# Accustomer/CUDA-AKAZE

Measured on AMD Instinct MI355X. Metric: pairs_per_sec_detect_describe_match_1080p, higher is better.
Workload: dtype f32; 1 GPU; configs[1]: 1920x1080 grayscale pairs, 4 octaves x 4 sublevels, PM_G2, MLDB-486, max_pts 10000, float path; detect+describe both images + match, D2H included; pairs_per_launch_sequence=256, distinct_pairs_per_gpu=16, float_sequences_enqueued=77, octave_streams=one stream per context, step_pipeline=2, rank0_gpu_numa_node=1

## Files before the change

### cuda-akaze_amd/akaze_hip/__init__.py

```python
import ctypes as C
import os

import numpy as np

try:
    import torch as _torch
except ImportError:
    _torch = None

_HERE = os.path.dirname(os.path.abspath(__file__))
LIB_PATH = os.environ.get("HAK_LIB") or os.path.join(os.path.dirname(_HERE), "libhipakaze.so")

FLEN = 61
MAX_DIST = 96
PM_G1, PM_G2, WEICKERT, CHARBONNIER = 0, 1, 2, 3

POINT_DTYPE = np.dtype([
    ("x", "<f4"), ("y", "<f4"), ("octave", "<i4"), ("response", "<f4"), ("size", "<f4"), ("angle", "<f4"),
    ("features", "u1", (FLEN,)), ("_pad", "u1", (3,)),
    ("match", "<i4"), ("distance", "<i4"), ("match_x", "<f4"), ("match_y", "<f4"),
])
assert POINT_DTYPE.itemsize == 104
MATCH_PAIR_DTYPE = np.dtype([("query", "<i4"), ("train", "<i4"), ("distance", "<i4"), ("second", "<i4"),
                             ("x1", "<f4"), ("y1", "<f4"), ("x2", "<f4"), ("y2", "<f4")])
assert MATCH_PAIR_DTYPE.itemsize == 32
HOMOGRAPHY_DTYPE = np.dtype([("H", "<f4", (9,)), ("inliers", "<i4"), ("hypothesis", "<i4"), ("refined", "<i4"),
                             ("n", "<i4")])
assert HOMOGRAPHY_DTYPE.itemsize == 52


class HakError(RuntimeError):
    pass


class hak_config(C.Structure):
    _fields_ = [
        ("noctaves", C.c_int), ("max_scale", C.c_int), ("per", C.c_float), ("kcontrast", C.c_float),
        ("soffset", C.c_float), ("reordering", C.c_int), ("derivative_factor", C.c_float),
        ("dthreshold", C.c_float), ("diffusivity", C.c_int), ("descriptor_pattern_size", C.c_int),
        ("max_pts", C.c_int), ("upright", C.c_int), ("batch", C.c_int),
    ]


class hak_traffic(C.Structure):
    _fields_ = [("fed_px_steps", C.c_double), ("fed_bytes", C.c_double), ("all_stage_bytes", C.c_double),
                ("fed_launches", C.c_int), ("fed_fused_bytes", C.c_double), ("hessian_bytes", C.c_double),
                ("prologue_bytes", C.c_double), ("describe_bytes", C.c_double), ("nms_bytes", C.c_double)]


PROF = dict(fed=0, lowpass=1, flow=2, hessian=3, contrast=4, down=5, extrema=6, nms=7, describe=8, match=9)

_vp, _fp, _ip = C.c_void_p, C.POINTER(C.c_float), C.POINTER(C.c_int)
SYMBOLS = {
    "hak_device_count": (C.c_int, []),
    "hak_set_device": (C.c_int, [C.c_int]),
    "hak_last_error": (C.c_char_p, []),
    "hak_default_config": (None, [C.POINTER(hak_config)]),
    "hak_create": (C.c_int, [C.POINTER(hak_config), C.c_int, C.c_int, C.POINTER(_vp)]),
    "hak_destroy": (None, [_vp]),
    "hak_set_stream": (C.c_int, [_vp, _vp]),
    "hak_sync": (C.c_int, [_vp]),
    "hak_wait_event": (C.c_int, [_vp, _vp]),
    "hak_phase_event": (C.c_int, [_vp, C.POINTER(C.c_void_p)]),
    "hak_set_concurrency": (C.c_int, [_vp, C.c_int]),
    "hak_set_null_order": (C.c_int, [_vp, C.c_int]),
    "hak_set_retain_best": (C.c_int, [_vp, C.c_int]),
    "hak_set_retain_grid": (C.c_int, [_vp, C.c_int]),
    "hak_detect_and_compute": (C.c_int, [_vp, _vp, C.c_int, _vp, C.c_int, _ip, _vp, C.c_int]),
    "hak_detect_and_compute_pair": (C.c_int, [_vp, _vp, _vp, C.c_int, _vp, _vp, C.c_int, C.c_int, _ip, _ip, _vp, _vp, C.c_int, C.c_int]),
    "hak_detect_and_compute_batch": (C.c_int, [_vp, _vp, C.c_long, C.c_int, C.c_int, _vp, _vp, C.c_int]),
    "hak_fast_detect_and_compute": (C.c_int, [_vp, _vp, C.c_int, _vp, C.c_int, _ip, _vp, C.c_int]),
    "hak_fast_detect_and_compute_batch": (C.c_int, [_vp, _vp, C.c_long, C.c_int, C.c_int, _vp, _vp, C.c_int]),
    "hak_match": (C.c_int, [_vp, _vp, C.c_int, _vp, C.c_int, _vp]),
    "hak_match_batch": (C.c_int, [_vp, _vp, _vp, C.c_int]),
    "hak_match_knn2": (C.c_int, [_vp, _vp, C.c_int, _vp, C.c_int, C.c_int, C.c_int, C.c_int, C.c_int, _vp, _vp, _ip, _vp]),
    "hak_match_knn2_batch": (C.c_int, [_vp, _vp, _vp, C.c_int, C.c_int, C.c_int, C.c_int, C.c_int, _vp, _vp]),
    "hak_find_homography": (C.c_int, [_vp, _vp, C.c_int, C.c_int, C.c_float, C.c_uint, C.c_int, _vp, _vp]),
    "hak_find_homography_batch": (C.c_int, [_vp, _vp, C.c_long, _vp, C.c_int, C.c_int, C.c_float, C.c_uint, C.c_int, _vp, _vp]),
    "hak_match_guided": (C.c_int, [_vp, _vp, C.c_int, _vp, C.c_int, _fp, C.c_float, C.c_int, C.c_int, C.c_int, C.c_int, _vp, _vp, _ip, _vp]),
    "hak_match_guided_batch": (C.c_int, [_vp, _vp, _vp, C.c_int, _vp, C.c_float, C.c_int, C.c_int, C.c_int, C.c_int, _vp, _vp]),
    "hak_points_alloc": (C.c_int, [C.POINTER(_vp), C.c_int]),
    "hak_points_free": (C.c_int, [_vp]),
    "hak_image_alloc": (C.c_int, [C.POINTER(_vp), C.c_int, C.c_int, _ip]),
    "hak_image_upload": (C.c_int, [_vp, C.c_int, _vp, C.c_int, C.c_int]),
    "hak_image_free": (C.c_int, [_vp]),
    "hak_ingest_u8": (C.c_int, [_vp, _vp, C.c_long, C.c_int, _vp, C.c_long, C.c_int, C.c_int, C.c_int, C.c_int]),
    "hak_host_alloc": (C.c_int, [C.POINTER(_vp), C.c_long]),
    "hak_host_free": (C.c_int, [_vp]),
    "hak_download_batch": (C.c_int, [_vp, _vp, _vp, C.c_int, _vp, _vp]),
    "hak_memcpy_d2h": (C.c_int, [_vp, _vp, C.c_long]),
    "hak_memcpy_h2d": (C.c_int, [_vp, _vp, C.c_long]),
    "hak_fed_tau": (C.c_int, [C.c_float, C.c_int, C.c_float, C.c_int, _fp, C.c_int]),
    "hak_gauss_taps": (None, [C.c_float, C.c_int, _fp]),
    "hak_compare_indices": (None, [_ip, _ip]),
    "hak_describe_plan_query": (C.c_int, [C.c_int, C.POINTER(C.c_uint), C.POINTER(C.c_uint)]),
    "hak_query_schedule": (C.c_int, [_vp, _ip, _ip, _fp, _fp]),
    "hak_query_geometry": (C.c_int, [_vp, _ip]),
    "hak_query_traffic": (C.c_int, [_vp, C.c_int, C.POINTER(hak_traffic)]),
    "hak_prof_enable": (C.c_int, [_vp, C.c_int]),
    "hak_prof_read": (C.c_int, [_vp, C.c_int, C.POINTER(C.c_double), _ip]),
    "hak_prof_reset": (C.c_int, [_vp]),
}
TEST_SYMBOLS = {
    "hak_debug_plane": (C.c_int, [_vp, C.c_int, C.c_int, C.c_int, C.c_int, _vp]),
    "hak_debug_kcontrast": (C.c_int, [_vp, C.c_int, _fp]),
    "hak_op_lowpass": (C.c_int, [_vp, _vp, C.c_int, C.c_int, C.c_int, C.c_float, C.c_int]),
    "hak_op_down_smooth": (C.c_int, [_vp, _vp, _vp, C.c_int, C.c_int, C.c_int, C.c_int, C.c_int, C.c_int]),
    "hak_op_kcontrast": (C.c_int, [_vp, C.c_int, C.c_int, C.c_int, C.c_float, _fp, _fp, _ip]),
    "hak_op_flow": (C.c_int, [_vp, _vp, C.c_int, C.c_int, C.c_int, C.c_int, C.c_float]),
    "hak_op_nld_steps": (C.c_int, [_vp, _vp, _vp, _vp, C.c_int, C.c_int, C.c_int, _fp, C.c_int]),
    "hak_op_rcp_check": (C.c_int, [C.c_uint, C.c_uint, C.POINTER(C.c_ulonglong)]),
    "hak_op_smooth_flow": (C.c_int, [_vp, _vp, _vp, C.c_int, C.c_int, C.c_int, C.c_int, C.c_float]),
    "hak_op_hessian": (C.c_int, [_vp, _vp, _vp, _vp, C.c_int, C.c_int, C.c_int, C.c_int]),
    "hak_debug_set_plane": (C.c_int, [_vp, C.c_int, C.c_int, C.c_int, C.c_int, _vp]),
    "hak_op_tail_begin": (C.c_int, [_vp]),
    "hak_op_tail_level": (C.c_int, [_vp, C.c_int, C.c_int, _vp]),
    "hak_op_tail_det_level": (C.c_int, [_vp, C.c_int, C.c_int, _vp]),
    "hak_op_tail_seed": (C.c_int, [_vp, _vp, _vp]),
    "hak_op_tail_finish": (C.c_int, [_vp, _vp, C.c_int, C.c_int, C.c_int, _ip]),
    "hak_op_orient_describe": (C.c_int, [_vp, _vp, C.c_int, C.c_int]),
    "hak_op_copy_probe": (C.c_int, [C.c_long, C.c_int, C.POINTER(C.c_double)]),
    "hak_op_copy_probe_shapes": (C.c_int, [C.c_long, C.c_int, C.POINTER(C.c_double), C.c_int]),
    "hak_op_stream_probe": (C.c_int, [C.c_int, C.c_int, C.c_int, C.c_int, C.c_int, C.c_int, C.POINTER(C.c_double), C.POINTER(C.c_double)]),
    "hak_op_hess_probe": (C.c_int, [C.c_int, C.c_int, C.c_int, C.c_int, C.c_int, C.POINTER(C.c_double), C.POINTER(C.c_double)]),
    "hak_debug_fill_match_scratch": (C.c_int, [_vp, C.c_int]),
    "hak_op_gather_probe": (C.c_int, [C.c_long, C.c_int, C.c_int, C.c_int, C.POINTER(C.c_double)]),
}

if not os.path.exists(LIB_PATH):
    raise ImportError(
        f"{LIB_PATH} is missing: build it with `python -c 'import __graft_entry__ as g; g.build()'` "
        "(there is no CPU fallback for the HIP path)")
TEST_LIB_PATH = os.path.join(os.path.dirname(LIB_PATH), "libhipakaze_test.so")


class _Libs:

    def __init__(self):
        self.product = C.CDLL(LIB_PATH, mode=C.RTLD_GLOBAL)
        self.test = None
        for name, (res, args) in SYMBOLS.items():
            try:
                f = getattr(self.product, name)
            except AttributeError:
                if os.environ.get("HAK_LIB"):
                    continue
                raise
            f.restype, f.argtypes = res, args
            setattr(self, name, f)

    def load_test(self):
        if self.test is None:
            if not os.path.exists(TEST_LIB_PATH):
                raise ImportError(f"{TEST_LIB_PATH} is missing: build it with `make -C cuda-akaze_amd/csrc`")
            self.test = C.CDLL(TEST_LIB_PATH)
            for name, (res, args) in TEST_SYMBOLS.items():
                f = getattr(self.test, name)
                f.restype, f.argtypes = res, args
                setattr(self, name, f)
        return self.test

    def __getattr__(self, name):
        if name in TEST_SYMBOLS:
            self.load_test()
            return self.__dict__[name]
        raise AttributeError(name)


lib = _Libs()


def check(status):
    if status != 0:
        raise HakError(lib.hak_last_error().decode() or f"libhipakaze status {status}")


def iAlignUp(a, b):
    return a - a % b + b if a % b else a


def device_count():
    return lib.hak_device_count()


def default_config(**kw):
    cfg = hak_config()
    lib.hak_default_config(C.byref(cfg))
    for k, v in kw.items():
        setattr(cfg, k, v)
    return cfg


def fed_tau(T, M=1, tau_max=0.25, reordering=True):
    buf = np.zeros(4096, np.float32)
    n = lib.hak_fed_tau(T, M, tau_max, int(reordering), buf.ctypes.data_as(_fp), 4096)
    if n < 0:
        raise HakError("FED cycle too long")
    return buf[:n].copy()


def gauss_taps(var, radius):
    buf = np.zeros(8, np.float32)
    lib.hak_gauss_taps(var, radius, buf.ctypes.data_as(_fp))
    return buf[:radius + 1].copy()


def compare_indices():
    a = np.zeros(488, np.int32)
    b = np.zeros(488, np.int32)
    lib.hak_compare_indices(a.ctypes.data_as(_ip), b.ctypes.data_as(_ip))
    return a, b


def describe_plan(pattern_size):
    pos = np.zeros((7, 64), np.uint32)
    cell = np.zeros((7, 64), np.uint32)
    ok = lib.hak_describe_plan_query(pattern_size, pos.ctypes.data_as(C.POINTER(C.c_uint)), cell.ctypes.data_as(C.POINTER(C.c_uint)))
    return bool(ok), pos, cell


class AkazeData:

    def __init__(self):
        self.num_pts = 0
        self.max_pts = 0
        self.h_data = None
        self.d_data = None
        self.h_pinned = None


def initAkazeData(data, max_pts, host, dev, pinned=False):
    data.num_pts = 0
    data.max_pts = max_pts
    data.h_pinned = None
    if host and pinned:
        hp = _vp()
        check(lib.hak_host_alloc(C.byref(hp), max_pts * POINT_DTYPE.itemsize))
        data.h_pinned = hp.value
        buf = (C.c_uint8 * (max_pts * POINT_DTYPE.itemsize)).from_address(hp.value)
        data.h_data = np.frombuffer(buf, dtype=POINT_DTYPE)
        data.h_data[:] = np.zeros(1, POINT_DTYPE)[0]
    else:
        data.h_data = np.zeros(max_pts, POINT_DTYPE) if host else None
    data.d_data = None
    if dev:
        p = _vp()
        check(lib.hak_points_alloc(C.byref(p), max_pts))
        data.d_data = p.value


def freeAkazeData(data):
    if data.d_data is not None:
        check(lib.hak_points_free(data.d_data))
    data.d_data = None
    data.h_data = None
    if getattr(data, "h_pinned", None):
        check(lib.hak_host_free(data.h_pinned))
        data.h_pinned = None
    data.num_pts = 0
    data.max_pts = 0


class Akazer:
# ... 225 lines not shown
```

### cuda-akaze_amd/csrc/fed_common.h

```cpp
#pragma once
#include "hak_internal.h"
#include <type_traits>

template <typename V> struct FedV;
template <> struct FedV<float> { using V4 = float4; };
template <> struct FedV<int> { using V4 = int4; };
__device__ __forceinline__ float4 mk4(float a, float b, float c, float d) { return make_float4(a, b, c, d); }
__device__ __forceinline__ int4 mk4(int a, int b, int c, int d) { return make_int4(a, b, c, d); }
__device__ __forceinline__ float vadd(float a, float b) { return a + b; }
__device__ __forceinline__ float vsub(float a, float b) { return a - b; }
__device__ __forceinline__ float vmul(float a, float b) { return a * b; }
__device__ __forceinline__ int vadd(int a, int b) { return (int)((unsigned)a + (unsigned)b); }
__device__ __forceinline__ int vsub(int a, int b) { return (int)((unsigned)a - (unsigned)b); }
__device__ __forceinline__ int vmul(int a, int b) { return (int)((unsigned)a * (unsigned)b); }
__device__ __forceinline__ float vstep(float f, float sum, float L) { return fmaf(f, sum, L); }
__device__ __forceinline__ int vstep(int f, int sum, int L) { return vadd(vmul(f, sum >> 16) >> 16, L); }

template <typename V, int NS>
struct FedFacs { V f[NS]; };

__device__ __forceinline__ int hak_dpp_shr1(int v) { return __builtin_amdgcn_update_dpp(0, v, 0x138, 0xf, 0xf, true); }
__device__ __forceinline__ int hak_dpp_shl1(int v) { return __builtin_amdgcn_update_dpp(0, v, 0x130, 0xf, 0xf, true); }
__device__ __forceinline__ float wave_shr1(float v) { return __int_as_float(hak_dpp_shr1(__float_as_int(v))); }
__device__ __forceinline__ float wave_shl1(float v) { return __int_as_float(hak_dpp_shl1(__float_as_int(v))); }
__device__ __forceinline__ int wave_shr1(int v)
{
    int r = hak_dpp_shr1(v);
    asm volatile("" : "+v"(r));
    return r;
}
__device__ __forceinline__ int wave_shl1(int v)
{
    int r = hak_dpp_shl1(v);
    asm volatile("" : "+v"(r));
    return r;
}

typedef float hak_v4f __attribute__((ext_vector_type(4)));
typedef int hak_v4i __attribute__((ext_vector_type(4)));
__device__ __forceinline__ void hak_store_nt(float4* p, const float4 v)
{
    const hak_v4f t = {v.x, v.y, v.z, v.w};
    __builtin_nontemporal_store(t, reinterpret_cast<hak_v4f*>(p));
}
__device__ __forceinline__ void hak_store_nt(int4* p, const int4 v)
{
    const hak_v4i t = {v.x, v.y, v.z, v.w};
    __builtin_nontemporal_store(t, reinterpret_cast<hak_v4i*>(p));
}

typedef unsigned hak_v4u __attribute__((ext_vector_type(4)));
constexpr unsigned HAK_BUF_OOB = 0x40000000u;
__device__ __forceinline__ __amdgpu_buffer_rsrc_t hak_buf_rsrc(void* base)
{
    return __builtin_amdgcn_make_buffer_rsrc(base, 0, HAK_BUF_OOB, 0x00020000);
}
__device__ __forceinline__ void hak_buf_store_nt(__amdgpu_buffer_rsrc_t r, unsigned voff, const float4 v)
{
    const hak_v4u d = {__float_as_uint(v.x), __float_as_uint(v.y), __float_as_uint(v.z), __float_as_uint(v.w)};
    __builtin_amdgcn_raw_buffer_store_b128(d, r, voff, 0, 2);
}
__device__ __forceinline__ void hak_buf_store_nt(__amdgpu_buffer_rsrc_t r, unsigned voff, const int4 v)
{
    const hak_v4u d = {(unsigned)v.x, (unsigned)v.y, (unsigned)v.z, (unsigned)v.w};
    __builtin_amdgcn_raw_buffer_store_b128(d, r, voff, 0, 2);
}

__device__ __forceinline__ float4 hak_load_stream(const float4* p)
{
#ifdef HAK_NT_LOADS
    const hak_v4f t = __builtin_nontemporal_load(reinterpret_cast<const hak_v4f*>(p));
    return make_float4(t.x, t.y, t.z, t.w);
#else
    return *p;
#endif
}
__device__ __forceinline__ int4 hak_load_stream(const int4* p)
{
#ifdef HAK_NT_LOADS
    const hak_v4i t = __builtin_nontemporal_load(reinterpret_cast<const hak_v4i*>(p));
    return make_int4(t.x, t.y, t.z, t.w);
#else
    return *p;
#endif
}

constexpr int pmod(int a, int m) { return ((a % m) + m) % m; }

template <typename V> struct GHrow { V h1, h2, h3, h4; };
__device__ __forceinline__ float vneg(float a) { return -a; }
__device__ __forceinline__ int vneg(int a) { return (int)(0u - (unsigned)a); }

template <bool XEDGE, typename V, typename V4>
__device__ __forceinline__ V4 fed_row(const V4 Lc, const GHrow<V>& gh, const V4 Qn, const V4 Qp, int x0, int w, V stepfac)
{
    const V Lr = wave_shl1(Lc.x);
    const V d1 = vsub(Lc.y, Lc.x), d2 = vsub(Lc.z, Lc.y), d3 = vsub(Lc.w, Lc.z), d4 = vsub(Lr, Lc.w);
    const V P1 = vmul(gh.h1, d1), P2 = vmul(gh.h2, d2), P3 = vmul(gh.h3, d3);
    V P4 = vmul(gh.h4, d4);
    if (XEDGE) P4 = x0 + 3 == w - 1 ? vneg(P3) : P4;
    V P0 = wave_shr1(P4);
    if (XEDGE) P0 = x0 == 0 ? vneg(P1) : P0;
    V4 o;
    o.x = vstep(stepfac, vsub(vadd(vsub(P1, P0), Qn.x), Qp.x), Lc.x);
    o.y = vstep(stepfac, vsub(vadd(vsub(P2, P1), Qn.y), Qp.y), Lc.y);
    o.z = vstep(stepfac, vsub(vadd(vsub(P3, P2), Qn.z), Qp.z), Lc.z);
    o.w = vstep(stepfac, vsub(vadd(vsub(P4, P3), Qn.w), Qp.w), Lc.w);
    return o;
}
template <typename V, typename V4>
__device__ __forceinline__ V4 fed_q(const V4 gv, const V4 Ln, const V4 Lc)
{
    return mk4(vmul(gv.x, vsub(Ln.x, Lc.x)), vmul(gv.y, vsub(Ln.y, Lc.y)), vmul(gv.z, vsub(Ln.z, Lc.z)), vmul(gv.w, vsub(Ln.w, Lc.w)));
}
template <typename V4> __device__ __forceinline__ V4 vneg4(const V4 a) { return mk4(vneg(a.x), vneg(a.y), vneg(a.z), vneg(a.w)); }
template <typename V4> __device__ __forceinline__ V4 vsel4(const bool c, const V4 a, const V4 b)
{
    return mk4(c ? a.x : b.x, c ? a.y : b.y, c ? a.z : b.z, c ? a.w : b.w);
}


template <typename V> struct SfTaps { V k0, k1, k2; };
__device__ __forceinline__ float sf_conv(float c, float a1, float b1, float a2, float b2, const SfTaps<float>& t)
{
    float ws = c * t.k0;
    ws += t.k1 * (a1 + b1);
    ws += t.k2 * (a2 + b2);
    return ws;
}
__device__ __forceinline__ int sf_conv(int c, int a1, int b1, int a2, int b2, const SfTaps<int>& t)
{
    const unsigned ws = (unsigned)c * (unsigned)t.k0 + (unsigned)t.k1 * (unsigned)(a1 + b1) + (unsigned)t.k2 * (unsigned)(a2 + b2);
    return (int)ws >> 16;
}
__device__ __forceinline__ float sf_dif2(float dx, float dy, float ikc) { return ikc * (dx * dx + dy * dy); }
__device__ __forceinline__ float sf_dif2(int dx, int dy, float ikc)
{
    return (float)(int)((unsigned)dx * (unsigned)dx + (unsigned)dy * (unsigned)dy) * ikc;
}
__device__ __forceinline__ void sf_store_g(float* o, float g) { *o = g; }
__device__ __forceinline__ void sf_store_g(int* o, float g) { *o = (int)(g * 65536 + 0.5f); }

__device__ __forceinline__ float sf_g_value(float g) { return g; }
__device__ __forceinline__ int sf_g_value_int(float g) { return (int)(g * 65536 + 0.5f); }
template <typename V> __device__ __forceinline__ V sf_g_as(float g);
template <> __device__ __forceinline__ float sf_g_as<float>(float g) { return g; }
template <> __device__ __forceinline__ int sf_g_as<int>(float g) { return (int)(g * 65536 + 0.5f); }

__device__ __forceinline__ float hak_rcp_newton(float d)
{
    const float y0 = __builtin_amdgcn_rcpf(d);
    const float e = fmaf(-d, y0, 1.0f);
    return fmaf(e, y0, y0);
}
```

### cuda-akaze_amd/csrc/hak_api.hip

```cpp
#include "hak_internal.h"
#include <chrono>
#include <cmath>
#include <cstdio>
#include <cstring>
#include <mutex>
#include <string>
#include <vector>

#include "hak_ctx.h"

static thread_local std::string g_err;
int hak_fail(const std::string& m) { g_err = m; return 1; }

extern "C" const char* hak_last_error(void) { return g_err.c_str(); }

extern "C" int hak_device_count(void)
{
    int n = 0;
    if (hipGetDeviceCount(&n) != hipSuccess) return 0;
    return n;
}

extern "C" int hak_set_device(int dev)
{
// ... 719 lines not shown
        if (!c) { pool_release(sc, false); (void)hipFree(buf); }
        return fail("hak_match_guided: out of device memory for the search scratch");
    }
    int4* fwd = sc->knn;
    int4* rev = sc->knn + n1;
    *sc->h_cnt = -1;
    {
        ProfScope ps(c, HAK_PROF_MATCH);
        hak_launch_guided(st, d_pts1, d_pts2, nullptr, nullptr, n1, n2, 0, 0, 1, nullptr, H, radius, cross_check ? 1 : 0,
                          hak_guided_scratch_carve(buf, 1, cap2, rev, 0), fwd, 0);
        hak_launch_knn2_finish(st, d_pts1, d_pts2, nullptr, n1, 0, 0, 1, fwd, cross_check ? rev : nullptr, 0, ratio_num, ratio_den,
                               cross_check ? 1 : 0, max_dist, d_out, 0, sc->d_cnt, sc);
    }
    int rc = 0;
    if (hipGetLastError() != hipSuccess) rc = fail("guided match launch failed");
    if (!rc && hipStreamSynchronize(st) != hipSuccess) rc = fail("hipStreamSynchronize(guided match)");
    rc = match_list_tail(c, sc, rc, h_pts1, d_pts1, n1, d_out, count, h_out);
    if (!c) (void)hipFree(buf);
    return rc;
}

extern "C" int hak_match_guided_batch(hak_ctx* c, hak_point* d_points, const int* d_num_pts, int npairs, const hak_homography* d_H,
                                      float radius, int ratio_num, int ratio_den, int cross_check, int max_dist, hak_match_pair* d_out,
                                      int* d_counts)
{
    if (!c) return fail("hak_match_guided_batch needs a context");
    if (!d_points || !d_num_pts || !d_H || !d_counts || npairs < 1) return fail("bad argument");
    if (2 * npairs > c->cfg.batch + 1) return fail("npairs exceeds the context's batch capacity");
    if (guided_args(radius, ratio_num, ratio_den)) return 1;
    if (max_dist <= 0) max_dist = HAK_MAX_DIST;
    const long mp = c->cfg.max_pts;
    if (!hak_mkey_fits(mp)) return fail("max_pts must stay below 2^20 for the matcher");
    if (knn_scratch(c)) return 1;
    const long npair_cap = (c->cfg.batch + 1) / 2;
    if (guided_scratch(c, hak_guided_scratch_bytes(npair_cap, mp))) return 1;
    order_after_null_stream(c, c->stream);
    int4* fwd = c->knn;
    int4* rev = c->knn + (size_t)npair_cap * mp;
    { ProfScope ps(c, HAK_PROF_MATCH);
      hak_launch_guided(c->stream, d_points, d_points + mp, d_num_pts, d_num_pts + 1, (int)mp, (int)mp, 2 * mp, 2 * mp, npairs, d_H, nullptr,
                        radius, cross_check ? 1 : 0, hak_guided_scratch_carve(c->guided, npair_cap, mp, rev, mp), fwd, mp);
      hak_launch_knn2_finish(c->stream, d_points, d_points + mp, d_num_pts, 0, 2 * mp, 2 * mp, npairs, fwd, cross_check ? rev : nullptr,
                             mp, ratio_num, ratio_den, cross_check ? 1 : 0, max_dist, d_out, mp, d_counts); }
    if (hipGetLastError() != hipSuccess) return fail("guided match launch failed");
    return 0;
}

extern "C" int hak_points_alloc(hak_point** d, int count)
{
    HIP_TRY(hipMalloc((void**)d, sizeof(hak_point) * (size_t)count));
    HIP_TRY(hipMemset(*d, 0, sizeof(hak_point) * (size_t)count));
    HIP_TRY(hipStreamSynchronize(nullptr));
    return 0;
}
extern "C" int hak_points_free(hak_point* d) { HIP_TRY(hipFree(d)); return 0; }

extern "C" int hak_image_alloc(float** d, int w, int h, int* pitch)
{
    int p = (w % 128 != 0) ? (w - w % 128 + 128) : w;
    HIP_TRY(hipMalloc((void**)d, sizeof(float) * (size_t)p * h));
    if (pitch) *pitch = p;
    return 0;
}
extern "C" int hak_image_upload(float* d, int pitch, const float* hsrc, int w, int h)
{
    HIP_TRY(hipMemcpy2D(d, sizeof(float) * pitch, hsrc, sizeof(float) * w, sizeof(float) * w, h, hipMemcpyHostToDevice));
    return 0;
}
extern "C" int hak_image_free(float* d) { HIP_TRY(hipFree(d)); return 0; }

extern "C" int hak_ingest_u8(hak_ctx* c, const unsigned char* d_src, long src_stride, int src_pitch,
                             float* d_dst, long dst_stride, int dst_pitch, int w, int h, int nimg)
{
    if (!d_src || !d_dst || w < 1 || h < 1 || nimg < 1 || src_pitch < w || dst_pitch < w) return fail("bad ingest argument");
    if (hak_device_count() == 0) return fail("no HIP device: libhipakaze has no CPU fallback");
    order_after_null_stream(c, c ? c->stream : nullptr);
    hak_launch_ingest_u8(c ? c->stream : nullptr, d_src, src_stride, src_pitch, d_dst, dst_stride, dst_pitch, w, h, nimg);
    if (hipGetLastError() != hipSuccess) return fail("ingest launch failed");
    return 0;
}
extern "C" int hak_host_alloc(void** p, long bytes) { HIP_TRY(hipHostMalloc(p, (size_t)bytes)); return 0; }
extern "C" int hak_host_free(void* p) { HIP_TRY(hipHostFree(p)); return 0; }

extern "C" int hak_download_batch(hak_ctx* c, const hak_point* d_points, const int* d_num_pts, int nimg,
                                  hak_point* h_points, int* h_num_pts)
{
    if (!c || !d_points || !d_num_pts || !h_points || !h_num_pts) return fail("null argument");
    {
        hipPointerAttribute_t ap{}, an{};
        const bool pinned = hipPointerGetAttributes(&ap, h_points) == hipSuccess && ap.type == hipMemoryTypeHost &&
                            hipPointerGetAttributes(&an, h_num_pts) == hipSuccess && an.type == hipMemoryTypeHost;
        (void)hipGetLastError();
        if (pinned) {
            hak_launch_download(c->stream, d_points, d_num_pts, c->cfg.max_pts, nimg, h_points, h_num_pts);
            if (hipGetLastError() != hipSuccess) return fail("download launch failed");
            HIP_TRY(hipStreamSynchronize(c->stream));
            return 0;
        }
    }
    HIP_TRY(hipMemcpyAsync(h_num_pts, d_num_pts, sizeof(int) * (size_t)nimg, hipMemcpyDeviceToHost, c->stream));
    HIP_TRY(hipStreamSynchronize(c->stream));
    const long mp = c->cfg.max_pts;
    for (int i = 0; i < nimg; i++)
        if (h_num_pts[i] > 0)
            HIP_TRY(hipMemcpyAsync(h_points + i * mp, d_points + i * mp, sizeof(hak_point) * (size_t)h_num_pts[i],
                                   hipMemcpyDeviceToHost, c->stream));
    HIP_TRY(hipStreamSynchronize(c->stream));
    return 0;
}

extern "C" int hak_memcpy_d2h(void* dst, const void* src, long bytes)
{
    HIP_TRY(hipMemcpy(dst, src, (size_t)bytes, hipMemcpyDeviceToHost));
    return 0;
}
extern "C" int hak_memcpy_h2d(void* dst, const void* src, long bytes)
{
    HIP_TRY(hipMemcpy(dst, src, (size_t)bytes, hipMemcpyHostToDevice));
    return 0;
}

extern "C" int hak_query_schedule(const hak_ctx* c, int* nsteps, int* sigma_size, float* sizes, float* borders)
{
    if (!c) return -1;
    for (size_t l = 0; l < c->plan.size(); l++) {
        if (nsteps) nsteps[l] = c->plan[l].nsteps;
        if (sigma_size) sigma_size[l] = c->plan[l].sigma_size;
        if (sizes) sizes[l] = c->plan[l].size;
        if (borders) borders[l] = c->plan[l].border;
    }
    return c->L.noct;
}

extern "C" int hak_query_geometry(const hak_ctx* c, int* whp)
{
    if (!c) return -1;
    for (int o = 0; o < c->L.noct; o++) {
        whp[3 * o] = c->L.oct[o].w; whp[3 * o + 1] = c->L.oct[o].h; whp[3 * o + 2] = c->L.oct[o].p;
    }
    return c->L.noct;
}

extern "C" int hak_query_traffic(const hak_ctx* c, int npts_hint, hak_traffic* out)
{
    if (!c || !out) return fail("null argument");
    const HakLayout& L = c->L;
    double pxsteps = 0, all = 0, folded = 0;
    int launches = 0;
    for (int o = 0; o < L.noct; o++) {
        const double N = (double)L.oct[o].w * L.oct[o].h;
        for (int s = 0; s < L.ms; s++) {
            const LevelPlan& lp = c->plan[(size_t)o * L.ms + s];
            pxsteps += N * lp.nsteps;
            launches += lp.nsteps ? hak_fed_groups(lp.nsteps, c->knobs.max_fuse, L.oct[o].w) : 0;
            if (s > 0 && hak_fed_sf_covers(c->knobs, c->cfg.diffusivity, L.oct[o], c->cfg.batch)) folded += 16.0 * N;
            if (s == 0 && o > 0 && hak_fed_sf_covers(c->knobs, c->cfg.diffusivity, L.oct[o], c->cfg.batch, &L.oct[o - 1]))
                folded += 4.0 * L.oct[o - 1].w * L.oct[o - 1].h + 16.0 * N;
            if (o == 0 && s == 0) all += 56.0 * N;
            else if (s == 0) all += 4.0 * L.oct[o - 1].w * L.oct[o - 1].h + 8.0 * N + 8.0 * N + 24.0 * N + 4.0 * N;
            else all += 44.0 * N;
        }
    }
    all += 16.0 * L.oct[0].w * L.oct[0].h;
    all += 12.0 * pxsteps;
    all += (872.0 + 5292.0 + 104.0) * npts_hint;
    out->fed_px_steps = pxsteps;
    out->fed_bytes = 12.0 * pxsteps + folded;
    out->all_stage_bytes = all;
    out->fed_launches = launches;
    out->fed_fused_bytes = c->fed_fused_bytes;
    double lvl_px = 0;
    for (int o = 0; o < L.noct; o++) lvl_px += (double)L.ms * L.oct[o].w * L.oct[o].h;
    out->hessian_bytes = 12.0 * lvl_px;
    out->prologue_bytes = 16.0 * L.oct[0].w * L.oct[0].h;
    out->describe_bytes = (872.0 + 5292.0) * npts_hint;
    out->nms_bytes = 104.0 * npts_hint;
    return 0;
}

extern "C" int hak_prof_enable(hak_ctx* c, int on) { if (!c) return 1; c->prof_on = on != 0; return 0; }
extern "C" int hak_prof_reset(hak_ctx* c)
{
    if (!c) return 1;
    for (auto& p : c->prof) { p.used = 0; p.acc_ms = 0; p.launches = 0; }
    return 0;
}
extern "C" int hak_prof_read(hak_ctx* c, int k, double* total_ms, int* launches)
{
    if (!c || k < 0 || k >= HAK_PROF_COUNT) return fail("bad profile class");
    HIP_TRY(hipStreamSynchronize(c->stream));
    ProfClass& p = c->prof[k];
    for (size_t i = 0; i + 1 < p.used; i += 2) {
        float ms = 0;
        HIP_TRY(hipEventElapsedTime(&ms, p.ev[i], p.ev[i + 1]));
        p.acc_ms += ms;
    }
    p.used = 0;
    if (total_ms) *total_ms = p.acc_ms;
    if (launches) *launches = p.launches;
    return 0;
}
```

### cuda-akaze_amd/csrc/hak_internal.h

```cpp
#pragma once
#include <cstdlib>
#include <hip/hip_runtime.h>
#include <stdint.h>
#include "../../include/hipakaze.h"
#include "hak_knobs.h"

#define HAK_NBINS 300
#define HAK_WAVE 64

struct HakOct {
    int w, h, p;
    long plane;
};

struct HakLayout {
    int noct, ms;
    HakOct oct[HAK_MAX_OCTAVES];
    long lvl_off[HAK_MAX_OCTAVES];
    long smooth_off[HAK_MAX_OCTAVES], flow_off[HAK_MAX_OCTAVES], tmp_off[HAK_MAX_OCTAVES];
    long arena;

    __host__ __device__ long lt(int o, int s) const { return lvl_off[o] + (long)s * oct[o].plane; }
    __host__ __device__ long dxy(int o, int s) const { return lvl_off[o] + (long)(ms + 2 * s) * oct[o].plane; }
};
// ... 235 lines not shown
    unsigned prefix;
    int pad;
};
#define HAK_SEL_BINS 2048
#define HAK_SEL_PASSES 3
struct HakSelScratch {
    HakSelState* st = nullptr;
    unsigned* bins = nullptr;
    int* tie = nullptr;
};

__device__ __forceinline__ unsigned sel_key(unsigned u, int fast)
{
    return fast ? (u ^ 0x80000000u) : ((u >> 31) ? ~u : (u | 0x80000000u));
}
__device__ __forceinline__ int sel_cap(int img, int max_pts, int cap0, int cap1)
{
    return cap0 > 0 ? (img == 0 ? cap0 : cap1) : max_pts;
}

#define HAK_GRID_MIN 8
#define HAK_GRID_MAX 128
struct HakGridState {
    int active;
    int cap;
    int q;
    int rem;
};
struct HakGridScratch {
    HakGridState* st = nullptr;
    int* count = nullptr;
    unsigned long long* comp = nullptr;
    long cell_cap = 0;
    int G = 0;
};

struct HakBatch {
    float* base;
    long stride;
    int nimg;
    HakImgState* state;
    unsigned long long* maps;
    long map_stride;
    unsigned long long* bitmap;
    int* rowcount;
    unsigned long long* cand;
    long cand_cap;
    const HakKnobs* knobs = nullptr;
    int* perm = nullptr;
    int perm_cap = 0;
    int cap0 = 0, cap1 = 0;
    HakSelScratch sel{};
    HakGridScratch grid{};
};
static inline HakKnobs hak_knobs_of(const HakBatch* b) { return (b && b->knobs) ? *b->knobs : hak_knobs_from_env(); }
template <typename V>
static inline HakExtremaArgs<V> hak_extrema_args(const HakBatch* b, const HakLayout* L, const HakTables* htab, int octave, int sub, V threshold)
{
    HakExtremaArgs<V> ex{};
    if (b) {
        const int layer = octave * L->ms + sub;
        ex.maps = b->maps; ex.map_stride = b->map_stride; ex.cand = b->cand; ex.cand_cap = b->cand_cap;
        ex.state = b->state; ex.p0 = L->oct[0].p; ex.octave = octave; ex.layer = layer;
        ex.psz = (int)htab->borders[octave * L->ms]; ex.border = htab->borders[layer]; ex.threshold = threshold;
    }
    return ex;
}

void hak_launch_lowpass(hipStream_t st, const float* src, long src_stride, int src_pitch, float* dst, long dst_stride,
                        int w, int h, int p, int nimg, const float* taps, int R);
void hak_launch_down_smooth(hipStream_t st, const float* src, float* dst, float* smooth, long stride,
                            HakOct so, HakOct dd, int nimg, const float* taps);
void hak_launch_contrast(hipStream_t st, const float* smooth, long stride, int w, int h, int p, int nimg,
                         HakImgState* state, float per, int noct);
void hak_launch_reset_state(hipStream_t st, HakImgState* state, int nimg);
void hak_launch_flow(hipStream_t st, const float* src, float* dst, long stride, int w, int h, int p, int nimg,
                     int diffusivity, const HakImgState* state, int octave, float fixed_ikc = 0.f);
static inline bool hak_stream_pays(int mode, int w, int h, int nimg)
{
    if (mode != 1) return mode != 0;
    const long strips = (w + 239) / 240;
    return strips * ((h + 31) / 32) * nimg >= 2048;
}
static inline int hak_stream_rows(int h, long strips_times_images, int min_rows)
{
    const long want = hak_process_knobs().stream_min_waves;
    int nseg = 4 * ((h + 512) / 1024 > 1 ? (h + 512) / 1024 : 1);
    while (strips_times_images * nseg < want && (h + 2 * nseg - 1) / (2 * nseg) >= min_rows) nseg *= 2;
    const int ry = (h + nseg - 1) / nseg;
    return ry > min_rows ? ry : min_rows;
}
static inline bool hak_hessian_stream_covers(int w, int h, int step, bool lp)
{
    return step >= 1 && step <= 4 && (w & 3) == 0 && w >= 16 && h >= 2 * step + 2 && (!lp || h >= 8);
}
bool hak_launch_hessian_stream(hipStream_t st, const float* src, float* dxy, float* det, bool store_det, long stride,
                               int w, int h, int p, int nimg, int step, float fac1, float fac2,
                               const HakBatch* b, const HakLayout* L, const HakTables* htab, int octave, int sub, float dthreshold,
                               const float* lp_taps = nullptr);
bool hak_launch_hessian_stream(hipStream_t st, const int* src, int* dxy, int* det, bool store_det, long stride,
                               int w, int h, int p, int nimg, int step, int fac1, int fac2,
                               const HakBatch* b, const HakLayout* L, const HakTables* htab, int octave, int sub, int idthreshold);
bool hak_launch_hessian_level(hipStream_t st, const float* src, float* dxy, float* det, bool store_det, long stride,
                              int w, int h, int p, int nimg, int step,
                              const HakBatch* b, const HakLayout* L, const HakTables* htab, int octave, int sub, float dthreshold,
                              const float* lp_taps = nullptr);
bool hak_launch_hessian_level(hipStream_t st, const int* src, int* dxy, int* det, bool store_det, long stride,
                              int w, int h, int p, int nimg, int step,
                              const HakBatch* b, const HakLayout* L, const HakTables* htab, int octave, int sub, int idthreshold);
bool hak_launch_base_stream(hipStream_t st, const float* img, long img_stride, int sp, float* lt, float* grad, long stride, int w, int h,
                            int p, int nimg, const float* taps1, const float* taps_base, int R, HakImgState* state, int mode);
bool hak_launch_base_stream(hipStream_t st, const unsigned char* img, long img_stride, int sp, int* lt, int* grad, long stride, int w,
                            int h, int p, int nimg, const int* taps1, const int* taps_base, int R, HakImgState* state, int mode);
bool hak_launch_base_level(hipStream_t st, const float* img, long img_stride, int sp, float* lt, float* grad_scratch, long stride,
                           int w, int h, int p, int nimg, const float* taps1, const float* taps_base, int R,
                           HakImgState* state, float per, int noct, const HakKnobs& knobs);
bool hak_launch_base_level(hipStream_t st, const unsigned char* img, long img_stride, int sp, int* lt, int* grad_scratch, long stride,
                           int w, int h, int p, int nimg, const int* taps1, const int* taps_base, int R, HakImgState* state,
                           float per, int noct, const HakKnobs& knobs);
void hak_launch_smooth_flow(hipStream_t st, const float* src, float* smooth, float* flow, long stride,
                            int w, int h, int p, int nimg, const float* taps, int diffusivity,
                            const HakImgState* state, int octave, float fixed_ikc = 0.f);
void hak_launch_smooth_flow(hipStream_t st, const int* src, int* smooth, int* flow, long stride,
                            int w, int h, int p, int nimg, const int* taps, int diffusivity,
                            const HakImgState* state, int octave);
#define HAK_LEVEL_TILE_MAX_PX (1920L * 1088L)
int hak_launch_level_tile(hipStream_t st, const float* src, HakOct so, bool head, float* smooth, float* dst, float* tmp, long stride,
                          HakOct dd, int nimg, const float* taps, int diffusivity, const float* tau, int n,
                          const HakImgState* state, int octave, float* dxy = nullptr, int step = 0, const HakBatch* b = nullptr,
                          const HakLayout* L = nullptr, const HakTables* htab = nullptr, int sub = 0, float dthreshold = 0.f,
                          bool* hess_done = nullptr, float fixed_ikc = 0.f);
int hak_launch_level_tile(hipStream_t st, const int* src, HakOct so, bool head, int* smooth, int* dst, int* tmp, long stride,
                          HakOct dd, int nimg, const int* taps, int diffusivity, const float* tau, int n,
                          const HakImgState* state, int octave, int* dxy = nullptr, int step = 0, const HakBatch* b = nullptr,
                          const HakLayout* L = nullptr, const HakTables* htab = nullptr, int sub = 0, int idthreshold = 0, bool* hess_done = nullptr);
int hak_launch_rcp_check(unsigned lo, unsigned hi, unsigned long long* d_bad);
static inline bool hak_fed_sf_covers(const HakKnobs& kn, int diffusivity, const HakOct& dd, int nimg, const HakOct* so = nullptr)
{
    if (!hak_stream_pays(kn.fuse_sf, dd.w, dd.h, nimg) || diffusivity != HAK_PM_G2 || (dd.w & 3) != 0 || dd.w < 16 || dd.h < 8) return false;
    return !so || (kn.fuse_head && !(so->w & 1) && !(so->h & 1));
}
bool hak_launch_fed_sf_head(hipStream_t st, const float* src, HakOct so, float* smooth, float* flow, float* dst, long stride,
                            HakOct dd, int nimg, const float* taps, int diffusivity, const float* tau, int ns,
                            const HakImgState* state, int octave, bool write_g);
bool hak_launch_fed_sf_head(hipStream_t st, const int* src, HakOct so, int* smooth, int* flow, int* dst, long stride,
                            HakOct dd, int nimg, const int* taps, int diffusivity, const float* tau, int ns,
                            const HakImgState* state, int octave, bool write_g);
bool hak_launch_fed_sf(hipStream_t st, const float* src, float* smooth, float* flow, float* dst, long stride,
                       int w, int h, int p, int nimg, const float* taps, int diffusivity, const float* tau, int ns,
                       const HakImgState* state, int octave, bool write_g, bool store_smooth = true, float fixed_ikc = 0.f);
bool hak_launch_fed_sf(hipStream_t st, const int* src, int* smooth, int* flow, int* dst, long stride,
                       int w, int h, int p, int nimg, const int* taps, int diffusivity, const float* tau, int ns,
                       const HakImgState* state, int octave, bool write_g);
int hak_fed_groups(int n, int max_fuse, int w);
int hak_fed_group_size(int n, int G, int g);
void hak_launch_fed_group(hipStream_t st, const float* src, const float* flow, float* dst, long stride,
                          int w, int h, int p, int nimg, const float* tau, int ns);
void hak_launch_fed_group(hipStream_t st, const int* src, const int* flow, int* dst, long stride,
                          int w, int h, int p, int nimg, const float* tau, int ns);
void hak_launch_derivate(hipStream_t st, const float* src, float* dxy, long stride,
                         int w, int h, int p, int nimg, int step);
void hak_launch_hessian(hipStream_t st, const float* dxy, float* det, long stride,
                        int w, int h, int p, int nimg, int step);
void hak_deriv_factors(float* fac1, float* fac2);
void hak_launch_deinterleave(hipStream_t st, const float* ab, float* a, float* b, int w, int h, int p);

void hak_launch_ingest_u8(hipStream_t st, const unsigned char* src, long src_stride, int sp, float* dst, long dst_stride,
                          int dp, int w, int h, int nimg);

void hak_launch_extrema_level(hipStream_t st, const HakBatch& b, const HakLayout& L, const HakTables* htab, int octave,
                              int s, float dthreshold, long det_off);
void hak_launch_extrema_level(hipStream_t st, const HakBatch& b, const HakLayout& L, const HakTables* htab, int octave, int s, int threshold,
                              long det_off);
void hak_launch_download(hipStream_t st, const hak_point* d_points, const int* d_num, long max_pts, int nimg, hak_point* h_points,
                         int* h_num);
struct HakPairDst { hak_point* d[2]; hak_point* h[2]; int cap[2]; };
void hak_launch_download_pair(hipStream_t st, const hak_point* src, const int* d_num, long max_pts, const HakPairDst& dst, int* h_num);
void hak_launch_nms_emit(hipStream_t st, const HakBatch& b, const HakLayout& L, const HakTables* tab, int psz,
                         hak_point* points, int max_pts, int* num_out, int fast = 0, int refine = 1);
void hak_launch_clear_maps(hipStream_t st, const HakBatch& b, const HakLayout& L);
void hak_launch_select(hipStream_t st, const HakBatch& b, const HakLayout& L, int max_pts, int cap0, int cap1, int fast);
void hak_launch_grid_select(hipStream_t st, const HakBatch& b, const HakLayout& L, int max_pts, int cap0, int cap1, int fast);
void hak_launch_seed_maps(hipStream_t st, const HakBatch& b, const HakLayout& L, const unsigned* d_resp_bits, const int* d_layer);

void hak_launch_down_smooth(hipStream_t st, const int* src, int* dst, int* smooth, long stride, HakOct so, HakOct dd, int nimg,
                            const int* taps);
void hak_launch_contrast(hipStream_t st, const int* smooth, long stride, int w, int h, int p, int nimg, HakImgState* state,
                         float per, int noct);
void hak_launch_flow(hipStream_t st, const int* src, int* dst, long stride, int w, int h, int p, int nimg, int type,
                     const HakImgState* state, int octave);
void hakf_launch_reset(hipStream_t st, HakImgState* state, int nimg);
void hakf_launch_conv_u8(hipStream_t st, const unsigned char* src, long src_stride, int sp, int* dst, long dst_stride,
                         int w, int h, int p, int nimg, const int* taps, int R);
void hakf_launch_conv_int(hipStream_t st, const int* src, int* dst, long stride, int w, int h, int p, int nimg, const int* taps, int R);
void hakf_launch_nld_step(hipStream_t st, const int* src, const int* flow, int* dst, long stride, int w, int h, int p, int nimg, float tau);
void hakf_launch_hessian(hipStream_t st, const int* src, int* dxy, int* det, long stride, int w, int h, int p, int nimg, int step);
void hakf_launch_det(hipStream_t st, const int* dxy, int* det, long stride, int w, int h, int p, int nimg, int step);
void hakf_launch_describe(hipStream_t st, const HakBatch& b, const HakLayout& L, const HakTables* tab, hak_point* points, int max_pts,
                          int patsize, int upright, int desc, int planned);

void hak_launch_describe(hipStream_t st, const HakBatch& b, const HakLayout& L, const HakTables* tab,
                         hak_point* points, int max_pts, int patsize, int upright, int desc, int planned, int orient = 1);

#define HAK_COPY_SHAPES 26
int hak_launch_copy_probe(long bytes, int iters, double* ms_per_copy, double* shapes_ms = nullptr);
int hak_launch_gather_probe(long bytes, int blocks, int per_lane, int iters, double* ms_per_launch);
int hak_launch_stream_probe(int w, int h, int nimg, int nwrite, int warm, int iters, double* ms, double* bytes);
int hak_launch_hess_probe(int w, int h, int nimg, int step, int iters, double* ms, double* bytes);

static inline int hak_grid_x(int blocks) { return blocks < 1 ? 1 : blocks > 4096 ? 4096 : blocks; }

#define HAK_MKEY_BITS 20
#define HAK_MKEY_EMPTY 0xFFFFFFFFu
static inline bool hak_mkey_fits(long n) { return n < (1L << HAK_MKEY_BITS); }
__device__ __forceinline__ unsigned hak_mkey(unsigned dist, unsigned index) { return (dist << HAK_MKEY_BITS) | index; }
__device__ __forceinline__ unsigned hak_mkey_dist(unsigned k) { return k >> HAK_MKEY_BITS; }
__device__ __forceinline__ int hak_mkey_index(unsigned k) { return (int)(k & ((1u << HAK_MKEY_BITS) - 1u)); }
__device__ __forceinline__ void hak_mkey_two_smallest(unsigned& best, unsigned& sec, unsigned key)
{
    sec = min(sec, max(best, key));
    best = min(best, key);
}
__device__ __forceinline__ void hak_desc_load(const hak_point* p, unsigned int d[16])
{
    const unsigned int* f = reinterpret_cast<const unsigned int*>(p->features);
#pragma unroll
    for (int i = 0; i < 15; i++) d[i] = f[i];
    d[15] = f[15] & 0xFFu;
}
__device__ __forceinline__ unsigned hak_bcnt_acc(unsigned x, unsigned acc)
{
    unsigned r;
    asm("v_bcnt_u32_b32 %0, %1, %2" : "=v"(r) : "v"(x), "v"(acc));
    return r;
}
#define HAK_KNN_NO_DIST 512
__device__ __forceinline__ int4 hak_knn_none() { return make_int4(-1, HAK_KNN_NO_DIST, HAK_KNN_NO_DIST, 0); }
__device__ __forceinline__ int4 hak_knn_record(unsigned k1, unsigned k2)
{
    if (k1 == HAK_MKEY_EMPTY) return hak_knn_none();
    return make_int4(hak_mkey_index(k1), (int)hak_mkey_dist(k1), k2 == HAK_MKEY_EMPTY ? HAK_KNN_NO_DIST : (int)hak_mkey_dist(k2), 0);
}
__device__ __forceinline__ void hak_match_store(hak_point* p1, const hak_point* __restrict__ pts2, bool ok, int bi, int dist)
{
    if (ok) {
        p1->match = bi;
        p1->distance = dist;
        p1->match_x = pts2[bi].x;
        p1->match_y = pts2[bi].y;
    } else {
        p1->match = -1;
        p1->distance = -1;
        p1->match_x = -1.f;
        p1->match_y = -1.f;
    }
}
__device__ __forceinline__ void hak_match_decide(hak_point* p1, const hak_point* __restrict__ pts2, int n2, unsigned kmin, int attain)
{
    const int dmin = (int)hak_mkey_dist(kmin);
    const bool ok = kmin != HAK_MKEY_EMPTY && attain == 1 && dmin < HAK_MAX_DIST;
    hak_match_store(p1, pts2, ok, min(hak_mkey_index(kmin), max(n2 - 1, 0)), dmin);
}
template <typename F>
__device__ __forceinline__ void hak_match_decide_classes(hak_point* p1, const hak_point* __restrict__ pts2, int n2, F cls)
{
    unsigned kmin = cls(0);
#pragma unroll
    for (int t = 1; t < 16; t++)
        if (hak_mkey_dist(cls(t)) < hak_mkey_dist(kmin)) kmin = cls(t);
    int attain = 0;
#pragma unroll
    for (int t = 0; t < 16; t++) attain += hak_mkey_dist(cls(t)) == hak_mkey_dist(kmin) ? 1 : 0;
    hak_match_decide(p1, pts2, n2, kmin, attain);
}
__device__ __forceinline__ void hak_match_merge_slice(unsigned& K, unsigned& M, unsigned k2, unsigned m2)
{
    if (hak_mkey_dist(k2) < hak_mkey_dist(K)) M = m2;
    else if (hak_mkey_dist(k2) == hak_mkey_dist(K)) M |= m2;
    K = min(K, k2);
}
__device__ __forceinline__ bool hak_knn2_rule(const int i, const int n1, const int4* __restrict__ fwd, const int4* __restrict__ rev,
                                              const int ratio_num, const int ratio_den, const int cross, const int max_dist, int4& f)
{
    f = hak_knn_none();
    if (i >= n1) return false;
    f = fwd[i];
    bool ok = f.x >= 0 && f.y < max_dist && (long)f.y * ratio_den < (long)f.z * ratio_num;
    if (ok && cross) ok = rev[f.x].x == i;
    return ok;
}
__device__ __forceinline__ hak_match_pair hak_knn2_pair(int i, const int4 f, const hak_point* pts1, const hak_point* __restrict__ pts2)
{
    hak_match_pair r;
    r.query = i; r.train = f.x; r.distance = f.y; r.second = f.z;
    r.x1 = pts1[i].x; r.y1 = pts1[i].y; r.x2 = pts2[f.x].x; r.y2 = pts2[f.x].y;
    return r;
}

struct HakMatchScratch {
    unsigned* keys = nullptr; long keys_cap = 0;
    int* ticket = nullptr; long ticket_cap = 0;
    uint2* part = nullptr; long part_cap = 0;
    int4* knn = nullptr; long knn_cap = 0;
    int* blk = nullptr; long blk_cap = 0;
    int* d_cnt = nullptr; int* h_cnt = nullptr;
    int device = -1;
};
// ... 35 lines not shown
```

### cuda-akaze_amd/csrc/hak_knobs.h

```cpp
#pragma once
#include "../../include/hipakaze.h"

#define HAK_FED_MAX_FUSE 4

struct HakKnobs {
    int hess_stream = 1;
    int base_stream = 1;
    int base_hist = 0;
    int hess_cbuf = 256;
    int desc_order = 4;
    int desc_plan = 1;
    int desc_sort = 1;
    int hess_lp = 0;
    int level_tile = 1;
    int level_hess = 1;
    int level_min_steps = 8;
    int level_min_blocks = 96;
    int fuse_sf = 1;
    int fuse_head = 1;
    int max_fuse = 4;
    int hist_min_blocks = 256;
    int hist_rpb_max = 8;
    int hess_side = 0;
    int spine_max_px = 0;
    int side_streams = HAK_MAX_OCTAVES;
    int graph_pads = 1;
    int tail_fork = 1;
    int graph = 1;
    int serial = 0;
    int null_order = 1;
    int timing = 0;
    int prof_fence = 0;
    int stream_min_waves = 2048;
    int download_blocks = 128;
};
HakKnobs hak_knobs_from_env();
const HakKnobs& hak_process_knobs();

struct HakMatchKnobs {
    int valu = 0;
    int qt = 1;
    int slices = 0;
};
HakMatchKnobs hak_match_knobs_from_env();
```

### cuda-akaze_amd/csrc/hak_sequence.hip

```cpp
#include "hak_internal.h"
#include <cstdio>
#include <cstring>
#include <string>
#include <type_traits>

#include "hak_ctx.h"

static thread_local const char* g_launch_err = nullptr;
void hak_note_launch_error(const char* msg) { if (!g_launch_err) g_launch_err = msg; }

void order_after_null_stream(hak_ctx* c, hipStream_t st)
{
    if (!c || !c->null_order || !c->ev_null || st == nullptr) return;
    const hipError_t q = hipStreamQuery(nullptr);
    if (q == hipSuccess) return;
    (void)hipGetLastError();
    if (hipEventRecord(c->ev_null, nullptr) != hipSuccess || hipStreamWaitEvent(st, c->ev_null, 0) != hipSuccess) (void)hipGetLastError();
}

void maps_guard_begin(hak_ctx* c)
{
    if (c->maps_dirty) {
        const size_t h = c->L.oct[0].h, words = (c->L.oct[0].w + 63) / 64, B = c->cfg.batch;
        (void)hipMemsetAsync(c->maps, 0, sizeof(unsigned long long) * (size_t)c->L.oct[0].plane * B, c->stream);
        (void)hipMemsetAsync(c->bitmap, 0, sizeof(unsigned long long) * h * words * B, c->stream);
        (void)hipMemsetAsync(c->rowcount, 0, sizeof(int) * h * B, c->stream);
    }
    c->maps_dirty = true;
}
int maps_guard_end(hak_ctx* c, int rc)
{
    if (!rc) c->maps_dirty = false;
    if (c->ev_last) (void)hipEventRecord(c->ev_last, c->sync_stream ? c->sync_stream : c->stream);
    return rc;
}

static bool level_tile_pays(const hak_ctx* c, const HakOct& oc, int nimg)
{
    const int mode = c->knobs.level_tile;
    if (mode != 1) return mode != 0;
    return c->knobs.fuse_sf != 2 && (long)oc.w * oc.h * nimg <= HAK_LEVEL_TILE_MAX_PX;
}

static bool spine_pays(const hak_ctx* c, int nimg)
{
    const long max_px = c->knobs.spine_max_px;
    if (max_px > 0 && c->knobs.level_tile == 1) return c->knobs.fuse_sf != 2 && (long)c->L.oct[0].w * c->L.oct[0].h * nimg <= max_px;
    return level_tile_pays(c, c->L.oct[0], nimg);
}

struct LevelArgs {
    hak_ctx* c;
    HakBatch b;
    const void* images;
    long image_stride;
    int pitch, nimg;
    bool hess_fused[HAK_MAX_OCTAVES * HAK_MAX_SCALES];
    bool hess_lp[HAK_MAX_OCTAVES * HAK_MAX_SCALES];
};

static LevelArgs level_args(hak_ctx* c, const void* images, long image_stride, int pitch, int nimg)
{
    const HakLayout& L = c->L;
    LevelArgs a{c, HakBatch{c->arena, L.arena, nimg, c->state, c->maps, L.oct[0].plane, c->bitmap, c->rowcount, c->cand, c->cand_cap, &c->knobs,
                            c->perm, c->cfg.max_pts},
                images, image_stride, pitch, nimg, {}, {}};
    hak_batch_selection(c, a.b);
    return a;
}

template <typename V> constexpr bool is_fast = std::is_same_v<V, int>;
template <typename V> static const V* taps_of(const float* f, const int* i) { if constexpr (is_fast<V>) return i; else return f; }
template <typename V> static V dthreshold_of(const hak_ctx* c) { if constexpr (is_fast<V>) return 65; else return c->cfg.dthreshold; }

template <typename V>
static void build_level(LevelArgs& a, int o, int s, hipStream_t st, V* smooth_alt = nullptr)
{
    hak_ctx* const c = a.c;
    hak_ctx* const pc = is_fast<V> ? nullptr : c;
    const hak_config& cfg = c->cfg;
    const HakLayout& L = c->L;
    const HakKnobs& kn = c->knobs;
    const int nimg = a.nimg;
    V* const A = reinterpret_cast<V*>(c->arena);
    const long S = L.arena;
    const HakOct oc = L.oct[o];
    V* smooth = smooth_alt ? smooth_alt : A + L.smooth_off[o];
    V* flow = A + L.flow_off[o];
    V* tmp = A + L.tmp_off[o];
    const LevelPlan& lp = c->plan[(size_t)o * L.ms + s];
    V* Lt = A + L.lt(o, s);
    const V* taps1 = taps_of<V>(c->taps1, c->itaps1);
    auto count_fed = [&](int nl, double bytes) { if constexpr (!is_fast<V>) { c->fed_launches += nl; c->fed_fused_bytes += bytes; } };
    if (o == 0 && s == 0) {
        ProfScope ps(pc, HAK_PROF_CONTRAST, st);
        const auto* img = static_cast<const std::conditional_t<is_fast<V>, unsigned char, float>*>(a.images);
        const V* taps_base = taps_of<V>(c->taps_base, c->itaps_base);
        const bool based = hak_launch_base_level(st, img, a.image_stride, a.pitch, Lt, tmp, S, oc.w, oc.h, oc.p, nimg, taps1, taps_base, c->base_R,
                                                 c->state, cfg.per, L.noct, kn);
        if constexpr (is_fast<V>) {
            if (!based) {
                hakf_launch_conv_u8(st, img, a.image_stride, a.pitch, smooth, S, oc.w, oc.h, oc.p, nimg, taps1, 2);
                hak_launch_contrast(st, smooth, S, oc.w, oc.h, oc.p, nimg, c->state, cfg.per, L.noct);
                hakf_launch_conv_u8(st, img, a.image_stride, a.pitch, Lt, S, oc.w, oc.h, oc.p, nimg, taps_base, c->base_R);
            }
        } else (void)based;
        return;
    }
    const int n = lp.nsteps;
    if (level_tile_pays(c, oc, nimg) && (is_fast<V> || s == 0 || n >= kn.level_min_steps || kn.level_tile == 2)) {
        ProfScope ps(pc, HAK_PROF_FED, st);
        const int nl = hak_launch_level_tile(st, s == 0 ? A + L.lt(o - 1, 0) : A + L.lt(o, s - 1), s == 0 ? L.oct[o - 1] : oc, s == 0, smooth, Lt, tmp, S,
                                             oc, nimg, taps1, cfg.diffusivity, lp.tau.data(), n, c->state, o,
                                             kn.level_hess ? A + L.dxy(o, s) : nullptr, lp.sigma_size, &a.b, &L, &c->htab, s, dthreshold_of<V>(c),
                                             &a.hess_fused[o * HAK_MAX_SCALES + s]);
        count_fed(nl, (s == 0 ? 1.0 * L.oct[o - 1].w * L.oct[o - 1].h : 4.0 * oc.w * oc.h) + 8.0 * oc.w * oc.h + (nl - 1) * 12.0 * oc.w * oc.h);
        return;
    }
    const int G = hak_fed_groups(n, kn.max_fuse, oc.w);
    const int ns0 = hak_fed_group_size(n, G, 0);
    V* dst0 = (G % 2 == 1) ? Lt : tmp;
    const V* fsrc;
    bool fused_first = false;
    if (s == 0) {
        if (hak_fed_sf_covers(kn, cfg.diffusivity, oc, nimg, &L.oct[o - 1])) {
            ProfScope ps(pc, HAK_PROF_FED, st);
            fused_first = hak_launch_fed_sf_head(st, A + L.lt(o - 1, 0), L.oct[o - 1], smooth, flow, dst0, S, oc, nimg, taps1, cfg.diffusivity,
                                                 lp.tau.data(), ns0, c->state, o, G > 1);
            if (fused_first) count_fed(1, 2.0 * L.oct[o - 1].w * L.oct[o - 1].h + (G > 1 ? 12.0 : 8.0) * oc.w * oc.h);
        }
        V* first = (G % 2 == 0) ? Lt : tmp;
        if (!fused_first) {
            { ProfScope ps(pc, HAK_PROF_DOWN, st);
              hak_launch_down_smooth(st, A + L.lt(o - 1, 0), first, smooth, S, L.oct[o - 1], oc, nimg, taps1); }
            ProfScope ps(pc, HAK_PROF_FLOW, st);
            hak_launch_flow(st, smooth, flow, S, oc.w, oc.h, oc.p, nimg, cfg.diffusivity, c->state, o);
        }
        fsrc = first;
    } else {
        fsrc = A + L.lt(o, s - 1);
        if (hak_fed_sf_covers(kn, cfg.diffusivity, oc, nimg)) {
            ProfScope ps(pc, HAK_PROF_FED, st);
            if constexpr (is_fast<V>) {
                fused_first = hak_launch_fed_sf(st, fsrc, smooth, flow, dst0, S, oc.w, oc.h, oc.p, nimg, taps1, cfg.diffusivity, lp.tau.data(),
                                                ns0, c->state, o, G > 1);
            } else {
                const bool lp_hess = kn.hess_lp != 0 && hak_stream_pays(kn.hess_stream, oc.w, oc.h, nimg) &&
                                     hak_hessian_stream_covers(oc.w, oc.h, lp.sigma_size, true);
                fused_first = hak_launch_fed_sf(st, fsrc, smooth, flow, dst0, S, oc.w, oc.h, oc.p, nimg, taps1, cfg.diffusivity, lp.tau.data(),
                                                ns0, c->state, o, G > 1, !lp_hess);
                if (fused_first) {
                    a.hess_lp[o * HAK_MAX_SCALES + s] = lp_hess;
                    count_fed(1, ((G > 1 ? 16.0 : 12.0) - (lp_hess ? 4.0 : 0.0)) * oc.w * oc.h);
                }
            }
        }
        if (!fused_first) {
            ProfScope ps(pc, HAK_PROF_LOWPASS, st);
            hak_launch_smooth_flow(st, fsrc, smooth, flow, S, oc.w, oc.h, oc.p, nimg, taps1, cfg.diffusivity, c->state, o);
        }
    }
    const V* src = fsrc;
    int done = 0;
    for (int g = 0; g < G; g++) {
        const int ns = hak_fed_group_size(n, G, g);
        V* dst = ((G - g) % 2 == 1) ? Lt : tmp;
        if (!(g == 0 && fused_first)) {
            ProfScope ps(pc, HAK_PROF_FED, st);
            hak_launch_fed_group(st, src, flow, dst, S, oc.w, oc.h, oc.p, nimg, lp.tau.data() + done, ns);
            count_fed(1, 12.0 * oc.w * oc.h);
        }
        done += ns;
        src = dst;
    }
}

template <typename V>
static void hessian_level(LevelArgs& a, int o, int s, hipStream_t st, const V* smooth_alt = nullptr)
{
    if (a.hess_fused[o * HAK_MAX_SCALES + s]) return;
    hak_ctx* const c = a.c;
    const HakLayout& L = c->L;
    V* const A = reinterpret_cast<V*>(c->arena);
    const HakOct oc = L.oct[o];
    const LevelPlan& lp = c->plan[(size_t)o * L.ms + s];
    const bool lph = a.hess_lp[o * HAK_MAX_SCALES + s];
    const V* hsrc = (o == 0 && s == 0) ? A + L.lt(0, 0) : lph ? A + L.lt(o, s - 1) : smooth_alt ? smooth_alt : A + L.smooth_off[o];
    const V thr = dthreshold_of<V>(c);
    ProfScope ps(is_fast<V> ? nullptr : c, HAK_PROF_HESSIAN, st);
    bool done;
    if constexpr (is_fast<V>)
        done = hak_launch_hessian_level(st, hsrc, A + L.dxy(o, s), A + L.flow_off[o], false, L.arena, oc.w, oc.h, oc.p, a.nimg, lp.sigma_size,
                                        &a.b, &L, &c->htab, o, s, thr);
    else
        done = hak_launch_hessian_level(st, hsrc, A + L.dxy(o, s), A + L.flow_off[o], false, L.arena, oc.w, oc.h, oc.p, a.nimg, lp.sigma_size,
                                        &a.b, &L, &c->htab, o, s, thr, lph ? c->taps1 : nullptr);
    if (!done) hak_launch_extrema_level(st, a.b, L, &c->htab, o, s, thr, L.flow_off[o]);
}

static int enqueue_detect(hak_ctx* c, const float* d_images, long image_stride, int pitch, int nimg,
                          hak_point* d_points, int* d_num_pts, int desc, int max_pts, hak_point* h_points = nullptr, int cap0 = 0, int cap1 = 0)
{
    const hak_config& cfg = c->cfg;
    const HakLayout& L = c->L;
    const bool spine = c->concurrent && L.noct > 1 && spine_pays(c, nimg);
    const hipStream_t main_st = c->stream;
    c->sync_stream = c->stream;
    float* A = c->arena;
    LevelArgs a = level_args(c, d_images, image_stride, pitch, nimg);
    HakBatch& b = a.b;
    b.cap0 = cap0; b.cap1 = cap1;
    c->last_fast = false;
    c->fed_launches = 0;
    c->fed_fused_bytes = 0;

    hak_launch_reset_state(main_st, c->state, nimg);

    if (spine) {
        const int last = L.noct - 1;
        hipGraphNode_t head_node[HAK_MAX_OCTAVES] = {};
        hipGraph_t cap_graph = nullptr;
        for (int o = 0; o <= last; o++) {
            build_level<float>(a, o, 0, main_st);
            if (o < last) {
                (void)hipEventRecord(c->ev_ready[o], main_st);
                hipStreamCaptureStatus cs = hipStreamCaptureStatusNone;
                const hipGraphNode_t* deps = nullptr;
                size_t ndeps = 0;
                if (hipStreamGetCaptureInfo_v2(main_st, &cs, nullptr, &cap_graph, &deps, &ndeps) == hipSuccess &&
                    cs == hipStreamCaptureStatusActive && ndeps == 1) head_node[o] = deps[0];
                else (void)hipGetLastError();
            }
        }
        for (int o = 0; o < last && c->knobs.graph_pads; o++)
            for (int k = 0; k < last - 1 - o && head_node[o] && cap_graph; k++) {
                hipGraphNode_t pad = nullptr;
                if (hipGraphAddEmptyNode(&pad, cap_graph, &head_node[o], 1) != hipSuccess) (void)hipGetLastError();
            }
        const int nside = c->knobs.side_streams < last ? c->knobs.side_streams : (last > 0 ? last : 1);
        auto side_of = [&](int o) { return c->oct_stream[1 + (o < nside ? o : nside - 1)]; };
        for (int s = 0; s < L.ms; s++)
            for (int k = 0; k <= last; k++) {
                const int o = k == 0 ? last : k - 1;
                const hipStream_t st = o == last ? main_st : side_of(o);
                if (s == 0 && o != last && hipStreamWaitEvent(st, c->ev_ready[o], 0) != hipSuccess) return fail("stream wait");
                if (s > 0) build_level<float>(a, o, s, st);
                hessian_level<float>(a, o, s, st);
            }
        for (int i = 0; i < nside && last > 0; i++) {
            (void)hipEventRecord(c->ev_done[i + 1], c->oct_stream[i + 1]);
            if (hipStreamWaitEvent(main_st, c->ev_done[i + 1], 0) != hipSuccess) return fail("stream join");
        }
    } else {
        bool side0 = c->knobs.hess_side != 0 && c->concurrent && L.noct > 1 && c->hess_stream && L.ms <= HAK_MAX_SCALES &&
                     !hak_stream_pays(c->knobs.hess_stream, L.oct[0].w, L.oct[0].h, nimg) && !level_tile_pays(c, L.oct[0], nimg) &&
                     !hak_stream_pays(c->knobs.fuse_sf, L.oct[0].w, L.oct[0].h, nimg);
        for (int s = 1; s < L.ms && side0; s++)
            side0 = hak_fed_groups(c->plan[s].nsteps, c->knobs.max_fuse, L.oct[0].w) == 1 && c->plan[s].sigma_size <= 4;
        hipStream_t st = main_st;
        for (int o = 0; o < L.noct; o++) {
            if (c->concurrent && o > 0) {
                st = c->oct_stream[o];
                if (hipStreamWaitEvent(st, c->ev_ready[o - 1], 0) != hipSuccess) return fail("stream wait");
            }
            for (int s = 0; s < L.ms; s++) {
                if (o == 0 && side0) {
                    float* sm = (s & 1) ? A + L.tmp_off[0] : A + L.smooth_off[0];
                    if (s >= 2 && hipStreamWaitEvent(st, c->ev_hd[s - 2], 0) != hipSuccess) return fail("stream wait");
                    build_level<float>(a, 0, s, st, sm);
                    if (s == 0) (void)hipEventRecord(c->ev_ready[0], st);
                    (void)hipEventRecord(c->ev_hs[s], st);
                    if (hipStreamWaitEvent(c->hess_stream, c->ev_hs[s], 0) != hipSuccess) return fail("stream wait");
                    hessian_level<float>(a, 0, s, c->hess_stream, sm);
                    (void)hipEventRecord(c->ev_hd[s], c->hess_stream);
                    continue;
                }
                build_level<float>(a, o, s, st);
                if (c->concurrent && s == 0) (void)hipEventRecord(c->ev_ready[o], st);
                hessian_level<float>(a, o, s, st);
            }
            if (c->concurrent && o > 0) (void)hipEventRecord(c->ev_done[o], st);
        }
        if (c->concurrent)
            for (int o = 1; o < L.noct; o++)
                if (hipStreamWaitEvent(main_st, c->ev_done[o], 0) != hipSuccess) return fail("stream join");
        if (side0)
            if (hipStreamWaitEvent(main_st, c->ev_hd[L.ms - 1], 0) != hipSuccess) return fail("stream join");
    }
    {
        hipStreamCaptureStatus cs = hipStreamCaptureStatusNone;
        hipGraph_t g = nullptr;
        const hipGraphNode_t* deps = nullptr;
        size_t ndeps = 0;
        if (hipStreamGetCaptureInfo_v2(main_st, &cs, nullptr, &g, &deps, &ndeps) != hipSuccess) { (void)hipGetLastError(); cs = hipStreamCaptureStatusNone; }
        hipError_t pe;
        if (cs == hipStreamCaptureStatusActive) {
            hipGraphNode_t node = nullptr;
            pe = hipGraphAddEventRecordNode(&node, g, deps, ndeps, c->ev_phase);
            if (pe == hipSuccess) pe = hipStreamUpdateCaptureDependencies(main_st, &node, 1, hipStreamSetCaptureDependencies);
        } else pe = hipEventRecord(c->ev_phase, main_st);
        if (pe != hipSuccess) { fprintf(stderr, "hipakaze: phase event record: %s\n", hipGetErrorString(pe)); (void)hipGetLastError(); }
    }
    bool tail_fork = false;
    { ProfScope ps(c, HAK_PROF_NMS);
      hak_launch_nms_emit(main_st, b, L, c->dtab, c->psz, d_points, max_pts, d_num_pts);
      tail_fork = spine && c->knobs.tail_fork;
      if (tail_fork) {
          (void)hipEventRecord(c->ev_tail_fork, main_st);
          if (hipStreamWaitEvent(c->oct_stream[1], c->ev_tail_fork, 0) != hipSuccess) return fail("stream wait");
          hak_launch_clear_maps(c->oct_stream[1], b, L);
          (void)hipEventRecord(c->ev_tail_join, c->oct_stream[1]);
      } else hak_launch_clear_maps(main_st, b, L); }
    { ProfScope ps(c, HAK_PROF_DESCRIBE);
      hak_launch_describe(main_st, b, L, c->dtab, d_points, max_pts, cfg.descriptor_pattern_size, cfg.upright, desc, c->htab.dsc_plan_ok); }
    if (h_points)
        hak_launch_download(main_st, d_points, d_num_pts, max_pts, nimg, h_points, c->h_num);
    if (tail_fork && hipStreamWaitEvent(main_st, c->ev_tail_join, 0) != hipSuccess) return fail("stream join");
    if (hipGetLastError() != hipSuccess) return fail("kernel launch failed");
    if (g_launch_err) { const char* m = g_launch_err; g_launch_err = nullptr; return fail(m); }
    return 0;
}

int enqueue_fast_detect(hak_ctx* c, const unsigned char* d_images, long image_stride, int pitch, int nimg,
                        hak_point* d_points, int* d_num_pts, int desc, int max_pts)
{
    const hak_config& cfg = c->cfg;
    const HakLayout& L = c->L;
    const hipStream_t st = c->stream;
    LevelArgs a = level_args(c, d_images, image_stride, pitch, nimg);
    c->last_fast = true;
    c->sync_stream = c->stream;
    hakf_launch_reset(st, c->state, nimg);
    for (int o = 0; o < L.noct; o++)
        for (int s = 0; s < L.ms; s++) {
            build_level<int>(a, o, s, st);
            hessian_level<int>(a, o, s, st);
        }
    hak_launch_nms_emit(st, a.b, L, c->dtab, c->psz, d_points, max_pts, d_num_pts, 1);
    hak_launch_clear_maps(st, a.b, L);
    hakf_launch_describe(st, a.b, L, c->dtab, d_points, max_pts, cfg.descriptor_pattern_size, cfg.upright, desc, c->htab.dsc_plan_ok);
    if (hipGetLastError() != hipSuccess) return fail("kernel launch failed");
    return 0;
}

static int run_detect_inner(hak_ctx* c, const float* d_images, long image_stride, int pitch, int nimg,
                            hak_point* d_points, int* d_num_pts, int desc, int max_pts, hak_point* h_pinned, int cap0, int cap1)
{
    const bool launch_bound = c->concurrent && c->L.noct > 1 && spine_pays(c, nimg);
    if (!c->use_graph || c->prof_on || (launch_bound && c->knobs.graph != 2))
        return enqueue_detect(c, d_images, image_stride, pitch, nimg, d_points, d_num_pts, desc, max_pts, h_pinned, cap0, cap1);
    hak_ctx::GraphKey key;
    memset(&key, 0, sizeof(key));
    key.img = d_images; key.stride = image_stride; key.pitch = pitch; key.nimg = nimg; key.pts = d_points;
    key.num = d_num_pts; key.desc = desc; key.max_pts = max_pts; key.conc = c->concurrent ? 1 : 0; key.st = c->stream; key.hpts = h_pinned; key.cap0 = cap0; key.cap1 = cap1;
    key.retain = (c->retain_best ? 1 : 0) | (c->retain_grid << 1);
    int slot = -1, victim = 0;
    for (int i = 0; i < hak_ctx::NGRAPH; i++) {
        if (c->graph_exec[i] && memcmp(&key, &c->gkey[i], sizeof(key)) == 0) slot = i;
        if (c->graph_age[i] < c->graph_age[victim]) victim = i;
    }
    if (slot >= 0) {
        c->graph_age[slot] = ++c->graph_clock;
        if (hipGraphLaunch(c->graph_exec[slot], c->stream) != hipSuccess) return fail("hipGraphLaunch");
        return 0;
    }
    slot = victim;
    if (c->graph_exec[slot]) { (void)hipGraphExecDestroy(c->graph_exec[slot]); c->graph_exec[slot] = nullptr; }
    hipGraph_t graph = nullptr;
    if (hipStreamBeginCapture(c->stream, hipStreamCaptureModeThreadLocal) != hipSuccess) {
        (void)hipGetLastError();
        c->use_graph = false;
        return enqueue_detect(c, d_images, image_stride, pitch, nimg, d_points, d_num_pts, desc, max_pts, h_pinned, cap0, cap1);
    }
    const int rc = enqueue_detect(c, d_images, image_stride, pitch, nimg, d_points, d_num_pts, desc, max_pts, h_pinned, cap0, cap1);
    const hipError_t e = hipStreamEndCapture(c->stream, &graph);
    if (rc) { if (graph) (void)hipGraphDestroy(graph); return rc; }
    if (e != hipSuccess || !graph) return fail(std::string("hipStreamEndCapture: ") + hipGetErrorString(e));
    const hipError_t ei = hipGraphInstantiate(&c->graph_exec[slot], graph, nullptr, nullptr, 0);
    (void)hipGraphDestroy(graph);
    if (ei != hipSuccess) { c->graph_exec[slot] = nullptr; return fail(std::string("hipGraphInstantiate: ") + hipGetErrorString(ei)); }
    c->gkey[slot] = key;
    c->graph_age[slot] = ++c->graph_clock;
    if (hipGraphLaunch(c->graph_exec[slot], c->stream) != hipSuccess) return fail("hipGraphLaunch");
    return 0;
}

int run_detect(hak_ctx* c, const float* d_images, long image_stride, int pitch, int nimg,
               hak_point* d_points, int* d_num_pts, int desc, int max_pts, hak_point* h_pinned, int cap0, int cap1)
{
    order_after_null_stream(c, c->stream);
    maps_guard_begin(c);
    return maps_guard_end(c, run_detect_inner(c, d_images, image_stride, pitch, nimg, d_points, d_num_pts, desc, max_pts, h_pinned, cap0, cap1));
}
```

### cuda-akaze_amd/csrc/hak_test_api.hip

```cpp
#include "hak_ctx.h"
#include "../../include/hipakaze_test.h"
#include <cmath>
#include <cstdio>
#include <cstring>

extern "C" int hak_debug_plane(hak_ctx* c, int img, int kind, int o, int s, float* h_dst)
{
    if (!c || img < 0 || img >= c->cfg.batch || o < 0 || o >= c->L.noct || s < 0 || s >= c->L.ms) return fail("bad plane");
    const HakLayout& L = c->L;
    const HakOct oc = L.oct[o];
    HIP_TRY(hipStreamSynchronize(c->stream));
    const float* arena = c->arena + (long)img * L.arena;
    if (kind == HAK_PLANE_LT) {
        HIP_TRY(hipMemcpy2D(h_dst, sizeof(float) * oc.w, arena + L.lt(o, s), sizeof(float) * oc.p, sizeof(float) * oc.w, oc.h, hipMemcpyDeviceToHost));
        return 0;
    }
    float* tmp = nullptr;
    HIP_TRY(hipMalloc((void**)&tmp, sizeof(float) * 2 * (size_t)oc.plane));
    int rc = 0;
    const float* src = tmp;
    if (kind == HAK_PLANE_DET) {
        const int step = c->plan[(size_t)o * L.ms + s].sigma_size;
        if (c->last_fast) hakf_launch_det(nullptr, reinterpret_cast<const int*>(arena + L.dxy(o, s)), reinterpret_cast<int*>(tmp), 0, oc.w, oc.h, oc.p, 1, step);
        else hak_launch_hessian(nullptr, arena + L.dxy(o, s), tmp, 0, oc.w, oc.h, oc.p, 1, step);
    } else {
        hak_launch_deinterleave(nullptr, arena + L.dxy(o, s), tmp, tmp + oc.plane, oc.w, oc.h, oc.p);
        if (kind == HAK_PLANE_LY) src = tmp + oc.plane;
    }
    if (hipDeviceSynchronize() != hipSuccess) rc = fail("debug plane kernel");
    if (!rc && hipMemcpy2D(h_dst, sizeof(float) * oc.w, src, sizeof(float) * oc.p, sizeof(float) * oc.w, oc.h, hipMemcpyDeviceToHost) != hipSuccess)
        rc = fail("debug plane copy");
    (void)hipFree(tmp);
    return rc;
}

extern "C" int hak_debug_kcontrast(hak_ctx* c, int img, float* kc)
{
    if (!c || img < 0 || img >= c->cfg.batch) return fail("bad image index");
    HakImgState s;
    HIP_TRY(hipStreamSynchronize(c->stream));
    HIP_TRY(hipMemcpy(&s, c->state + img, sizeof(s), hipMemcpyDeviceToHost));
    *kc = s.kcontrast[0];
    return 0;
}

extern "C" int hak_op_lowpass(const float* s, float* d, int w, int h, int p, float var, int radius)
{
    if (radius < 1 || radius > 5) return fail("radius must be 1..5");
    float taps[8];
    hak_gauss_taps(var, radius, taps);
    hak_launch_lowpass(nullptr, s, 0, p, d, 0, w, h, p, 1, taps, radius);
    HIP_TRY(hipDeviceSynchronize());
    return 0;
}

extern "C" int hak_op_down_smooth(const float* s, float* d, float* sm, int sw, int sh, int sp, int dw, int dh, int dp)
{
    float taps[8];
    hak_gauss_taps(1.f, 2, taps);
    HakOct so{sw, sh, sp, (long)sh * sp}, dd{dw, dh, dp, (long)dh * dp};
    hak_launch_down_smooth(nullptr, s, d, sm, 0, so, dd, 1, taps);
    HIP_TRY(hipDeviceSynchronize());
    return 0;
}

extern "C" int hak_op_kcontrast(const float* smooth, int w, int h, int p, float per, float* kc, float* hmax, int* hist)
{
    HakImgState* st = nullptr;
    HIP_TRY(hipMalloc((void**)&st, sizeof(HakImgState)));
    hak_launch_reset_state(nullptr, st, 1);
    hak_launch_contrast(nullptr, smooth, 0, w, h, p, 1, st, per, 1);
    HakImgState hs;
    HIP_TRY(hipMemcpy(&hs, st, sizeof(hs), hipMemcpyDeviceToHost));
    HIP_TRY(hipFree(st));
    if (kc) *kc = hs.kcontrast[0];
    if (hmax) memcpy(hmax, &hs.hmax_bits, 4);
    if (hist) { memcpy(hist, hs.hist, sizeof(hs.hist)); hist[0] += hak_hist_extra0(w, h); }
    return 0;
}

extern "C" int hak_op_flow(const float* s, float* d, int w, int h, int p, int diffusivity, float kcontrast)
{
    float ikc = 1.f / (kcontrast * kcontrast);
    hak_launch_flow(nullptr, s, d, 0, w, h, p, 1, diffusivity, nullptr, 0, ikc);
    HIP_TRY(hipDeviceSynchronize());
    return 0;
}

extern "C" int hak_op_rcp_check(unsigned lo_bits, unsigned hi_bits, unsigned long long* mismatches)
{
    if (!mismatches) return fail("null argument");
    unsigned long long* d = nullptr;
    HIP_TRY(hipMalloc((void**)&d, sizeof(unsigned long long)));
    HIP_TRY(hipMemset(d, 0, sizeof(unsigned long long)));
    int rc = hak_launch_rcp_check(lo_bits, hi_bits, d);
    if (!rc && hipDeviceSynchronize() != hipSuccess) rc = fail("rcp check kernel");
    if (!rc && hipMemcpy(mismatches, d, sizeof(unsigned long long), hipMemcpyDeviceToHost) != hipSuccess) rc = fail("rcp check download");
    (void)hipFree(d);
    return rc;
}

extern "C" int hak_op_smooth_flow(const float* s, float* sm, float* fl, int w, int h, int p, int diffusivity, float kcontrast)
{
    float taps[8];
    hak_gauss_taps(1.f, 2, taps);
    const float ikc = 1.f / (kcontrast * kcontrast);
    hak_launch_smooth_flow(nullptr, s, sm, fl, 0, w, h, p, 1, taps, diffusivity, nullptr, 0, ikc);
    HIP_TRY(hipDeviceSynchronize());
    return 0;
}

extern "C" int hak_op_nld_steps(const float* src, const float* flow, float* dst, float* tmp, int w, int h, int p,
                                const float* tau, int nsteps)
{
    if (nsteps < 1) return fail("nsteps < 1");
    if (p % 4) return fail("pitch must be a multiple of 4");
    const int G = hak_fed_groups(nsteps, hak_knobs_from_env().max_fuse, w);
    const float* s = src;
    int done = 0;
    for (int g = 0; g < G; g++) {
        const int ns = hak_fed_group_size(nsteps, G, g);
        float* d = ((G - g) % 2 == 1) ? dst : tmp;
        hak_launch_fed_group(nullptr, s, flow, d, 0, w, h, p, 1, tau + done, ns);
        done += ns;
        s = d;
    }
    HIP_TRY(hipDeviceSynchronize());
    return 0;
}

extern "C" int hak_op_hessian(const float* s, float* lx, float* ly, float* det, int w, int h, int p, int step)
{
    float* dxy = nullptr;
    HIP_TRY(hipMalloc((void**)&dxy, sizeof(float) * 2 * (size_t)h * p));
    hak_launch_hessian_level(nullptr, s, dxy, det, true, 0, w, h, p, 1, step, nullptr, nullptr, nullptr, 0, 0, 0.f);
    hak_launch_deinterleave(nullptr, dxy, lx, ly, w, h, p);
    const hipError_t e = hipDeviceSynchronize();
    (void)hipFree(dxy);
    if (e != hipSuccess) return fail(std::string("hak_op_hessian: ") + hipGetErrorString(e));
    return 0;
}

static HakBatch tail_batch(hak_ctx* c)
{
    HakBatch b{c->arena, c->L.arena, 1, c->state, c->maps, c->L.oct[0].plane, c->bitmap, c->rowcount, c->cand, c->cand_cap, &c->knobs};
    hak_batch_selection(c, b);
    return b;
}
static int tail_level_ok(hak_ctx* c, int o, int s, const void* h)
{
    if (!c || !h) return fail("null argument");
    if (o < 0 || o >= c->L.noct || s < 0 || s >= c->L.ms) return fail("bad level");
    return 0;
}

extern "C" int hak_debug_set_plane(hak_ctx* c, int img, int kind, int o, int s, const float* h_src)
{
    if (tail_level_ok(c, o, s, h_src)) return 1;
    if (img < 0 || img >= c->cfg.batch) return fail("bad image index");
    const HakLayout& L = c->L;
    const HakOct oc = L.oct[o];
    HIP_TRY(hipStreamSynchronize(c->stream));
    float* arena = c->arena + (long)img * L.arena;
    if (kind == HAK_PLANE_LT) {
        HIP_TRY(hipMemcpy2D(arena + L.lt(o, s), sizeof(float) * oc.p, h_src, sizeof(float) * oc.w, sizeof(float) * oc.w, oc.h, hipMemcpyHostToDevice));
        return 0;
    }
    if (kind != HAK_PLANE_LX && kind != HAK_PLANE_LY) return fail("only the Lt, Lx and Ly planes can be set");
    float* dst = arena + L.dxy(o, s) + (kind == HAK_PLANE_LY ? 1 : 0);
    for (int y = 0; y < oc.h; y++)
        HIP_TRY(hipMemcpy2D(dst + 2L * y * oc.p, 2 * sizeof(float), h_src + (long)y * oc.w, sizeof(float), sizeof(float), oc.w, hipMemcpyHostToDevice));
    return 0;
}

extern "C" int hak_op_tail_begin(hak_ctx* c)
{
    if (!c) return fail("null context");
    c->last_fast = false;
    c->sync_stream = c->stream;
    maps_guard_begin(c);
    hak_launch_reset_state(c->stream, c->state, 1);
    HIP_TRY(hipStreamSynchronize(c->stream));
    return 0;
}

extern "C" int hak_op_tail_level(hak_ctx* c, int o, int s, const float* h_src)
{
    if (tail_level_ok(c, o, s, h_src)) return 1;
    const HakLayout& L = c->L;
    const HakOct oc = L.oct[o];
    float* A = c->arena;
    float* smooth = A + L.smooth_off[o];
    HIP_TRY(hipMemcpy2D(smooth, sizeof(float) * oc.p, h_src, sizeof(float) * oc.w, sizeof(float) * oc.w, oc.h, hipMemcpyHostToDevice));
    HakBatch b = tail_batch(c);
    const int step = c->plan[(size_t)o * L.ms + s].sigma_size;
    if (!hak_launch_hessian_level(c->stream, smooth, A + L.dxy(o, s), A + L.flow_off[o], false, L.arena, oc.w, oc.h, oc.p, 1, step, &b, &L,
                                  &c->htab, o, s, c->cfg.dthreshold))
        hak_launch_extrema_level(c->stream, b, L, &c->htab, o, s, c->cfg.dthreshold, L.flow_off[o]);
    if (hipGetLastError() != hipSuccess) return fail("tail level launch failed");
    HIP_TRY(hipStreamSynchronize(c->stream));
    return 0;
}

extern "C" int hak_op_tail_det_level(hak_ctx* c, int o, int s, const float* h_det)
{
    if (tail_level_ok(c, o, s, h_det)) return 1;
    const HakLayout& L = c->L;
    const HakOct oc = L.oct[o];
    HIP_TRY(hipMemcpy2D(c->arena + L.flow_off[o], sizeof(float) * oc.p, h_det, sizeof(float) * oc.w, sizeof(float) * oc.w, oc.h,
                        hipMemcpyHostToDevice));
    hak_launch_extrema_level(c->stream, tail_batch(c), L, &c->htab, o, s, c->cfg.dthreshold, L.flow_off[o]);
    if (hipGetLastError() != hipSuccess) return fail("extrema launch failed");
    HIP_TRY(hipStreamSynchronize(c->stream));
    return 0;
}

extern "C" int hak_op_tail_seed(hak_ctx* c, const unsigned int* h_resp_bits, const int* h_layer)
{
    if (!c || !h_resp_bits || !h_layer) return fail("null argument");
    const size_t n = (size_t)c->L.oct[0].w * c->L.oct[0].h;
    unsigned* d_r = nullptr;
    int* d_l = nullptr;
    HIP_TRY(hipMalloc((void**)&d_r, sizeof(unsigned) * n));
    int rc = 0;
    if (hipMalloc((void**)&d_l, sizeof(int) * n) != hipSuccess) rc = fail("seed scratch");
    if (!rc && (hipMemcpy(d_r, h_resp_bits, sizeof(unsigned) * n, hipMemcpyHostToDevice) != hipSuccess ||
                hipMemcpy(d_l, h_layer, sizeof(int) * n, hipMemcpyHostToDevice) != hipSuccess)) rc = fail("seed upload");
    if (!rc) {
        hak_launch_seed_maps(c->stream, tail_batch(c), c->L, d_r, d_l);
        if (hipGetLastError() != hipSuccess || hipStreamSynchronize(c->stream) != hipSuccess) rc = fail("seed kernel");
    }
    (void)hipFree(d_r); (void)hipFree(d_l);
    return rc;
}

extern "C" int hak_op_tail_finish(hak_ctx* c, hak_point* d_points, int max_pts, int refine, int fast, int* num_pts)
{
    if (!c || !d_points || !num_pts || max_pts < 1) return fail("bad argument");
    hak_launch_nms_emit(c->stream, tail_batch(c), c->L, c->dtab, c->psz, d_points, max_pts, c->d_num, fast ? 1 : 0, refine ? 1 : 0);
    hak_launch_clear_maps(c->stream, tail_batch(c), c->L);
    int rc = hipGetLastError() != hipSuccess ? fail("tail finish launch failed") : 0;
    if (!rc && hipMemcpyAsync(c->h_num, c->d_num, sizeof(int), hipMemcpyDeviceToHost, c->stream) != hipSuccess) rc = fail("count download");
    if (!rc && hipStreamSynchronize(c->stream) != hipSuccess) rc = fail("sync");
    if (!rc) *num_pts = c->h_num[0];
    return maps_guard_end(c, rc);
}

extern "C" int hak_op_orient_describe(hak_ctx* c, hak_point* d_points, int n, int desc)
{
    if (!c || !d_points || n < 1) return fail("bad argument");
    HIP_TRY(hipMemcpy(&c->state[0].num_pts, &n, sizeof(int), hipMemcpyHostToDevice));
    hak_launch_describe(c->stream, tail_batch(c), c->L, c->dtab, d_points, n, c->cfg.descriptor_pattern_size, c->cfg.upright, desc ? 1 : 0,
                        c->htab.dsc_plan_ok, desc == 2 ? 0 : 1);
    if (hipGetLastError() != hipSuccess) return fail("describe launch failed");
    HIP_TRY(hipStreamSynchronize(c->stream));
    return 0;
}

extern "C" int hak_op_copy_probe(long bytes, int iters, double* gbytes_per_s)
{
    if (bytes < 16 || iters < 1 || !gbytes_per_s) return fail("bad probe argument");
    if (hak_device_count() == 0) return fail("no HIP device: libhipakaze has no CPU fallback");
    bytes &= ~15L;
    double ms = 0;
    if (hak_launch_copy_probe(bytes, iters, &ms) || ms <= 0) return fail("copy probe failed");
    *gbytes_per_s = 2.0 * (double)bytes / (ms * 1e-3) / 1e9;
    return 0;
}

extern "C" int hak_op_copy_probe_shapes(long bytes, int iters, double* gbytes_per_s, int n)
{
    if (bytes < 16 || iters < 1 || !gbytes_per_s || n < HAK_COPY_SHAPES) return fail("bad probe argument");
    if (hak_device_count() == 0) return fail("no HIP device: libhipakaze has no CPU fallback");
    bytes &= ~15L;
    double best = 0, ms[HAK_COPY_SHAPES] = {};
    if (hak_launch_copy_probe(bytes, iters, &best, ms)) return fail("copy probe failed");
    for (int i = 0; i < HAK_COPY_SHAPES; i++) {
        const double moved = i < HAK_COPY_SHAPES - 2 ? 2.0 * (double)bytes : (double)bytes;
        gbytes_per_s[i] = ms[i] > 0 ? moved / (ms[i] * 1e-3) / 1e9 : 0.0;
    }
    return HAK_COPY_SHAPES;
// ... 39 lines not shown
```

### cuda-akaze_amd/csrc/kernels_fed.hip

```cpp
#include "fed_common.h"

#ifndef HAK_FM_PD
#define HAK_FM_PD 3
#endif
#ifndef HAK_FM_PD_MAXNS
#define HAK_FM_PD_MAXNS 4
#endif

template <typename V, int NS>
struct FedState {
    using V4 = typename FedV<V>::V4;
    static constexpr int GS = 6;
    V4 Lw[NS][2];
    V4 Qw[NS][2];
    GHrow<V> GH[GS];
    V4 GV[GS];
    V4 gprev;
    static constexpr int PD = NS <= HAK_FM_PD_MAXNS ? HAK_FM_PD : 3;
    V4 Lq[PD], Gq[PD];
};

template <typename V, int NS, int U, bool YEDGE, bool XE>
__device__ __forceinline__ void fed_iter(FedState<V, NS>& S, const int t, const V* __restrict__ L,
                                         const V* __restrict__ G, V* __restrict__ D, const int p, const int xl,
                                         const int x0, const int w, const int h,
                                         const int ybeg, const int yend, const bool owns, const FedFacs<V, NS>& fac)
{
    using V4 = typename FedV<V>::V4;
    constexpr int GS = FedState<V, NS>::GS;
    {
        constexpr int PD = FedState<V, NS>::PD;
        const V4 g = S.Gq[pmod(U, PD)];
        S.Lw[0][pmod(U, 2)] = S.Lq[pmod(U, PD)];
        const long nrow = (long)min(t + PD, h - 1) * p + xl;
        S.Lq[pmod(U, PD)] = hak_load_stream(reinterpret_cast<const V4*>(L + nrow));
        S.Gq[pmod(U, PD)] = hak_load_stream(reinterpret_cast<const V4*>(G + nrow));
        const V gr = wave_shl1(g.x);
        S.GH[pmod(U, GS)] = GHrow<V>{vadd(g.x, g.y), vadd(g.y, g.z), vadd(g.z, g.w), vadd(g.w, gr)};
        S.GV[pmod(U - 1, GS)] = mk4(vadd(S.gprev.x, g.x), vadd(S.gprev.y, g.y), vadd(S.gprev.z, g.z), vadd(S.gprev.w, g.w));
        S.gprev = g;
    }
#pragma unroll
    for (int k = 1; k <= NS; k++) {
        const int rho = t - k;
        const V4 Lc = S.Lw[k - 1][pmod(U - k, 2)];
        V4 Qn = fed_q<V, V4>(S.GV[pmod(U - k, GS)], S.Lw[k - 1][pmod(U - k + 1, 2)], Lc);
        V4 Qp = S.Qw[k - 1][pmod(U - k - 1, 2)];
        if (YEDGE) {
            Qp = vsel4(rho == 0, vneg4(Qn), Qp);
            Qn = vsel4(rho == h - 1, vneg4(Qp), Qn);
        }
        S.Qw[k - 1][pmod(U - k, 2)] = Qn;
        const V4 out = fed_row<XE, V, V4>(Lc, S.GH[pmod(U - k, GS)], Qn, Qp, x0, w, fac.f[k - 1]);
        if (k < NS) {
            S.Lw[k < NS ? k : 0][pmod(U - k, 2)] = out;
        } else if (rho >= ybeg && rho < yend && owns) {
            hak_store_nt(reinterpret_cast<V4*>(D + (long)rho * p + x0), out);
        }
    }
}

template <typename V, int NS, bool XE>
__device__ __forceinline__ void fed_strip(const V* __restrict__ L, const V* __restrict__ G,
                                          V* __restrict__ D, int w, int h, int p, const FedFacs<V, NS>& fac,
                                          int x0, int ybeg, int yend, bool owns)
{
    using V4 = typename FedV<V>::V4;
    const int xl = min(max(x0, 0), p - 4);
    const int t0 = max(0, ybeg - NS);
    const int tend = min(yend - 1, h - 1) + NS;
    FedState<V, NS> S;
    const V z = 0;
#pragma unroll
    for (int k = 0; k < NS; k++) S.Lw[k][0] = S.Lw[k][1] = S.Qw[k][0] = S.Qw[k][1] = mk4(z, z, z, z);
#pragma unroll
    for (int i = 0; i < FedState<V, NS>::GS; i++) {
        S.GH[i] = GHrow<V>{z, z, z, z};
        S.GV[i] = mk4(z, z, z, z);
    }
    S.gprev = mk4(z, z, z, z);
#pragma unroll
    for (int i = 0; i < FedState<V, NS>::PD; i++) {
        const long row = (long)min(t0 + i, h - 1) * p + xl;
        S.Lq[i] = hak_load_stream(reinterpret_cast<const V4*>(L + row));
        S.Gq[i] = hak_load_stream(reinterpret_cast<const V4*>(G + row));
    }
    for (int tb = t0; tb <= tend; tb += 6) {
        if (tb <= NS || tb + 5 >= h) {
            fed_iter<V, NS, 0, true, XE>(S, tb + 0, L, G, D, p, xl, x0, w, h, ybeg, yend, owns, fac);
            fed_iter<V, NS, 1, true, XE>(S, tb + 1, L, G, D, p, xl, x0, w, h, ybeg, yend, owns, fac);
            fed_iter<V, NS, 2, true, XE>(S, tb + 2, L, G, D, p, xl, x0, w, h, ybeg, yend, owns, fac);
            fed_iter<V, NS, 3, true, XE>(S, tb + 3, L, G, D, p, xl, x0, w, h, ybeg, yend, owns, fac);
            fed_iter<V, NS, 4, true, XE>(S, tb + 4, L, G, D, p, xl, x0, w, h, ybeg, yend, owns, fac);
            fed_iter<V, NS, 5, true, XE>(S, tb + 5, L, G, D, p, xl, x0, w, h, ybeg, yend, owns, fac);
        } else {
            fed_iter<V, NS, 0, false, XE>(S, tb + 0, L, G, D, p, xl, x0, w, h, ybeg, yend, owns, fac);
            fed_iter<V, NS, 1, false, XE>(S, tb + 1, L, G, D, p, xl, x0, w, h, ybeg, yend, owns, fac);
            fed_iter<V, NS, 2, false, XE>(S, tb + 2, L, G, D, p, xl, x0, w, h, ybeg, yend, owns, fac);
            fed_iter<V, NS, 3, false, XE>(S, tb + 3, L, G, D, p, xl, x0, w, h, ybeg, yend, owns, fac);
            fed_iter<V, NS, 4, false, XE>(S, tb + 4, L, G, D, p, xl, x0, w, h, ybeg, yend, owns, fac);
            fed_iter<V, NS, 5, false, XE>(S, tb + 5, L, G, D, p, xl, x0, w, h, ybeg, yend, owns, fac);
        }
    }
}

template <typename V, int NS>
__global__ __launch_bounds__(256) void k_fed_multi(const V* __restrict__ src, const V* __restrict__ flow,
                                                   V* __restrict__ dst, long stride, int w, int h, int p,
                                                   FedFacs<V, NS> fac, int ry, int xv, int hx, int nbx, int nby, int nimg)
{
    int bx, by, img;
    if (!hak_xcd_decode(nbx, nby, nimg, bx, by, img)) return;
    const V* L = src + (long)img * stride;
    const V* G = flow + (long)img * stride;
    V* D = dst + (long)img * stride;
    const int lane = threadIdx.x & 63;
    const int wv = __builtin_amdgcn_readfirstlane(threadIdx.x >> 6);
    const int x0 = bx * xv - hx + 4 * lane;
    const int ybeg = (by * 4 + wv) * ry;
    if (ybeg >= h) return;
    const int yend = min(ybeg + ry, h);
    const bool owns = 4 * lane >= hx && 4 * lane < hx + xv && x0 < w && x0 >= 0;
    if (bx == 0 || (bx + 1) * xv + hx >= w) fed_strip<V, NS, true>(L, G, D, w, h, p, fac, x0, ybeg, yend, owns);
    else fed_strip<V, NS, false>(L, G, D, w, h, p, fac, x0, ybeg, yend, owns);
}

__global__ __launch_bounds__(256) void k_fed_generic(const float* __restrict__ src, const float* __restrict__ flow,
                                                     float* __restrict__ dst, long stride, int w, int h, int p,
                                                     float stepfac, int ry)
{
    const float* L = src + (long)blockIdx.z * stride;
    const float* G = flow + (long)blockIdx.z * stride;
    float* D = dst + (long)blockIdx.z * stride;
    const int lane = threadIdx.x & 63;
    const int wv = __builtin_amdgcn_readfirstlane(threadIdx.x >> 6);
    const int x0 = blockIdx.x * 248 - 4 + 4 * lane;
    const int ybeg = (blockIdx.y * 4 + wv) * ry;
    if (ybeg >= h) return;
    const int yend = min(ybeg + ry, h);
    const int xl = min(max(x0, 0), p - 4);
    const bool owns = lane >= 1 && lane < 63 && x0 < w && x0 >= 0;
    for (int y = ybeg; y < yend; y++) {
        const int yn = y == 0 ? 1 : y - 1, ys = y == h - 1 ? h - 2 : y + 1;
        const float4 Lc = *reinterpret_cast<const float4*>(L + (long)y * p + xl);
        const float4 Gc = *reinterpret_cast<const float4*>(G + (long)y * p + xl);
        const float4 Ln = *reinterpret_cast<const float4*>(L + (long)yn * p + xl);
        const float4 Gn = *reinterpret_cast<const float4*>(G + (long)yn * p + xl);
        const float4 Ls = *reinterpret_cast<const float4*>(L + (long)ys * p + xl);
        const float4 Gs = *reinterpret_cast<const float4*>(G + (long)ys * p + xl);
        const float Ll = wave_shr1(Lc.w), Lr = wave_shl1(Lc.x), Gl = wave_shr1(Gc.w), Gr = wave_shl1(Gc.x);
        const float l[6] = {Ll, Lc.x, Lc.y, Lc.z, Lc.w, Lr}, g[6] = {Gl, Gc.x, Gc.y, Gc.z, Gc.w, Gr};
        const float ln[4] = {Ln.x, Ln.y, Ln.z, Ln.w}, gn[4] = {Gn.x, Gn.y, Gn.z, Gn.w};
        const float ls[4] = {Ls.x, Ls.y, Ls.z, Ls.w}, gs[4] = {Gs.x, Gs.y, Gs.z, Gs.w};
        float o[4];
#pragma unroll
        for (int e = 0; e < 4; e++) {
            const int x = x0 + e;
            float LW = l[e], GW = g[e], LE = l[e + 2], GE = g[e + 2];
            if (x == 0) { LW = LE; GW = GE; }
            if (x == w - 1) { LE = l[e]; GE = g[e]; }
            const float Lx = l[e + 1], Gx = g[e + 1];
            const float step = (Gx + GE) * (LE - Lx) + (Gx + GW) * (LW - Lx) + (Gx + gs[e]) * (ls[e] - Lx) +
                               (Gx + gn[e]) * (ln[e] - Lx);
            o[e] = fmaf(stepfac, step, Lx);
        }
        if (owns) {
            float* drow = D + (long)y * p + x0;
            if (x0 + 3 < w) *reinterpret_cast<float4*>(drow) = make_float4(o[0], o[1], o[2], o[3]);
            else {
                if (x0 < w) drow[0] = o[0];
                if (x0 + 1 < w) drow[1] = o[1];
                if (x0 + 2 < w) drow[2] = o[2];
            }
        }
    }
}

template <typename V, int NS>
static void launch_multi(hipStream_t st, const V* src, const V* flow, V* dst, long stride,
                         int w, int h, int p, int nimg, const float* tau)
{
    FedFacs<V, NS> fac;
    for (int k = 0; k < NS; k++) {
        if constexpr (std::is_same<V, float>::value) fac.f[k] = 0.5f * tau[k];
        else fac.f[k] = (int)(0.5f * tau[k] * 65536 + 0.5f);
    }
    const int hx = 4;
    const int xv = 256 - 2 * hx;
    const int gx = (w + xv - 1) / xv;
    const int ry = hak_stream_rows(h, (long)gx * nimg, 8);
    const int gy = (h + 4 * ry - 1) / (4 * ry);
    k_fed_multi<V, NS><<<hak_xcd_grid(gx, gy, nimg), 256, 0, st>>>(src, flow, dst, stride, w, h, p, fac, ry, xv, hx, gx, gy, nimg);
}

int hak_fed_groups(int n, int max_fuse, int w)
{
    if (max_fuse < 1 || w % 4 != 0) max_fuse = 1;
    if (max_fuse > HAK_FED_MAX_FUSE) max_fuse = HAK_FED_MAX_FUSE;
    return (n + max_fuse - 1) / max_fuse;
}

int hak_fed_group_size(int n, int G, int g)
{
    int done = 0, ns = 0;
    for (int i = 0; i <= g; i++) { ns = (n - done + (G - i) - 1) / (G - i); done += ns; }
    return ns;
}

template <typename V>
static void launch_fed_group_t(hipStream_t st, const V* src, const V* flow, V* dst, long stride,
                               int w, int h, int p, int nimg, const float* tau, int ns)
{
    if (w % 4 != 0) {
        if constexpr (std::is_same<V, int>::value) hakf_launch_nld_step(st, src, flow, dst, stride, w, h, p, nimg, tau[0]);
        else {
            const int gx = (w + 247) / 248;
            int ry = 16;
            while (ry > 2 && (long)gx * ((h + ry - 1) / ry) * nimg < 2048) ry >>= 1;
            dim3 grid(gx, (h + 4 * ry - 1) / (4 * ry), nimg);
            k_fed_generic<<<grid, 256, 0, st>>>(src, flow, dst, stride, w, h, p, 0.5f * tau[0], ry);
        }
        return;
    }
    switch (ns) {
    case 1: launch_multi<V, 1>(st, src, flow, dst, stride, w, h, p, nimg, tau); break;
    case 2: launch_multi<V, 2>(st, src, flow, dst, stride, w, h, p, nimg, tau); break;
    case 3: launch_multi<V, 3>(st, src, flow, dst, stride, w, h, p, nimg, tau); break;
    default: launch_multi<V, 4>(st, src, flow, dst, stride, w, h, p, nimg, tau); break;
    }
}

void hak_launch_fed_group(hipStream_t st, const float* src, const float* flow, float* dst, long stride,
                          int w, int h, int p, int nimg, const float* tau, int ns)
{ launch_fed_group_t<float>(st, src, flow, dst, stride, w, h, p, nimg, tau, ns); }
void hak_launch_fed_group(hipStream_t st, const int* src, const int* flow, int* dst, long stride,
                          int w, int h, int p, int nimg, const float* tau, int ns)
{ launch_fed_group_t<int>(st, src, flow, dst, stride, w, h, p, nimg, tau, ns); }
```

### cuda-akaze_amd/csrc/kernels_fedsf.hip

```cpp
#include "fed_common.h"

#ifndef HAK_FS_PD
#define HAK_FS_PD 3
#endif
#ifndef HAK_FS_PD_MAXNS
#define HAK_FS_PD_MAXNS 4
#endif

namespace {

template <typename V, int NS>
struct FsState {
    using V4 = typename FedV<V>::V4;
    static constexpr int GS = 6;
    static constexpr int PD = NS <= HAK_FS_PD_MAXNS ? HAK_FS_PD : 3;
    V4 Lr[6];
    V4 Rp[6];
    V4 Sm[3];
    V SmL[3], SmR[3];
    V4 Lw[NS][2];
    V4 Qw[NS][2];
    GHrow<V> GH[GS];
    V4 GV[GS];
    V4 gprev;
    V4 Lq[PD];
};

template <bool DEC, typename V, typename V4>
__device__ __forceinline__ V4 fs_fetch(const V* __restrict__ L, const int row, const int lp, const int xl, const int sh)
{
    if constexpr (!DEC) return hak_load_stream(reinterpret_cast<const V4*>(L + (long)row * lp + xl));
    else {
        const V* r = L + (long)min(2 * row, sh - 1) * lp + min(2 * xl, lp - 8);
        const V4 a = hak_load_stream(reinterpret_cast<const V4*>(r)), b = hak_load_stream(reinterpret_cast<const V4*>(r + 4));
        return mk4(a.x, a.z, b.x, b.z);
    }
}

struct FsOut { __amdgpu_buffer_rsrc_t r; unsigned smo, go; };

template <typename V, int NS, int U, bool YEDGE, bool XE, bool WRITE_G, bool DEC, bool WRITE_SM>
__device__ __forceinline__ void fs_iter(FsState<V, NS>& S, const int t, const V* __restrict__ L, V* __restrict__ SMO,
                                        V* __restrict__ GO, V* __restrict__ D, const int p, const int xl,
                                        const int x0, const int w, const int h, const int ybeg, const int yend,
                                        const bool owns, const FedFacs<V, NS>& fac, const SfTaps<V> kk, const float ikc,
                                        const int lp, const int sh, const FsOut& O)
{
    using V4 = typename FedV<V>::V4;
    constexpr int GS = FsState<V, NS>::GS, PD = FsState<V, NS>::PD;
    const bool le = x0 == 0, re = x0 + 3 == w - 1;
    {
        const V4 Lc = S.Lq[pmod(U, PD)];
        S.Lr[pmod(U, 6)] = Lc;
        S.Lq[pmod(U, PD)] = fs_fetch<DEC, V, V4>(L, min(t + PD, h - 1), lp, xl, sh);
    }
    {
        const V4 c = S.Lr[pmod(U, 6)];
        const V sl1 = wave_shr1(c.w), sl2 = wave_shr1(c.z), sr1 = wave_shl1(c.x), sr2 = wave_shl1(c.y);
        V4 l1 = mk4(sl1, c.x, c.y, c.z), l2 = mk4(sl2, sl1, c.x, c.y);
        V4 r1 = mk4(c.y, c.z, c.w, sr1), r2 = mk4(c.z, c.w, sr1, sr2);
        if (XE) {
            l1.x = le ? c.y : l1.x;
            l2.x = le ? c.z : l2.x;
            l2.y = le ? c.y : l2.y;
            if constexpr (!DEC) {
                r1.w = re ? c.z : r1.w;
                r2.z = re ? c.z : r2.z;
                r2.w = re ? c.y : r2.w;
            } else {
                r1.w = re ? c.w : r1.w;
                r2.z = re ? c.w : r2.z;
                r2.w = re ? c.z : r2.w;
            }
        }
        V4 rp;
        rp.x = sf_conv(c.x, l1.x, r1.x, l2.x, r2.x, kk);
        rp.y = sf_conv(c.y, l1.y, r1.y, l2.y, r2.y, kk);
        rp.z = sf_conv(c.z, l1.z, r1.z, l2.z, r2.z, kk);
        rp.w = sf_conv(c.w, l1.w, r1.w, l2.w, r2.w, kk);
        S.Rp[pmod(U, 6)] = rp;
        if (YEDGE) {
            S.Rp[pmod(U - 2, 6)] = vsel4(t == 1, rp, S.Rp[pmod(U - 2, 6)]);
            S.Rp[pmod(U - 4, 6)] = vsel4(t == 2, rp, S.Rp[pmod(U - 4, 6)]);
            if constexpr (!DEC) {
                S.Rp[pmod(U, 6)] = vsel4(t == h, S.Rp[pmod(U - 2, 6)], S.Rp[pmod(U, 6)]);
                S.Rp[pmod(U, 6)] = vsel4(t == h + 1, S.Rp[pmod(U - 4, 6)], S.Rp[pmod(U, 6)]);
            } else {
                S.Rp[pmod(U, 6)] = vsel4(t == h, S.Rp[pmod(U - 1, 6)], S.Rp[pmod(U, 6)]);
                S.Rp[pmod(U, 6)] = vsel4(t == h + 1, S.Rp[pmod(U - 3, 6)], S.Rp[pmod(U, 6)]);
            }
        }
    }
    {
        const int a = t - 2;
        const V4 c = S.Rp[pmod(U - 2, 6)], u1 = S.Rp[pmod(U - 3, 6)], d1 = S.Rp[pmod(U - 1, 6)];
        const V4 u2 = S.Rp[pmod(U - 4, 6)], d2 = S.Rp[pmod(U, 6)];
        V4 sm;
        sm.x = sf_conv(c.x, u1.x, d1.x, u2.x, d2.x, kk);
        sm.y = sf_conv(c.y, u1.y, d1.y, u2.y, d2.y, kk);
        sm.z = sf_conv(c.z, u1.z, d1.z, u2.z, d2.z, kk);
        sm.w = sf_conv(c.w, u1.w, d1.w, u2.w, d2.w, kk);
        if constexpr (WRITE_SM)
            hak_buf_store_nt(O.r, O.smo + (a >= ybeg && a < yend ? (unsigned)(a * p) * (unsigned)sizeof(V) : HAK_BUF_OOB), sm);
        V sl = wave_shr1(sm.w), sr = wave_shl1(sm.x);
        if (XE) {
            sl = le ? sm.y : sl;
            sr = re ? sm.z : sr;
        }
        S.Sm[pmod(U, 3)] = sm; S.SmL[pmod(U, 3)] = sl; S.SmR[pmod(U, 3)] = sr;
        if (YEDGE && a == 1) { S.Sm[pmod(U - 2, 3)] = sm; S.SmL[pmod(U - 2, 3)] = sl; S.SmR[pmod(U - 2, 3)] = sr; }
        if (YEDGE && a == h) {
            S.Sm[pmod(U, 3)] = S.Sm[pmod(U - 2, 3)]; S.SmL[pmod(U, 3)] = S.SmL[pmod(U - 2, 3)]; S.SmR[pmod(U, 3)] = S.SmR[pmod(U - 2, 3)];
        }
    }
    const int tf = t - 3;
    {
        const V4 su = S.Sm[pmod(U - 2, 3)], sc = S.Sm[pmod(U - 1, 3)], sd = S.Sm[pmod(U, 3)];
        const V uL = S.SmL[pmod(U - 2, 3)], uR = S.SmR[pmod(U - 2, 3)];
        const V cL = S.SmL[pmod(U - 1, 3)], cR = S.SmR[pmod(U - 1, 3)];
        const V dL = S.SmL[pmod(U, 3)], dR = S.SmR[pmod(U, 3)];
        V4 g;
        float4 den;
#define FS_G(k, ul, uc, ur, cl, cr, ll, lc, lr)                                             \
        {                                                                                   \
            const V dx = 10 * ((cr) - (cl)) + 3 * ((ur) + (lr) - (ul) - (ll));              \
            const V dy = 10 * ((lc) - (uc)) + 3 * ((ll) + (lr) - (ul) - (ur));              \
            den.k = 1.f + sf_dif2(dx, dy, ikc);                                             \
        }
        FS_G(x, uL, su.x, su.y, cL, sc.y, dL, sd.x, sd.y)
        FS_G(y, su.x, su.y, su.z, sc.x, sc.z, sd.x, sd.y, sd.z)
        FS_G(z, su.y, su.z, su.w, sc.y, sc.w, sd.y, sd.z, sd.w)
        FS_G(w, su.z, su.w, uR, sc.z, cR, sd.z, sd.w, dR)
#undef FS_G
        const bool fast = den.x < 0x1p64f && den.y < 0x1p64f && den.z < 0x1p64f && den.w < 0x1p64f;
        if (__ballot(!fast) == 0ull) {
            g = mk4(sf_g_as<V>(hak_rcp_newton(den.x)), sf_g_as<V>(hak_rcp_newton(den.y)), sf_g_as<V>(hak_rcp_newton(den.z)),
                    sf_g_as<V>(hak_rcp_newton(den.w)));
        } else {
            g = mk4(sf_g_as<V>(1.f / den.x), sf_g_as<V>(1.f / den.y), sf_g_as<V>(1.f / den.z), sf_g_as<V>(1.f / den.w));
        }
        if (WRITE_G) hak_buf_store_nt(O.r, O.go + (tf >= ybeg && tf < yend ? (unsigned)(tf * p) * (unsigned)sizeof(V) : HAK_BUF_OOB), g);
        const V gr = wave_shl1(g.x);
        S.GH[pmod(U, GS)] = GHrow<V>{vadd(g.x, g.y), vadd(g.y, g.z), vadd(g.z, g.w), vadd(g.w, gr)};
        S.GV[pmod(U - 1, GS)] = mk4(vadd(S.gprev.x, g.x), vadd(S.gprev.y, g.y), vadd(S.gprev.z, g.z), vadd(S.gprev.w, g.w));
        S.gprev = g;
    }
#pragma unroll
    for (int k = 1; k <= NS; k++) {
        const int rho = tf - k;
        const V4 Lc = k == 1 ? S.Lr[pmod(U - 3 - 1, 6)] : S.Lw[k - 1][pmod(U - k, 2)];
        const V4 Ls = k == 1 ? S.Lr[pmod(U - 3, 6)] : S.Lw[k - 1][pmod(U - k + 1, 2)];
        V4 Qn = fed_q<V, V4>(S.GV[pmod(U - k, GS)], Ls, Lc);
        V4 Qp = S.Qw[k - 1][pmod(U - k - 1, 2)];
        if (YEDGE) {
            Qp = vsel4(rho == 0, vneg4(Qn), Qp);
            Qn = vsel4(rho == h - 1, vneg4(Qp), Qn);
        }
        S.Qw[k - 1][pmod(U - k, 2)] = Qn;
        const V4 out = fed_row<XE, V, V4>(Lc, S.GH[pmod(U - k, GS)], Qn, Qp, x0, w, fac.f[k - 1]);
        if (k < NS) {
            S.Lw[k < NS ? k : 0][pmod(U - k, 2)] = out;
        } else if (rho >= ybeg && rho < yend && owns) {
            hak_store_nt(reinterpret_cast<V4*>(D + (long)rho * p + x0), out);
        }
    }
}

template <typename V, int NS, bool XE, bool WRITE_G, bool DEC, bool WRITE_SM>
__device__ __forceinline__ void fs_strip(const V* __restrict__ L, V* __restrict__ SMO, V* __restrict__ GO,
                                         V* __restrict__ D, int w, int h, int p, const FedFacs<V, NS>& fac,
                                         const SfTaps<V> kk, const float ikc, int x0, int ybeg, int yend, bool owns,
                                         const int lp, const int sh)
{
    using V4 = typename FedV<V>::V4;
    const int xl = min(max(x0, 0), p - 4);
    FsOut O;
    {
        V* lo = SMO ? SMO : GO;
        if (WRITE_G && SMO) lo = GO < lo ? GO : lo;
        O.r = hak_buf_rsrc(lo);
        const unsigned xb = (unsigned)x0 * (unsigned)sizeof(V);
        O.smo = owns && SMO ? xb + (unsigned)((SMO - lo) * (long)sizeof(V)) : HAK_BUF_OOB;
        O.go = WRITE_G && owns ? xb + (unsigned)((GO - lo) * (long)sizeof(V)) : HAK_BUF_OOB;
    }
    const int t0 = max(0, ybeg - NS - 4);
    const int tend = min(yend - 1, h - 1) + NS + 3;
    FsState<V, NS> S;
    const V z = 0;
    const V4 z4 = mk4(z, z, z, z);
#pragma unroll
    for (int i = 0; i < 6; i++) { S.Lr[i] = z4; S.Rp[i] = z4; }
#pragma unroll
    for (int i = 0; i < 3; i++) { S.Sm[i] = z4; S.SmL[i] = z; S.SmR[i] = z; }
#pragma unroll
    for (int k = 0; k < NS; k++) S.Lw[k][0] = S.Lw[k][1] = S.Qw[k][0] = S.Qw[k][1] = z4;
#pragma unroll
    for (int i = 0; i < FsState<V, NS>::GS; i++) {
        S.GH[i] = GHrow<V>{z, z, z, z};
        S.GV[i] = z4;
    }
    S.gprev = z4;
#pragma unroll
    for (int i = 0; i < FsState<V, NS>::PD; i++)
        S.Lq[i] = fs_fetch<DEC, V, V4>(L, min(t0 + i, h - 1), lp, xl, sh);
    for (int tb = t0; tb <= tend; tb += 6) {
        if (tb <= NS + 4 || tb + 5 >= h) {
            fs_iter<V, NS, 0, true, XE, WRITE_G, DEC, WRITE_SM>(S, tb + 0, L, SMO, GO, D, p, xl, x0, w, h, ybeg, yend, owns, fac, kk, ikc, lp, sh, O);
            fs_iter<V, NS, 1, true, XE, WRITE_G, DEC, WRITE_SM>(S, tb + 1, L, SMO, GO, D, p, xl, x0, w, h, ybeg, yend, owns, fac, kk, ikc, lp, sh, O);
            fs_iter<V, NS, 2, true, XE, WRITE_G, DEC, WRITE_SM>(S, tb + 2, L, SMO, GO, D, p, xl, x0, w, h, ybeg, yend, owns, fac, kk, ikc, lp, sh, O);
            fs_iter<V, NS, 3, true, XE, WRITE_G, DEC, WRITE_SM>(S, tb + 3, L, SMO, GO, D, p, xl, x0, w, h, ybeg, yend, owns, fac, kk, ikc, lp, sh, O);
            fs_iter<V, NS, 4, true, XE, WRITE_G, DEC, WRITE_SM>(S, tb + 4, L, SMO, GO, D, p, xl, x0, w, h, ybeg, yend, owns, fac, kk, ikc, lp, sh, O);
            fs_iter<V, NS, 5, true, XE, WRITE_G, DEC, WRITE_SM>(S, tb + 5, L, SMO, GO, D, p, xl, x0, w, h, ybeg, yend, owns, fac, kk, ikc, lp, sh, O);
        } else {
            fs_iter<V, NS, 0, false, XE, WRITE_G, DEC, WRITE_SM>(S, tb + 0, L, SMO, GO, D, p, xl, x0, w, h, ybeg, yend, owns, fac, kk, ikc, lp, sh, O);
            fs_iter<V, NS, 1, false, XE, WRITE_G, DEC, WRITE_SM>(S, tb + 1, L, SMO, GO, D, p, xl, x0, w, h, ybeg, yend, owns, fac, kk, ikc, lp, sh, O);
            fs_iter<V, NS, 2, false, XE, WRITE_G, DEC, WRITE_SM>(S, tb + 2, L, SMO, GO, D, p, xl, x0, w, h, ybeg, yend, owns, fac, kk, ikc, lp, sh, O);
            fs_iter<V, NS, 3, false, XE, WRITE_G, DEC, WRITE_SM>(S, tb + 3, L, SMO, GO, D, p, xl, x0, w, h, ybeg, yend, owns, fac, kk, ikc, lp, sh, O);
            fs_iter<V, NS, 4, false, XE, WRITE_G, DEC, WRITE_SM>(S, tb + 4, L, SMO, GO, D, p, xl, x0, w, h, ybeg, yend, owns, fac, kk, ikc, lp, sh, O);
            fs_iter<V, NS, 5, false, XE, WRITE_G, DEC, WRITE_SM>(S, tb + 5, L, SMO, GO, D, p, xl, x0, w, h, ybeg, yend, owns, fac, kk, ikc, lp, sh, O);
        }
    }
}

constexpr int FS_HX = 8;
constexpr int FS_XV = 256 - 2 * FS_HX;

template <typename V, int NS, bool WRITE_G, bool DEC, bool WRITE_SM>
__global__ __launch_bounds__(256) void k_fed_sf(const V* __restrict__ src, V* __restrict__ smooth, V* __restrict__ flow,
                                                V* __restrict__ dst, long stride, int w, int h, int p,
                                                FedFacs<V, NS> fac, SfTaps<V> kk, const HakImgState* __restrict__ state, int octave,
                                                float fixed_ikc, int ry, int nbx, int nby, int nimg, int lp, int sh)
{
    int bx, by, img;
    if (!hak_xcd_decode(nbx, nby, nimg, bx, by, img)) return;
    const V* L = src + (long)img * stride;
    V* SMO = smooth ? smooth + (long)img * stride : nullptr;
    V* GO = flow + (long)img * stride;
    V* D = dst + (long)img * stride;
    const float ikc = state ? state[img].ikc[octave] : fixed_ikc;
    const int lane = threadIdx.x & 63;
    const int wv = __builtin_amdgcn_readfirstlane(threadIdx.x >> 6);
    const int x0 = bx * FS_XV - FS_HX + 4 * lane;
    const int ybeg = (by * 4 + wv) * ry;
    if (ybeg >= h) return;
    const int yend = min(ybeg + ry, h);
    const bool owns = 4 * lane >= FS_HX && 4 * lane < FS_HX + FS_XV && x0 < w && x0 >= 0;
    if (bx == 0 || (bx + 1) * FS_XV + FS_HX >= w) fs_strip<V, NS, true, WRITE_G, DEC, WRITE_SM>(L, SMO, GO, D, w, h, p, fac, kk, ikc, x0, ybeg, yend, owns, lp, sh);
    else fs_strip<V, NS, false, WRITE_G, DEC, WRITE_SM>(L, SMO, GO, D, w, h, p, fac, kk, ikc, x0, ybeg, yend, owns, lp, sh);
}

template <typename V, int NS>
void launch_fs(hipStream_t st, const V* src, V* smooth, V* flow, V* dst, long stride, int w, int h, int p,
               int nimg, SfTaps<V> kk, const float* tau, const HakImgState* state, int octave, float fixed_ikc, bool write_g,
               int sp = 0, int sh = 0)
{
    FedFacs<V, NS> fac;
    for (int k = 0; k < NS; k++) {
        if constexpr (std::is_same<V, float>::value) fac.f[k] = 0.5f * tau[k];
        else fac.f[k] = (int)(0.5f * tau[k] * 65536 + 0.5f);
    }
    const int gx = (w + FS_XV - 1) / FS_XV;
    const int ry = hak_stream_rows(h, (long)gx * nimg, 8);
    const int gy = (h + 4 * ry - 1) / (4 * ry);
    const unsigned grid = hak_xcd_grid(gx, gy, nimg);
    if (!smooth) {
        if constexpr (std::is_same<V, float>::value) {
            if (write_g) k_fed_sf<V, NS, true, false, false><<<grid, 256, 0, st>>>(src, smooth, flow, dst, stride, w, h, p, fac, kk, state, octave, fixed_ikc, ry, gx, gy, nimg, p, h);
            else k_fed_sf<V, NS, false, false, false><<<grid, 256, 0, st>>>(src, smooth, flow, dst, stride, w, h, p, fac, kk, state, octave, fixed_ikc, ry, gx, gy, nimg, p, h);
        }
    } else if (sp > 0) {
        if (write_g) k_fed_sf<V, NS, true, true, true><<<grid, 256, 0, st>>>(src, smooth, flow, dst, stride, w, h, p, fac, kk, state, octave, fixed_ikc, ry, gx, gy, nimg, sp, sh);
        else k_fed_sf<V, NS, false, true, true><<<grid, 256, 0, st>>>(src, smooth, flow, dst, stride, w, h, p, fac, kk, state, octave, fixed_ikc, ry, gx, gy, nimg, sp, sh);
    } else {
        if (write_g) k_fed_sf<V, NS, true, false, true><<<grid, 256, 0, st>>>(src, smooth, flow, dst, stride, w, h, p, fac, kk, state, octave, fixed_ikc, ry, gx, gy, nimg, p, h);
        else k_fed_sf<V, NS, false, false, true><<<grid, 256, 0, st>>>(src, smooth, flow, dst, stride, w, h, p, fac, kk, state, octave, fixed_ikc, ry, gx, gy, nimg, p, h);
    }
}

template <typename V>
bool launch_fs_any(hipStream_t st, const V* src, V* smooth, V* flow, V* dst, long stride, int w, int h, int p, int nimg,
                   SfTaps<V> kk, int diffusivity, const float* tau, int ns, const HakImgState* state, int octave, float fixed_ikc,
                   bool write_g, int sp = 0, int sh = 0)
{
    if (diffusivity != HAK_PM_G2 || (w & 3) || w < 16 || h < 8 || ns < 1 || ns > 4) return false;
    if (!smooth && (sp > 0 || !std::is_same<V, float>::value)) return false;
    if ((write_g && smooth ? (flow < smooth ? smooth - flow : flow - smooth) : 0L) + (long)h * p >= (long)HAK_BUF_OOB / (long)sizeof(V)) return false;
    switch (ns) {
    case 1: launch_fs<V, 1>(st, src, smooth, flow, dst, stride, w, h, p, nimg, kk, tau, state, octave, fixed_ikc, write_g, sp, sh); break;
    case 2: launch_fs<V, 2>(st, src, smooth, flow, dst, stride, w, h, p, nimg, kk, tau, state, octave, fixed_ikc, write_g, sp, sh); break;
    case 3: launch_fs<V, 3>(st, src, smooth, flow, dst, stride, w, h, p, nimg, kk, tau, state, octave, fixed_ikc, write_g, sp, sh); break;
    default: launch_fs<V, 4>(st, src, smooth, flow, dst, stride, w, h, p, nimg, kk, tau, state, octave, fixed_ikc, write_g, sp, sh); break;
    }
    return true;
}

__global__ __launch_bounds__(256) void k_rcp_check(unsigned lo, unsigned hi, unsigned long long* bad)
{
    unsigned long long n = 0;
    for (unsigned long long b = lo + blockIdx.x * (unsigned long long)blockDim.x + threadIdx.x; b < hi;
         b += (unsigned long long)gridDim.x * blockDim.x) {
        const float d = __uint_as_float((unsigned)b);
        n += __float_as_uint(hak_rcp_newton(d)) != __float_as_uint(1.0f / d);
    }
    if (n) atomicAdd(bad, n);
}

template <typename V>
bool launch_fed_sf_head_t(hipStream_t st, const V* src, HakOct so, V* smooth, V* flow, V* dst, long stride, HakOct dd, int nimg,
                          const V* taps, int diffusivity, const float* tau, int ns, const HakImgState* state, int octave, bool write_g)
{
    if ((so.w & 1) || (so.h & 1) || so.p < 2 * 8 || dd.w != so.w / 2 || dd.h != so.h / 2) return false;
    return launch_fs_any<V>(st, src, smooth, flow, dst, stride, dd.w, dd.h, dd.p, nimg, SfTaps<V>{taps[0], taps[1], taps[2]},
                            diffusivity, tau, ns, state, octave, 0.f, write_g, so.p, so.h);
}

}

int hak_launch_rcp_check(unsigned lo, unsigned hi, unsigned long long* d_bad)
{
    k_rcp_check<<<4096, 256>>>(lo, hi, d_bad);
    return hipGetLastError() == hipSuccess ? 0 : 1;
}

bool hak_launch_fed_sf(hipStream_t st, const float* src, float* smooth, float* flow, float* dst, long stride,
                       int w, int h, int p, int nimg, const float* taps, int diffusivity, const float* tau, int ns,
                       const HakImgState* state, int octave, bool write_g, bool store_smooth, float fixed_ikc)
{ return launch_fs_any<float>(st, src, store_smooth ? smooth : nullptr, flow, dst, stride, w, h, p, nimg, SfTaps<float>{taps[0], taps[1], taps[2]},
                                diffusivity, tau, ns, state, octave, fixed_ikc, write_g); }
bool hak_launch_fed_sf(hipStream_t st, const int* src, int* smooth, int* flow, int* dst, long stride,
                       int w, int h, int p, int nimg, const int* taps, int diffusivity, const float* tau, int ns,
                       const HakImgState* state, int octave, bool write_g)
{ return launch_fs_any<int>(st, src, smooth, flow, dst, stride, w, h, p, nimg, SfTaps<int>{taps[0], taps[1], taps[2]},
                              diffusivity, tau, ns, state, octave, 0.f, write_g); }

bool hak_launch_fed_sf_head(hipStream_t st, const float* src, HakOct so, float* smooth, float* flow, float* dst, long stride,
                            HakOct dd, int nimg, const float* taps, int diffusivity, const float* tau, int ns,
                            const HakImgState* state, int octave, bool write_g)
{ return launch_fed_sf_head_t<float>(st, src, so, smooth, flow, dst, stride, dd, nimg, taps, diffusivity, tau, ns, state, octave, write_g); }
bool hak_launch_fed_sf_head(hipStream_t st, const int* src, HakOct so, int* smooth, int* flow, int* dst, long stride,
                            HakOct dd, int nimg, const int* taps, int diffusivity, const float* tau, int ns,
                            const HakImgState* state, int octave, bool write_g)
{ return launch_fed_sf_head_t<int>(st, src, so, smooth, flow, dst, stride, dd, nimg, taps, diffusivity, tau, ns, state, octave, write_g); }
```

Measured before the change: 6167 pairs/s.

## Fuse up to eight FED steps per pass using two-pixel lanes for deep fusion

Raises the FED step-fusion limit from 4 to 8 for the float path. Fused kernels with more than 4 steps have each lane own 2 pixels instead of 4, with wider halos and longer unrolls, so register pressure stays bounded. The aim is fewer passes over the image pyramid, which cuts global-memory round trips and kernel launches. In exchange, halos grow and redundant compute rises at the strip edges, and the larger per-thread state may lower occupancy.

```diff
diff --git a/cuda-akaze_amd/akaze_hip/__init__.py b/cuda-akaze_amd/akaze_hip/__init__.py
--- a/cuda-akaze_amd/akaze_hip/__init__.py
+++ b/cuda-akaze_amd/akaze_hip/__init__.py
@@ -109,6 +109,9 @@
     "hak_op_kcontrast": (C.c_int, [_vp, C.c_int, C.c_int, C.c_int, C.c_float, _fp, _fp, _ip]),
     "hak_op_flow": (C.c_int, [_vp, _vp, C.c_int, C.c_int, C.c_int, C.c_int, C.c_float]),
     "hak_op_nld_steps": (C.c_int, [_vp, _vp, _vp, _vp, C.c_int, C.c_int, C.c_int, _fp, C.c_int]),
+    "hak_op_nld_steps_batch": (C.c_int, [_vp, _vp, _vp, _vp, C.c_long, C.c_int, C.c_int, C.c_int, C.c_int, _fp, C.c_int]),
+    "hak_op_fed_cycle": (C.c_int, [_vp, C.c_int, C.c_int, C.c_int, C.c_int, _vp, _vp, _vp, _vp, C.c_long, C.c_int, C.c_int, C.c_int, C.c_int,
+                                   _fp, _fp, C.c_int]),
     "hak_op_rcp_check": (C.c_int, [C.c_uint, C.c_uint, C.POINTER(C.c_ulonglong)]),
     "hak_op_smooth_flow": (C.c_int, [_vp, _vp, _vp, C.c_int, C.c_int, C.c_int, C.c_int, C.c_float]),
     "hak_op_hessian": (C.c_int, [_vp, _vp, _vp, _vp, C.c_int, C.c_int, C.c_int, C.c_int]),
diff --git a/cuda-akaze_amd/csrc/fed_common.h b/cuda-akaze_amd/csrc/fed_common.h
--- a/cuda-akaze_amd/csrc/fed_common.h
+++ b/cuda-akaze_amd/csrc/fed_common.h
@@ -1,6 +1,7 @@
 #pragma once
 #include "hak_internal.h"
 #include <type_traits>
+#include <utility>
 
 template <typename V> struct FedV;
 template <> struct FedV<float> { using V4 = float4; };
@@ -87,37 +88,117 @@
 
 constexpr int pmod(int a, int m) { return ((a % m) + m) % m; }
 
-template <typename V> struct GHrow { V h1, h2, h3, h4; };
 __device__ __forceinline__ float vneg(float a) { return -a; }
 __device__ __forceinline__ int vneg(int a) { return (int)(0u - (unsigned)a); }
 
-template <bool XEDGE, typename V, typename V4>
-__device__ __forceinline__ V4 fed_row(const V4 Lc, const GHrow<V>& gh, const V4 Qn, const V4 Qp, int x0, int w, V stepfac)
-{
-    const V Lr = wave_shl1(Lc.x);
-    const V d1 = vsub(Lc.y, Lc.x), d2 = vsub(Lc.z, Lc.y), d3 = vsub(Lc.w, Lc.z), d4 = vsub(Lr, Lc.w);
-    const V P1 = vmul(gh.h1, d1), P2 = vmul(gh.h2, d2), P3 = vmul(gh.h3, d3);
-    V P4 = vmul(gh.h4, d4);
-    if (XEDGE) P4 = x0 + 3 == w - 1 ? vneg(P3) : P4;
-    V P0 = wave_shr1(P4);
-    if (XEDGE) P0 = x0 == 0 ? vneg(P1) : P0;
-    V4 o;
-    o.x = vstep(stepfac, vsub(vadd(vsub(P1, P0), Qn.x), Qp.x), Lc.x);
-    o.y = vstep(stepfac, vsub(vadd(vsub(P2, P1), Qn.y), Qp.y), Lc.y);
-    o.z = vstep(stepfac, vsub(vadd(vsub(P3, P2), Qn.z), Qp.z), Lc.z);
-    o.w = vstep(stepfac, vsub(vadd(vsub(P4, P3), Qn.w), Qp.w), Lc.w);
+template <typename V, int W> struct alignas(sizeof(V) * W) FedPx { V e[W]; };
+template <typename V, int W> __device__ __forceinline__ FedPx<V, W> px_fill(const V a)
+{
+    FedPx<V, W> r;
+#pragma unroll
+    for (int j = 0; j < W; j++) r.e[j] = a;
+    return r;
+}
+template <typename V, int W> __device__ __forceinline__ FedPx<V, W> px_add(const FedPx<V, W>& a, const FedPx<V, W>& b)
+{
+    FedPx<V, W> r;
+#pragma unroll
+    for (int j = 0; j < W; j++) r.e[j] = vadd(a.e[j], b.e[j]);
+    return r;
+}
+template <typename V, int W> __device__ __forceinline__ FedPx<V, W> px_neg(const FedPx<V, W>& a)
+{
+    FedPx<V, W> r;
+#pragma unroll
+    for (int j = 0; j < W; j++) r.e[j] = vneg(a.e[j]);
+    return r;
+}
+template <typename V, int W> __device__ __forceinline__ FedPx<V, W> px_sel(const bool c, const FedPx<V, W>& a, const FedPx<V, W>& b)
+{
+    FedPx<V, W> r;
+#pragma unroll
+    for (int j = 0; j < W; j++) r.e[j] = c ? a.e[j] : b.e[j];
+    return r;
+}
+template <typename V, int W> __device__ __forceinline__ FedPx<V, W> px_load(const V* p)
+{
+    typedef V vec __attribute__((ext_vector_type(W)));
+#ifdef HAK_NT_LOADS
+    const vec t = __builtin_nontemporal_load(reinterpret_cast<const vec*>(p));
+#else
+    const vec t = *reinterpret_cast<const vec*>(p);
+#endif
+    FedPx<V, W> r;
+#pragma unroll
+    for (int j = 0; j < W; j++) r.e[j] = t[j];
+    return r;
+}
+template <typename V, int W> __device__ __forceinline__ void px_store_nt(V* p, const FedPx<V, W>& v)
+{
+    typedef V vec __attribute__((ext_vector_type(W)));
+    vec t;
+#pragma unroll
+    for (int j = 0; j < W; j++) t[j] = v.e[j];
+    __builtin_nontemporal_store(t, reinterpret_cast<vec*>(p));
+}
+__device__ __forceinline__ unsigned px_bits(float a) { return __float_as_uint(a); }
+__device__ __forceinline__ unsigned px_bits(int a) { return (unsigned)a; }
+template <typename V, int W> __device__ __forceinline__ void px_buf_store_nt(__amdgpu_buffer_rsrc_t r, unsigned voff, const FedPx<V, W>& v)
+{
+    if constexpr (W == 4) {
+        const hak_v4u d = {px_bits(v.e[0]), px_bits(v.e[1]), px_bits(v.e[2]), px_bits(v.e[3])};
+        __builtin_amdgcn_raw_buffer_store_b128(d, r, voff, 0, 2);
+    } else {
+        static_assert(W == 2, "a lane owns 4 or 2 pixels");
+        typedef unsigned v2u __attribute__((ext_vector_type(2)));
+        const v2u d = {px_bits(v.e[0]), px_bits(v.e[1])};
+        __builtin_amdgcn_raw_buffer_store_b64(d, r, voff, 0, 2);
+    }
+}
+
+template <typename V, int W> struct GHrow { V h[W]; };
+template <typename V, int W> __device__ __forceinline__ GHrow<V, W> fed_gh(const FedPx<V, W>& g)
+{
+    const V gr = wave_shl1(g.e[0]);
+    GHrow<V, W> r;
+#pragma unroll
+    for (int j = 0; j < W; j++) r.h[j] = vadd(g.e[j], j + 1 < W ? g.e[(j + 1) % W] : gr);
+    return r;
+}
+
+template <bool XEDGE, typename V, int W>
+__device__ __forceinline__ FedPx<V, W> fed_row(const FedPx<V, W>& Lc, const GHrow<V, W>& gh, const FedPx<V, W>& Qn, const FedPx<V, W>& Qp,
+                                               int x0, int w, V stepfac)
+{
+    const V Lr = wave_shl1(Lc.e[0]);
+    V P[W + 1];
+#pragma unroll
+    for (int j = 1; j <= W; j++) P[j] = vmul(gh.h[j - 1], vsub(j < W ? Lc.e[j % W] : Lr, Lc.e[j - 1]));
+    if (XEDGE) P[W] = x0 + W - 1 == w - 1 ? vneg(P[W - 1]) : P[W];
+    P[0] = wave_shr1(P[W]);
+    if (XEDGE) P[0] = x0 == 0 ? vneg(P[1]) : P[0];
+    FedPx<V, W> o;
+#pragma unroll
+    for (int j = 0; j < W; j++) o.e[j] = vstep(stepfac, vsub(vadd(vsub(P[j + 1], P[j]), Qn.e[j]), Qp.e[j]), Lc.e[j]);
     return o;
 }
-template <typename V, typename V4>
-__device__ __forceinline__ V4 fed_q(const V4 gv, const V4 Ln, const V4 Lc)
-{
-    return mk4(vmul(gv.x, vsub(Ln.x, Lc.x)), vmul(gv.y, vsub(Ln.y, Lc.y)), vmul(gv.z, vsub(Ln.z, Lc.z)), vmul(gv.w, vsub(Ln.w, Lc.w)));
-}
-template <typename V4> __device__ __forceinline__ V4 vneg4(const V4 a) { return mk4(vneg(a.x), vneg(a.y), vneg(a.z), vneg(a.w)); }
+template <typename V, int W>
+__device__ __forceinline__ FedPx<V, W> fed_q(const FedPx<V, W>& gv, const FedPx<V, W>& Ln, const FedPx<V, W>& Lc)
+{
+    FedPx<V, W> r;
+#pragma unroll
+    for (int j = 0; j < W; j++) r.e[j] = vmul(gv.e[j], vsub(Ln.e[j], Lc.e[j]));
+    return r;
+}
 template <typename V4> __device__ __forceinline__ V4 vsel4(const bool c, const V4 a, const V4 b)
 {
     return mk4(c ? a.x : b.x, c ? a.y : b.y, c ? a.z : b.z, c ? a.w : b.w);
 }
+
+constexpr int HAK_FED_WIDE_STEPS = 4;
+constexpr int fed_lane_px(int ns) { return ns <= HAK_FED_WIDE_STEPS ? 4 : 2; }
+constexpr int fed_gsum_slots(int ns) { return ns + 1 <= 6 ? 6 : 9; }
+constexpr int fed_unroll(int ns) { return ns + 1 <= 6 ? 6 : 18; }
 
 
 template <typename V> struct SfTaps { V k0, k1, k2; };
diff --git a/cuda-akaze_amd/csrc/hak_api.hip b/cuda-akaze_amd/csrc/hak_api.hip
--- a/cuda-akaze_amd/csrc/hak_api.hip
+++ b/cuda-akaze_amd/csrc/hak_api.hip
@@ -895,7 +895,7 @@
         for (int s = 0; s < L.ms; s++) {
             const LevelPlan& lp = c->plan[(size_t)o * L.ms + s];
             pxsteps += N * lp.nsteps;
-            launches += lp.nsteps ? hak_fed_groups(lp.nsteps, c->knobs.max_fuse, L.oct[o].w) : 0;
+            launches += lp.nsteps ? hak_fed_groups(lp.nsteps, c->knobs.max_fuse, L.oct[o].w, hak_fed_wide_only(o, L.oct[o].w)) : 0;
             if (s > 0 && hak_fed_sf_covers(c->knobs, c->cfg.diffusivity, L.oct[o], c->cfg.batch)) folded += 16.0 * N;
             if (s == 0 && o > 0 && hak_fed_sf_covers(c->knobs, c->cfg.diffusivity, L.oct[o], c->cfg.batch, &L.oct[o - 1]))
                 folded += 4.0 * L.oct[o - 1].w * L.oct[o - 1].h + 16.0 * N;
diff --git a/cuda-akaze_amd/csrc/hak_internal.h b/cuda-akaze_amd/csrc/hak_internal.h
--- a/cuda-akaze_amd/csrc/hak_internal.h
+++ b/cuda-akaze_amd/csrc/hak_internal.h
@@ -411,7 +411,8 @@
 bool hak_launch_fed_sf(hipStream_t st, const int* src, int* smooth, int* flow, int* dst, long stride,
                        int w, int h, int p, int nimg, const int* taps, int diffusivity, const float* tau, int ns,
                        const HakImgState* state, int octave, bool write_g);
-int hak_fed_groups(int n, int max_fuse, int w);
+int hak_fed_groups(int n, int max_fuse, int w, bool wide_only);
+bool hak_fed_wide_only(int octave, int w);
 int hak_fed_group_size(int n, int G, int g);
 void hak_launch_fed_group(hipStream_t st, const float* src, const float* flow, float* dst, long stride,
                           int w, int h, int p, int nimg, const float* tau, int ns);
diff --git a/cuda-akaze_amd/csrc/hak_knobs.h b/cuda-akaze_amd/csrc/hak_knobs.h
--- a/cuda-akaze_amd/csrc/hak_knobs.h
+++ b/cuda-akaze_amd/csrc/hak_knobs.h
@@ -1,7 +1,7 @@
 #pragma once
 #include "../../include/hipakaze.h"
 
-#define HAK_FED_MAX_FUSE 4
+#define HAK_FED_MAX_FUSE 8
 
 struct HakKnobs {
     int hess_stream = 1;
@@ -18,7 +18,7 @@
     int level_min_blocks = 96;
     int fuse_sf = 1;
     int fuse_head = 1;
-    int max_fuse = 4;
+    int max_fuse = 8;
     int hist_min_blocks = 256;
     int hist_rpb_max = 8;
     int hess_side = 0;
diff --git a/cuda-akaze_amd/csrc/hak_sequence.hip b/cuda-akaze_amd/csrc/hak_sequence.hip
--- a/cuda-akaze_amd/csrc/hak_sequence.hip
+++ b/cuda-akaze_amd/csrc/hak_sequence.hip
@@ -117,7 +117,7 @@
         count_fed(nl, (s == 0 ? 1.0 * L.oct[o - 1].w * L.oct[o - 1].h : 4.0 * oc.w * oc.h) + 8.0 * oc.w * oc.h + (nl - 1) * 12.0 * oc.w * oc.h);
         return;
     }
-    const int G = hak_fed_groups(n, kn.max_fuse, oc.w);
+    const int G = hak_fed_groups(n, is_fast<V> && kn.max_fuse > 4 ? 4 : kn.max_fuse, oc.w, hak_fed_wide_only(o, oc.w));
     const int ns0 = hak_fed_group_size(n, G, 0);
     V* dst0 = (G % 2 == 1) ? Lt : tmp;
     const V* fsrc;
@@ -256,7 +256,7 @@
                      !hak_stream_pays(c->knobs.hess_stream, L.oct[0].w, L.oct[0].h, nimg) && !level_tile_pays(c, L.oct[0], nimg) &&
                      !hak_stream_pays(c->knobs.fuse_sf, L.oct[0].w, L.oct[0].h, nimg);
         for (int s = 1; s < L.ms && side0; s++)
-            side0 = hak_fed_groups(c->plan[s].nsteps, c->knobs.max_fuse, L.oct[0].w) == 1 && c->plan[s].sigma_size <= 4;
+            side0 = hak_fed_groups(c->plan[s].nsteps, c->knobs.max_fuse, L.oct[0].w, true) == 1 && c->plan[s].sigma_size <= 4;
         hipStream_t st = main_st;
         for (int o = 0; o < L.noct; o++) {
             if (c->concurrent && o > 0) {
diff --git a/cuda-akaze_amd/csrc/hak_test_api.hip b/cuda-akaze_amd/csrc/hak_test_api.hip
--- a/cuda-akaze_amd/csrc/hak_test_api.hip
+++ b/cuda-akaze_amd/csrc/hak_test_api.hip
@@ -115,7 +115,7 @@
 {
     if (nsteps < 1) return fail("nsteps < 1");
     if (p % 4) return fail("pitch must be a multiple of 4");
-    const int G = hak_fed_groups(nsteps, hak_knobs_from_env().max_fuse, w);
+    const int G = hak_fed_groups(nsteps, hak_knobs_from_env().max_fuse, w, false);
     const float* s = src;
     int done = 0;
     for (int g = 0; g < G; g++) {
@@ -127,6 +127,66 @@
     }
     HIP_TRY(hipDeviceSynchronize());
     return 0;
+}
+
+extern "C" int hak_op_nld_steps_batch(const float* src, const float* flow, float* dst, float* tmp, long stride, int w, int h, int p,
+                                      int nimg, const float* tau, int nsteps)
+{
+    if (nsteps < 1 || nimg < 1) return fail("nsteps < 1 or nimg < 1");
+    if (p % 4 || stride % 4) return fail("pitch and stride must be multiples of 4");
+    const int G = hak_fed_groups(nsteps, hak_knobs_from_env().max_fuse, w, false);
+    const float* s = src;
+    int done = 0;
+    for (int g = 0; g < G; g++) {
+        const int ns = hak_fed_group_size(nsteps, G, g);
+        float* d = ((G - g) % 2 == 1) ? dst : tmp;
+        hak_launch_fed_group(nullptr, s, flow, d, stride, w, h, p, nimg, tau + done, ns);
+        done += ns;
+        s = d;
+    }
+    HIP_TRY(hipDeviceSynchronize());
+    return 0;
+}
+
+extern "C" int hak_op_fed_cycle(const float* src, int head, int sw, int sh, int sp, float* smooth, float* flow, float* dst, float* tmp,
+                                long stride, int w, int h, int p, int nimg, const float* kcontrast, const float* tau, int nsteps)
+{
+    if (nsteps < 1 || nimg < 1 || !kcontrast) return fail("nsteps < 1, nimg < 1 or no contrast factors");
+    if (p % 4 || stride % 4) return fail("pitch and stride must be multiples of 4");
+    std::vector<HakImgState> hs((size_t)nimg);
+    for (int i = 0; i < nimg; i++) {
+        hs[i] = HakImgState{};
+        hs[i].kcontrast[0] = kcontrast[i];
+        hs[i].ikc[0] = 1.f / (kcontrast[i] * kcontrast[i]);
+    }
+    HakImgState* state = nullptr;
+    HIP_TRY(hipMalloc((void**)&state, sizeof(HakImgState) * (size_t)nimg));
+    int rc = 0;
+    if (hipMemcpy(state, hs.data(), sizeof(HakImgState) * (size_t)nimg, hipMemcpyHostToDevice) != hipSuccess) rc = fail("state upload");
+    float taps[8];
+    hak_gauss_taps(1.f, 2, taps);
+    const int G = hak_fed_groups(nsteps, hak_knobs_from_env().max_fuse, w, false);
+    const int ns0 = hak_fed_group_size(nsteps, G, 0);
+    float* dst0 = (G % 2 == 1) ? dst : tmp;
+    if (!rc) {
+        const bool ok = head ? hak_launch_fed_sf_head(nullptr, src, HakOct{sw, sh, sp, (long)sh * sp}, smooth, flow, dst0, stride,
+                                                      HakOct{w, h, p, (long)h * p}, nimg, taps, HAK_PM_G2, tau, ns0, state, 0, G > 1)
+                             : hak_launch_fed_sf(nullptr, src, smooth, flow, dst0, stride, w, h, p, nimg, taps, HAK_PM_G2, tau, ns0, state, 0,
+                                                 G > 1);
+        if (!ok) rc = fail("hak_op_fed_cycle: k_fed_sf does not cover this case");
+    }
+    const float* s = dst0;
+    int done = ns0;
+    for (int g = 1; g < G && !rc; g++) {
+        const int ns = hak_fed_group_size(nsteps, G, g);
+        float* d = ((G - g) % 2 == 1) ? dst : tmp;
+        hak_launch_fed_group(nullptr, s, flow, d, stride, w, h, p, nimg, tau + done, ns);
+        done += ns;
+        s = d;
+    }
+    if (hipDeviceSynchronize() != hipSuccess && !rc) rc = fail("hak_op_fed_cycle: kernel");
+    (void)hipFree(state);
+    return rc;
 }
 
 extern "C" int hak_op_hessian(const float* s, float* lx, float* ly, float* det, int w, int h, int p, int step)
diff --git a/cuda-akaze_amd/csrc/kernels_fed.hip b/cuda-akaze_amd/csrc/kernels_fed.hip
--- a/cuda-akaze_amd/csrc/kernels_fed.hip
+++ b/cuda-akaze_amd/csrc/kernels_fed.hip
@@ -9,15 +9,17 @@
 
 template <typename V, int NS>
 struct FedState {
-    using V4 = typename FedV<V>::V4;
-    static constexpr int GS = 6;
-    V4 Lw[NS][2];
-    V4 Qw[NS][2];
-    GHrow<V> GH[GS];
-    V4 GV[GS];
-    V4 gprev;
+    static constexpr int W = fed_lane_px(NS);
+    using Px = FedPx<V, W>;
+    static constexpr int GS = fed_gsum_slots(NS);
+    static constexpr int UF = fed_unroll(NS);
+    Px Lw[NS][2];
+    Px Qw[NS][2];
+    GHrow<V, W> GH[GS];
+    Px GV[GS];
+    Px gprev;
     static constexpr int PD = NS <= HAK_FM_PD_MAXNS ? HAK_FM_PD : 3;
-    V4 Lq[PD], Gq[PD];
+    Px Lq[PD], Gq[PD];
 };
 
 template <typename V, int NS, int U, bool YEDGE, bool XE>
@@ -26,38 +28,45 @@
                                          const int x0, const int w, const int h,
                                          const int ybeg, const int yend, const bool owns, const FedFacs<V, NS>& fac)
 {
-    using V4 = typename FedV<V>::V4;
-    constexpr int GS = FedState<V, NS>::GS;
+    constexpr int W = FedState<V, NS>::W, GS = FedState<V, NS>::GS;
+    using Px = FedPx<V, W>;
     {
         constexpr int PD = FedState<V, NS>::PD;
-        const V4 g = S.Gq[pmod(U, PD)];
+        const Px g = S.Gq[pmod(U, PD)];
         S.Lw[0][pmod(U, 2)] = S.Lq[pmod(U, PD)];
         const long nrow = (long)min(t + PD, h - 1) * p + xl;
-        S.Lq[pmod(U, PD)] = hak_load_stream(reinterpret_cast<const V4*>(L + nrow));
-        S.Gq[pmod(U, PD)] = hak_load_stream(reinterpret_cast<const V4*>(G + nrow));
-        const V gr = wave_shl1(g.x);
-        S.GH[pmod(U, GS)] = GHrow<V>{vadd(g.x, g.y), vadd(g.y, g.z), vadd(g.z, g.w), vadd(g.w, gr)};
-        S.GV[pmod(U - 1, GS)] = mk4(vadd(S.gprev.x, g.x), vadd(S.gprev.y, g.y), vadd(S.gprev.z, g.z), vadd(S.gprev.w, g.w));
+        S.Lq[pmod(U, PD)] = px_load<V, W>(L + nrow);
+        S.Gq[pmod(U, PD)] = px_load<V, W>(G + nrow);
+        S.GH[pmod(U, GS)] = fed_gh(g);
+        S.GV[pmod(U - 1, GS)] = px_add(S.gprev, g);
         S.gprev = g;
     }
 #pragma unroll
     for (int k = 1; k <= NS; k++) {
         const int rho = t - k;
-        const V4 Lc = S.Lw[k - 1][pmod(U - k, 2)];
-        V4 Qn = fed_q<V, V4>(S.GV[pmod(U - k, GS)], S.Lw[k - 1][pmod(U - k + 1, 2)], Lc);
-        V4 Qp = S.Qw[k - 1][pmod(U - k - 1, 2)];
+        const Px Lc = S.Lw[k - 1][pmod(U - k, 2)];
+        Px Qn = fed_q(S.GV[pmod(U - k, GS)], S.Lw[k - 1][pmod(U - k + 1, 2)], Lc);
+        Px Qp = S.Qw[k - 1][pmod(U - k - 1, 2)];
         if (YEDGE) {
-            Qp = vsel4(rho == 0, vneg4(Qn), Qp);
-            Qn = vsel4(rho == h - 1, vneg4(Qp), Qn);
+            Qp = px_sel(rho == 0, px_neg(Qn), Qp);
+            Qn = px_sel(rho == h - 1, px_neg(Qp), Qn);
         }
         S.Qw[k - 1][pmod(U - k, 2)] = Qn;
-        const V4 out = fed_row<XE, V, V4>(Lc, S.GH[pmod(U - k, GS)], Qn, Qp, x0, w, fac.f[k - 1]);
+        const Px out = fed_row<XE>(Lc, S.GH[pmod(U - k, GS)], Qn, Qp, x0, w, fac.f[k - 1]);
         if (k < NS) {
             S.Lw[k < NS ? k : 0][pmod(U - k, 2)] = out;
         } else if (rho >= ybeg && rho < yend && owns) {
-            hak_store_nt(reinterpret_cast<V4*>(D + (long)rho * p + x0), out);
-        }
-    }
+            px_store_nt(D + (long)rho * p + x0, out);
+        }
+    }
+}
+template <typename V, int NS, bool YEDGE, bool XE, int... U>
+__device__ __forceinline__ void fed_body(std::integer_sequence<int, U...>, FedState<V, NS>& S, const int tb, const V* __restrict__ L,
+                                         const V* __restrict__ G, V* __restrict__ D, const int p, const int xl, const int x0,
+                                         const int w, const int h, const int ybeg, const int yend, const bool owns,
+                                         const FedFacs<V, NS>& fac)
+{
+    (fed_iter<V, NS, U, YEDGE, XE>(S, tb + U, L, G, D, p, xl, x0, w, h, ybeg, yend, owns, fac), ...);
 }
 
 template <typename V, int NS, bool XE>
@@ -65,50 +74,45 @@
                                           V* __restrict__ D, int w, int h, int p, const FedFacs<V, NS>& fac,
                                           int x0, int ybeg, int yend, bool owns)
 {
-    using V4 = typename FedV<V>::V4;
-    const int xl = min(max(x0, 0), p - 4);
+    using St = FedState<V, NS>;
+    constexpr int W = St::W, UF = St::UF;
+    const int xl = min(max(x0, 0), p - W);
     const int t0 = max(0, ybeg - NS);
     const int tend = min(yend - 1, h - 1) + NS;
-    FedState<V, NS> S;
-    const V z = 0;
-#pragma unroll
-    for (int k = 0; k < NS; k++) S.Lw[k][0] = S.Lw[k][1] = S.Qw[k][0] = S.Qw[k][1] = mk4(z, z, z, z);
-#pragma unroll
-    for (int i = 0; i < FedState<V, NS>::GS; i++) {
-        S.GH[i] = GHrow<V>{z, z, z, z};
-        S.GV[i] = mk4(z, z, z, z);
-    }
-    S.gprev = mk4(z, z, z, z);
-#pragma unroll
-    for (int i = 0; i < FedState<V, NS>::PD; i++) {
+    St S;
+    const FedPx<V, W> z = px_fill<V, W>(0);
+#pragma unroll
+    for (int k = 0; k < NS; k++) S.Lw[k][0] = S.Lw[k][1] = S.Qw[k][0] = S.Qw[k][1] = z;
+#pragma unroll
+    for (int i = 0; i < St::GS; i++) {
+#pragma unroll
+        for (int j = 0; j < W; j++) S.GH[i].h[j] = 0;
+        S.GV[i] = z;
+    }
+    S.gprev = z;
+#pragma unroll
+    for (int i = 0; i < St::PD; i++) {
         const long row = (long)min(t0 + i, h - 1) * p + xl;
-        S.Lq[i] = hak_load_stream(reinterpret_cast<const V4*>(L + row));
-        S.Gq[i] = hak_load_stream(reinterpret_cast<const V4*>(G + row));
-    }
-    for (int tb = t0; tb <= tend; tb += 6) {
-        if (tb <= NS || tb + 5 >= h) {
-            fed_iter<V, NS, 0, true, XE>(S, tb + 0, L, G, D, p, xl, x0, w, h, ybeg, yend, owns, fac);
-            fed_iter<V, NS, 1, true, XE>(S, tb + 1, L, G, D, p, xl, x0, w, h, ybeg, yend, owns, fac);
-            fed_iter<V, NS, 2, true, XE>(S, tb + 2, L, G, D, p, xl, x0, w, h, ybeg, yend, owns, fac);
-            fed_iter<V, NS, 3, true, XE>(S, tb + 3, L, G, D, p, xl, x0, w, h, ybeg, yend, owns, fac);
-            fed_iter<V, NS, 4, true, XE>(S, tb + 4, L, G, D, p, xl, x0, w, h, ybeg, yend, owns, fac);
-            fed_iter<V, NS, 5, true, XE>(S, tb + 5, L, G, D, p, xl, x0, w, h, ybeg, yend, owns, fac);
-        } else {
-            fed_iter<V, NS, 0, false, XE>(S, tb + 0, L, G, D, p, xl, x0, w, h, ybeg, yend, owns, fac);
-            fed_iter<V, NS, 1, false, XE>(S, tb + 1, L, G, D, p, xl, x0, w, h, ybeg, yend, owns, fac);
-            fed_iter<V, NS, 2, false, XE>(S, tb + 2, L, G, D, p, xl, x0, w, h, ybeg, yend, owns, fac);
-            fed_iter<V, NS, 3, false, XE>(S, tb + 3, L, G, D, p, xl, x0, w, h, ybeg, yend, owns, fac);
-            fed_iter<V, NS, 4, false, XE>(S, tb + 4, L, G, D, p, xl, x0, w, h, ybeg, yend, owns, fac);
-            fed_iter<V, NS, 5, false, XE>(S, tb + 5, L, G, D, p, xl, x0, w, h, ybeg, yend, owns, fac);
-        }
-    }
-}
+        S.Lq[i] = px_load<V, W>(L + row);
+        S.Gq[i] = px_load<V, W>(G + row);
+    }
+    for (int tb = t0; tb <= tend; tb += UF) {
+        if (tb <= NS || tb + UF - 1 >= h)
+            fed_body<V, NS, true, XE>(std::make_integer_sequence<int, UF>{}, S, tb, L, G, D, p, xl, x0, w, h, ybeg, yend, owns, fac);
+        else
+            fed_body<V, NS, false, XE>(std::make_integer_sequence<int, UF>{}, S, tb, L, G, D, p, xl, x0, w, h, ybeg, yend, owns, fac);
+    }
+}
+
+constexpr int fed_hx(int ns) { return (ns + 3) & ~3; }
+constexpr int fed_xv(int ns) { return 64 * fed_lane_px(ns) - 2 * fed_hx(ns); }
 
 template <typename V, int NS>
 __global__ __launch_bounds__(256) void k_fed_multi(const V* __restrict__ src, const V* __restrict__ flow,
                                                    V* __restrict__ dst, long stride, int w, int h, int p,
-                                                   FedFacs<V, NS> fac, int ry, int xv, int hx, int nbx, int nby, int nimg)
-{
+                                                   FedFacs<V, NS> fac, int ry, int nbx, int nby, int nimg)
+{
+    constexpr int W = fed_lane_px(NS), hx = fed_hx(NS), xv = fed_xv(NS);
     int bx, by, img;
     if (!hak_xcd_decode(nbx, nby, nimg, bx, by, img)) return;
     const V* L = src + (long)img * stride;
@@ -116,11 +120,11 @@
     V* D = dst + (long)img * stride;
     const int lane = threadIdx.x & 63;
     const int wv = __builtin_amdgcn_readfirstlane(threadIdx.x >> 6);
-    const int x0 = bx * xv - hx + 4 * lane;
+    const int x0 = bx * xv - hx + W * lane;
     const int ybeg = (by * 4 + wv) * ry;
     if (ybeg >= h) return;
     const int yend = min(ybeg + ry, h);
-    const bool owns = 4 * lane >= hx && 4 * lane < hx + xv && x0 < w && x0 >= 0;
+    const bool owns = W * lane >= hx && W * lane < hx + xv && x0 < w && x0 >= 0;
     if (bx == 0 || (bx + 1) * xv + hx >= w) fed_strip<V, NS, true>(L, G, D, w, h, p, fac, x0, ybeg, yend, owns);
     else fed_strip<V, NS, false>(L, G, D, w, h, p, fac, x0, ybeg, yend, owns);
 }
@@ -185,19 +189,25 @@
         if constexpr (std::is_same<V, float>::value) fac.f[k] = 0.5f * tau[k];
         else fac.f[k] = (int)(0.5f * tau[k] * 65536 + 0.5f);
     }
-    const int hx = 4;
-    const int xv = 256 - 2 * hx;
+    constexpr int xv = fed_xv(NS);
     const int gx = (w + xv - 1) / xv;
     const int ry = hak_stream_rows(h, (long)gx * nimg, 8);
     const int gy = (h + 4 * ry - 1) / (4 * ry);
-    k_fed_multi<V, NS><<<hak_xcd_grid(gx, gy, nimg), 256, 0, st>>>(src, flow, dst, stride, w, h, p, fac, ry, xv, hx, gx, gy, nimg);
-}
-
-int hak_fed_groups(int n, int max_fuse, int w)
+    k_fed_multi<V, NS><<<hak_xcd_grid(gx, gy, nimg), 256, 0, st>>>(src, flow, dst, stride, w, h, p, fac, ry, gx, gy, nimg);
+}
+
+int hak_fed_groups(int n, int max_fuse, int w, bool wide_only)
 {
     if (max_fuse < 1 || w % 4 != 0) max_fuse = 1;
     if (max_fuse > HAK_FED_MAX_FUSE) max_fuse = HAK_FED_MAX_FUSE;
-    return (n + max_fuse - 1) / max_fuse;
+    const int wide = max_fuse < HAK_FED_WIDE_STEPS ? max_fuse : HAK_FED_WIDE_STEPS;
+    const int Gw = (n + wide - 1) / wide, Gd = (n + max_fuse - 1) / max_fuse;
+    return !wide_only && Gd < Gw ? Gd : Gw;
+}
+bool hak_fed_wide_only(int octave, int w)
+{
+    const int strips = (w + fed_xv(HAK_FED_MAX_FUSE) - 1) / fed_xv(HAK_FED_MAX_FUSE);
+    return octave == 0 || 4L * w < 3L * strips * 64 * fed_lane_px(HAK_FED_MAX_FUSE);
 }
 
 int hak_fed_group_size(int n, int G, int g)
@@ -226,7 +236,17 @@
     case 1: launch_multi<V, 1>(st, src, flow, dst, stride, w, h, p, nimg, tau); break;
     case 2: launch_multi<V, 2>(st, src, flow, dst, stride, w, h, p, nimg, tau); break;
     case 3: launch_multi<V, 3>(st, src, flow, dst, stride, w, h, p, nimg, tau); break;
-    default: launch_multi<V, 4>(st, src, flow, dst, stride, w, h, p, nimg, tau); break;
+    case 4: launch_multi<V, 4>(st, src, flow, dst, stride, w, h, p, nimg, tau); break;
+    default:
+        if constexpr (std::is_same<V, float>::value) {
+            switch (ns) {
+            case 5: launch_multi<V, 5>(st, src, flow, dst, stride, w, h, p, nimg, tau); break;
+            case 6: launch_multi<V, 6>(st, src, flow, dst, stride, w, h, p, nimg, tau); break;
+            case 7: launch_multi<V, 7>(st, src, flow, dst, stride, w, h, p, nimg, tau); break;
+            default: launch_multi<V, 8>(st, src, flow, dst, stride, w, h, p, nimg, tau); break;
+            }
+        } else launch_multi<V, 4>(st, src, flow, dst, stride, w, h, p, nimg, tau);
+        break;
     }
 }
 
diff --git a/cuda-akaze_amd/csrc/kernels_fedsf.hip b/cuda-akaze_amd/csrc/kernels_fedsf.hip
--- a/cuda-akaze_amd/csrc/kernels_fedsf.hip
+++ b/cuda-akaze_amd/csrc/kernels_fedsf.hip
@@ -11,101 +11,103 @@
 
 template <typename V, int NS>
 struct FsState {
-    using V4 = typename FedV<V>::V4;
-    static constexpr int GS = 6;
+    static constexpr int W = fed_lane_px(NS);
+    using Px = FedPx<V, W>;
+    static constexpr int GS = fed_gsum_slots(NS);
+    static constexpr int UF = fed_unroll(NS);
     static constexpr int PD = NS <= HAK_FS_PD_MAXNS ? HAK_FS_PD : 3;
-    V4 Lr[6];
-    V4 Rp[6];
-    V4 Sm[3];
+    Px Lr[6];
+    Px Rp[6];
+    Px Sm[3];
     V SmL[3], SmR[3];
-    V4 Lw[NS][2];
-    V4 Qw[NS][2];
-    GHrow<V> GH[GS];
-    V4 GV[GS];
-    V4 gprev;
-    V4 Lq[PD];
+    Px Lw[NS][2];
+    Px Qw[NS][2];
+    GHrow<V, W> GH[GS];
+    Px GV[GS];
+    Px gprev;
+    Px Lq[PD];
 };
 
-template <bool DEC, typename V, typename V4>
-__device__ __forceinline__ V4 fs_fetch(const V* __restrict__ L, const int row, const int lp, const int xl, const int sh)
-{
-    if constexpr (!DEC) return hak_load_stream(reinterpret_cast<const V4*>(L + (long)row * lp + xl));
+template <bool DEC, typename V, int W>
+__device__ __forceinline__ FedPx<V, W> fs_fetch(const V* __restrict__ L, const int row, const int lp, const int xl, const int sh)
+{
+    if constexpr (!DEC) return px_load<V, W>(L + (long)row * lp + xl);
     else {
-        const V* r = L + (long)min(2 * row, sh - 1) * lp + min(2 * xl, lp - 8);
-        const V4 a = hak_load_stream(reinterpret_cast<const V4*>(r)), b = hak_load_stream(reinterpret_cast<const V4*>(r + 4));
-        return mk4(a.x, a.z, b.x, b.z);
+        const V* r = L + (long)min(2 * row, sh - 1) * lp + min(2 * xl, lp - 2 * W);
+        FedPx<V, W> o;
+#pragma unroll
+        for (int i = 0; i < W / 2; i++) {
+            const FedPx<V, 4> a = px_load<V, 4>(r + 4 * i);
+            o.e[2 * i] = a.e[0];
+            o.e[2 * i + 1] = a.e[2];
+        }
+        return o;
     }
 }
 
 struct FsOut { __amdgpu_buffer_rsrc_t r; unsigned smo, go; };
 
 template <typename V, int NS, int U, bool YEDGE, bool XE, bool WRITE_G, bool DEC, bool WRITE_SM>
-__device__ __forceinline__ void fs_iter(FsState<V, NS>& S, const int t, const V* __restrict__ L, V* __restrict__ SMO,
-                                        V* __restrict__ GO, V* __restrict__ D, const int p, const int xl,
-                                        const int x0, const int w, const int h, const int ybeg, const int yend,
+__device__ __forceinline__ void fs_iter(FsState<V, NS>& S, const int t, const V* __restrict__ L, V* __restrict__ D, const int p,
+                                        const int xl, const int x0, const int w, const int h, const int ybeg, const int yend,
                                         const bool owns, const FedFacs<V, NS>& fac, const SfTaps<V> kk, const float ikc,
                                         const int lp, const int sh, const FsOut& O)
 {
-    using V4 = typename FedV<V>::V4;
-    constexpr int GS = FsState<V, NS>::GS, PD = FsState<V, NS>::PD;
-    const bool le = x0 == 0, re = x0 + 3 == w - 1;
-    {
-        const V4 Lc = S.Lq[pmod(U, PD)];
+    constexpr int W = FsState<V, NS>::W, GS = FsState<V, NS>::GS, PD = FsState<V, NS>::PD;
+    using Px = FedPx<V, W>;
+    const bool le = x0 == 0, re = x0 + W - 1 == w - 1;
+    {
+        const Px Lc = S.Lq[pmod(U, PD)];
         S.Lr[pmod(U, 6)] = Lc;
-        S.Lq[pmod(U, PD)] = fs_fetch<DEC, V, V4>(L, min(t + PD, h - 1), lp, xl, sh);
-    }
-    {
-        const V4 c = S.Lr[pmod(U, 6)];
-        const V sl1 = wave_shr1(c.w), sl2 = wave_shr1(c.z), sr1 = wave_shl1(c.x), sr2 = wave_shl1(c.y);
-        V4 l1 = mk4(sl1, c.x, c.y, c.z), l2 = mk4(sl2, sl1, c.x, c.y);
-        V4 r1 = mk4(c.y, c.z, c.w, sr1), r2 = mk4(c.z, c.w, sr1, sr2);
+        S.Lq[pmod(U, PD)] = fs_fetch<DEC, V, W>(L, min(t + PD, h - 1), lp, xl, sh);
+    }
+    {
+        const Px c = S.Lr[pmod(U, 6)];
+        V a[W + 4];
+        a[0] = wave_shr1(c.e[W - 2]); a[1] = wave_shr1(c.e[W - 1]);
+#pragma unroll
+        for (int j = 0; j < W; j++) a[2 + j] = c.e[j];
+        a[W + 2] = wave_shl1(c.e[0]); a[W + 3] = wave_shl1(c.e[1]);
         if (XE) {
-            l1.x = le ? c.y : l1.x;
-            l2.x = le ? c.z : l2.x;
-            l2.y = le ? c.y : l2.y;
+            a[1] = le ? a[3] : a[1];
+            a[0] = le ? a[4] : a[0];
             if constexpr (!DEC) {
-                r1.w = re ? c.z : r1.w;
-                r2.z = re ? c.z : r2.z;
-                r2.w = re ? c.y : r2.w;
+                a[W + 2] = re ? a[W] : a[W + 2];
+                a[W + 3] = re ? a[W - 1] : a[W + 3];
             } else {
-                r1.w = re ? c.w : r1.w;
-                r2.z = re ? c.w : r2.z;
-                r2.w = re ? c.z : r2.w;
+                a[W + 2] = re ? a[W + 1] : a[W + 2];
+                a[W + 3] = re ? a[W] : a[W + 3];
             }
         }
-        V4 rp;
-        rp.x = sf_conv(c.x, l1.x, r1.x, l2.x, r2.x, kk);
-        rp.y = sf_conv(c.y, l1.y, r1.y, l2.y, r2.y, kk);
-        rp.z = sf_conv(c.z, l1.z, r1.z, l2.z, r2.z, kk);
-        rp.w = sf_conv(c.w, l1.w, r1.w, l2.w, r2.w, kk);
+        Px rp;
+#pragma unroll
+        for (int j = 0; j < W; j++) rp.e[j] = sf_conv(a[j + 2], a[j + 1], a[j + 3], a[j], a[j + 4], kk);
         S.Rp[pmod(U, 6)] = rp;
         if (YEDGE) {
-            S.Rp[pmod(U - 2, 6)] = vsel4(t == 1, rp, S.Rp[pmod(U - 2, 6)]);
-            S.Rp[pmod(U - 4, 6)] = vsel4(t == 2, rp, S.Rp[pmod(U - 4, 6)]);
+            S.Rp[pmod(U - 2, 6)] = px_sel(t == 1, rp, S.Rp[pmod(U - 2, 6)]);
+            S.Rp[pmod(U - 4, 6)] = px_sel(t == 2, rp, S.Rp[pmod(U - 4, 6)]);
             if constexpr (!DEC) {
-                S.Rp[pmod(U, 6)] = vsel4(t == h, S.Rp[pmod(U - 2, 6)], S.Rp[pmod(U, 6)]);
-                S.Rp[pmod(U, 6)] = vsel4(t == h + 1, S.Rp[pmod(U - 4, 6)], S.Rp[pmod(U, 6)]);
+                S.Rp[pmod(U, 6)] = px_sel(t == h, S.Rp[pmod(U - 2, 6)], S.Rp[pmod(U, 6)]);
+                S.Rp[pmod(U, 6)] = px_sel(t == h + 1, S.Rp[pmod(U - 4, 6)], S.Rp[pmod(U, 6)]);
             } else {
-                S.Rp[pmod(U, 6)] = vsel4(t == h, S.Rp[pmod(U - 1, 6)], S.Rp[pmod(U, 6)]);
-                S.Rp[pmod(U, 6)] = vsel4(t == h + 1, S.Rp[pmod(U - 3, 6)], S.Rp[pmod(U, 6)]);
+                S.Rp[pmod(U, 6)] = px_sel(t == h, S.Rp[pmod(U - 1, 6)], S.Rp[pmod(U, 6)]);
+                S.Rp[pmod(U, 6)] = px_sel(t == h + 1, S.Rp[pmod(U - 3, 6)], S.Rp[pmod(U, 6)]);
             }
         }
     }
     {
         const int a = t - 2;
-        const V4 c = S.Rp[pmod(U - 2, 6)], u1 = S.Rp[pmod(U - 3, 6)], d1 = S.Rp[pmod(U - 1, 6)];
-        const V4 u2 = S.Rp[pmod(U - 4, 6)], d2 = S.Rp[pmod(U, 6)];
-        V4 sm;
-        sm.x = sf_conv(c.x, u1.x, d1.x, u2.x, d2.x, kk);
-        sm.y = sf_conv(c.y, u1.y, d1.y, u2.y, d2.y, kk);
-        sm.z = sf_conv(c.z, u1.z, d1.z, u2.z, d2.z, kk);
-        sm.w = sf_conv(c.w, u1.w, d1.w, u2.w, d2.w, kk);
+        const Px c = S.Rp[pmod(U - 2, 6)], u1 = S.Rp[pmod(U - 3, 6)], d1 = S.Rp[pmod(U - 1, 6)];
+        const Px u2 = S.Rp[pmod(U - 4, 6)], d2 = S.Rp[pmod(U, 6)];
+        Px sm;
+#pragma unroll
+        for (int j = 0; j < W; j++) sm.e[j] = sf_conv(c.e[j], u1.e[j], d1.e[j], u2.e[j], d2.e[j], kk);
         if constexpr (WRITE_SM)
-            hak_buf_store_nt(O.r, O.smo + (a >= ybeg && a < yend ? (unsigned)(a * p) * (unsigned)sizeof(V) : HAK_BUF_OOB), sm);
-        V sl = wave_shr1(sm.w), sr = wave_shl1(sm.x);
+            px_buf_store_nt(O.r, O.smo + (a >= ybeg && a < yend ? (unsigned)(a * p) * (unsigned)sizeof(V) : HAK_BUF_OOB), sm);
+        V sl = wave_shr1(sm.e[W - 1]), sr = wave_shl1(sm.e[0]);
         if (XE) {
-            sl = le ? sm.y : sl;
-            sr = re ? sm.z : sr;
+            sl = le ? sm.e[1] : sl;
+            sr = re ? sm.e[W - 2] : sr;
         }
         S.Sm[pmod(U, 3)] = sm; S.SmL[pmod(U, 3)] = sl; S.SmR[pmod(U, 3)] = sr;
         if (YEDGE && a == 1) { S.Sm[pmod(U - 2, 3)] = sm; S.SmL[pmod(U - 2, 3)] = sl; S.SmR[pmod(U - 2, 3)] = sr; }
@@ -115,55 +117,65 @@
     }
     const int tf = t - 3;
     {
-        const V4 su = S.Sm[pmod(U - 2, 3)], sc = S.Sm[pmod(U - 1, 3)], sd = S.Sm[pmod(U, 3)];
-        const V uL = S.SmL[pmod(U - 2, 3)], uR = S.SmR[pmod(U - 2, 3)];
-        const V cL = S.SmL[pmod(U - 1, 3)], cR = S.SmR[pmod(U - 1, 3)];
-        const V dL = S.SmL[pmod(U, 3)], dR = S.SmR[pmod(U, 3)];
-        V4 g;
-        float4 den;
-#define FS_G(k, ul, uc, ur, cl, cr, ll, lc, lr)                                             \
-        {                                                                                   \
-            const V dx = 10 * ((cr) - (cl)) + 3 * ((ur) + (lr) - (ul) - (ll));              \
-            const V dy = 10 * ((lc) - (uc)) + 3 * ((ll) + (lr) - (ul) - (ur));              \
-            den.k = 1.f + sf_dif2(dx, dy, ikc);                                             \
-        }
-        FS_G(x, uL, su.x, su.y, cL, sc.y, dL, sd.x, sd.y)
-        FS_G(y, su.x, su.y, su.z, sc.x, sc.z, sd.x, sd.y, sd.z)
-        FS_G(z, su.y, su.z, su.w, sc.y, sc.w, sd.y, sd.z, sd.w)
-        FS_G(w, su.z, su.w, uR, sc.z, cR, sd.z, sd.w, dR)
-#undef FS_G
-        const bool fast = den.x < 0x1p64f && den.y < 0x1p64f && den.z < 0x1p64f && den.w < 0x1p64f;
+        V su[W + 2], sc[W + 2], sd[W + 2];
+        su[0] = S.SmL[pmod(U - 2, 3)]; su[W + 1] = S.SmR[pmod(U - 2, 3)];
+        sc[0] = S.SmL[pmod(U - 1, 3)]; sc[W + 1] = S.SmR[pmod(U - 1, 3)];
+        sd[0] = S.SmL[pmod(U, 3)]; sd[W + 1] = S.SmR[pmod(U, 3)];
+#pragma unroll
+        for (int j = 0; j < W; j++) {
+            su[j + 1] = S.Sm[pmod(U - 2, 3)].e[j];
+            sc[j + 1] = S.Sm[pmod(U - 1, 3)].e[j];
+            sd[j + 1] = S.Sm[pmod(U, 3)].e[j];
+        }
+        float den[W];
+        bool fast = true;
+#pragma unroll
+        for (int j = 0; j < W; j++) {
+            const V dx = 10 * (sc[j + 2] - sc[j]) + 3 * (su[j + 2] + sd[j + 2] - su[j] - sd[j]);
+            const V dy = 10 * (sd[j + 1] - su[j + 1]) + 3 * (sd[j] + sd[j + 2] - su[j] - su[j + 2]);
+            den[j] = 1.f + sf_dif2(dx, dy, ikc);
+            fast = fast && den[j] < 0x1p64f;
+        }
+        Px g;
         if (__ballot(!fast) == 0ull) {
-            g = mk4(sf_g_as<V>(hak_rcp_newton(den.x)), sf_g_as<V>(hak_rcp_newton(den.y)), sf_g_as<V>(hak_rcp_newton(den.z)),
-                    sf_g_as<V>(hak_rcp_newton(den.w)));
+#pragma unroll
+            for (int j = 0; j < W; j++) g.e[j] = sf_g_as<V>(hak_rcp_newton(den[j]));
         } else {
-            g = mk4(sf_g_as<V>(1.f / den.x), sf_g_as<V>(1.f / den.y), sf_g_as<V>(1.f / den.z), sf_g_as<V>(1.f / den.w));
-        }
-        if (WRITE_G) hak_buf_store_nt(O.r, O.go + (tf >= ybeg && tf < yend ? (unsigned)(tf * p) * (unsigned)sizeof(V) : HAK_BUF_OOB), g);
-        const V gr = wave_shl1(g.x);
-        S.GH[pmod(U, GS)] = GHrow<V>{vadd(g.x, g.y), vadd(g.y, g.z), vadd(g.z, g.w), vadd(g.w, gr)};
-        S.GV[pmod(U - 1, GS)] = mk4(vadd(S.gprev.x, g.x), vadd(S.gprev.y, g.y), vadd(S.gprev.z, g.z), vadd(S.gprev.w, g.w));
+#pragma unroll
+            for (int j = 0; j < W; j++) g.e[j] = sf_g_as<V>(1.f / den[j]);
+        }
+        if (WRITE_G) px_buf_store_nt(O.r, O.go + (tf >= ybeg && tf < yend ? (unsigned)(tf * p) * (unsigned)sizeof(V) : HAK_BUF_OOB), g);
+        S.GH[pmod(U, GS)] = fed_gh(g);
+        S.GV[pmod(U - 1, GS)] = px_add(S.gprev, g);
         S.gprev = g;
     }
 #pragma unroll
     for (int k = 1; k <= NS; k++) {
         const int rho = tf - k;
-        const V4 Lc = k == 1 ? S.Lr[pmod(U - 3 - 1, 6)] : S.Lw[k - 1][pmod(U - k, 2)];
-        const V4 Ls = k == 1 ? S.Lr[pmod(U - 3, 6)] : S.Lw[k - 1][pmod(U - k + 1, 2)];
-        V4 Qn = fed_q<V, V4>(S.GV[pmod(U - k, GS)], Ls, Lc);
-        V4 Qp = S.Qw[k - 1][pmod(U - k - 1, 2)];
+        const Px Lc = k == 1 ? S.Lr[pmod(U - 3 - 1, 6)] : S.Lw[k - 1][pmod(U - k, 2)];
+        const Px Ls = k == 1 ? S.Lr[pmod(U - 3, 6)] : S.Lw[k - 1][pmod(U - k + 1, 2)];
+        Px Qn = fed_q(S.GV[pmod(U - k, GS)], Ls, Lc);
+        Px Qp = S.Qw[k - 1][pmod(U - k - 1, 2)];
         if (YEDGE) {
-            Qp = vsel4(rho == 0, vneg4(Qn), Qp);
-            Qn = vsel4(rho == h - 1, vneg4(Qp), Qn);
+            Qp = px_sel(rho == 0, px_neg(Qn), Qp);
+            Qn = px_sel(rho == h - 1, px_neg(Qp), Qn);
         }
         S.Qw[k - 1][pmod(U - k, 2)] = Qn;
-        const V4 out = fed_row<XE, V, V4>(Lc, S.GH[pmod(U - k, GS)], Qn, Qp, x0, w, fac.f[k - 1]);
+        const Px out = fed_row<XE>(Lc, S.GH[pmod(U - k, GS)], Qn, Qp, x0, w, fac.f[k - 1]);
         if (k < NS) {
             S.Lw[k < NS ? k : 0][pmod(U - k, 2)] = out;
         } else if (rho >= ybeg && rho < yend && owns) {
-            hak_store_nt(reinterpret_cast<V4*>(D + (long)rho * p + x0), out);
-        }
-    }
+            px_store_nt(D + (long)rho * p + x0, out);
+        }
+    }
+}
+template <typename V, int NS, bool YEDGE, bool XE, bool WRITE_G, bool DEC, bool WRITE_SM, int... U>
+__device__ __forceinline__ void fs_body(std::integer_sequence<int, U...>, FsState<V, NS>& S, const int tb, const V* __restrict__ L,
+                                        V* __restrict__ D, const int p, const int xl, const int x0, const int w, const int h,
+                                        const int ybeg, const int yend, const bool owns, const FedFacs<V, NS>& fac,
+                                        const SfTaps<V> kk, const float ikc, const int lp, const int sh, const FsOut& O)
+{
+    (fs_iter<V, NS, U, YEDGE, XE, WRITE_G, DEC, WRITE_SM>(S, tb + U, L, D, p, xl, x0, w, h, ybeg, yend, owns, fac, kk, ikc, lp, sh, O), ...);
 }
 
 template <typename V, int NS, bool XE, bool WRITE_G, bool DEC, bool WRITE_SM>
@@ -172,8 +184,9 @@
                                          const SfTaps<V> kk, const float ikc, int x0, int ybeg, int yend, bool owns,
                                          const int lp, const int sh)
 {
-    using V4 = typename FedV<V>::V4;
-    const int xl = min(max(x0, 0), p - 4);
+    using St = FsState<V, NS>;
+    constexpr int W = St::W, UF = St::UF;
+    const int xl = min(max(x0, 0), p - W);
     FsOut O;
     {
         V* lo = SMO ? SMO : GO;
@@ -185,45 +198,35 @@
     }
     const int t0 = max(0, ybeg - NS - 4);
     const int tend = min(yend - 1, h - 1) + NS + 3;
-    FsState<V, NS> S;
+    St S;
     const V z = 0;
-    const V4 z4 = mk4(z, z, z, z);
-#pragma unroll
-    for (int i = 0; i < 6; i++) { S.Lr[i] = z4; S.Rp[i] = z4; }
-#pragma unroll
-    for (int i = 0; i < 3; i++) { S.Sm[i] = z4; S.SmL[i] = z; S.SmR[i] = z; }
-#pragma unroll
-    for (int k = 0; k < NS; k++) S.Lw[k][0] = S.Lw[k][1] = S.Qw[k][0] = S.Qw[k][1] = z4;
-#pragma unroll
-    for (int i = 0; i < FsState<V, NS>::GS; i++) {
-        S.GH[i] = GHrow<V>{z, z, z, z};
-        S.GV[i] = z4;
-    }
-    S.gprev = z4;
-#pragma unroll
-    for (int i = 0; i < FsState<V, NS>::PD; i++)
-        S.Lq[i] = fs_fetch<DEC, V, V4>(L, min(t0 + i, h - 1), lp, xl, sh);
-    for (int tb = t0; tb <= tend; tb += 6) {
-        if (tb <= NS + 4 || tb + 5 >= h) {
-            fs_iter<V, NS, 0, true, XE, WRITE_G, DEC, WRITE_SM>(S, tb + 0, L, SMO, GO, D, p, xl, x0, w, h, ybeg, yend, owns, fac, kk, ikc, lp, sh, O);
-            fs_iter<V, NS, 1, true, XE, WRITE_G, DEC, WRITE_SM>(S, tb + 1, L, SMO, GO, D, p, xl, x0, w, h, ybeg, yend, owns, fac, kk, ikc, lp, sh, O);
-            fs_iter<V, NS, 2, true, XE, WRITE_G, DEC, WRITE_SM>(S, tb + 2, L, SMO, GO, D, p, xl, x0, w, h, ybeg, yend, owns, fac, kk, ikc, lp, sh, O);
-            fs_iter<V, NS, 3, true, XE, WRITE_G, DEC, WRITE_SM>(S, tb + 3, L, SMO, GO, D, p, xl, x0, w, h, ybeg, yend, owns, fac, kk, ikc, lp, sh, O);
-            fs_iter<V, NS, 4, true, XE, WRITE_G, DEC, WRITE_SM>(S, tb + 4, L, SMO, GO, D, p, xl, x0, w, h, ybeg, yend, owns, fac, kk, ikc, lp, sh, O);
-            fs_iter<V, NS, 5, true, XE, WRITE_G, DEC, WRITE_SM>(S, tb + 5, L, SMO, GO, D, p, xl, x0, w, h, ybeg, yend, owns, fac, kk, ikc, lp, sh, O);
-        } else {
-            fs_iter<V, NS, 0, false, XE, WRITE_G, DEC, WRITE_SM>(S, tb + 0, L, SMO, GO, D, p, xl, x0, w, h, ybeg, yend, owns, fac, kk, ikc, lp, sh, O);
-            fs_iter<V, NS, 1, false, XE, WRITE_G, DEC, WRITE_SM>(S, tb + 1, L, SMO, GO, D, p, xl, x0, w, h, ybeg, yend, owns, fac, kk, ikc, lp, sh, O);
-            fs_iter<V, NS, 2, false, XE, WRITE_G, DEC, WRITE_SM>(S, tb + 2, L, SMO, GO, D, p, xl, x0, w, h, ybeg, yend, owns, fac, kk, ikc, lp, sh, O);
-            fs_iter<V, NS, 3, false, XE, WRITE_G, DEC, WRITE_SM>(S, tb + 3, L, SMO, GO, D, p, xl, x0, w, h, ybeg, yend, owns, fac, kk, ikc, lp, sh, O);
-            fs_iter<V, NS, 4, false, XE, WRITE_G, DEC, WRITE_SM>(S, tb + 4, L, SMO, GO, D, p, xl, x0, w, h, ybeg, yend, owns, fac, kk, ikc, lp, sh, O);
-            fs_iter<V, NS, 5, false, XE, WRITE_G, DEC, WRITE_SM>(S, tb + 5, L, SMO, GO, D, p, xl, x0, w, h, ybeg, yend, owns, fac, kk, ikc, lp, sh, O);
-        }
-    }
-}
-
-constexpr int FS_HX = 8;
-constexpr int FS_XV = 256 - 2 * FS_HX;
+    const FedPx<V, W> zp = px_fill<V, W>(z);
+#pragma unroll
+    for (int i = 0; i < 6; i++) { S.Lr[i] = zp; S.Rp[i] = zp; }
+#pragma unroll
+    for (int i = 0; i < 3; i++) { S.Sm[i] = zp; S.SmL[i] = z; S.SmR[i] = z; }
+#pragma unroll
+    for (int k = 0; k < NS; k++) S.Lw[k][0] = S.Lw[k][1] = S.Qw[k][0] = S.Qw[k][1] = zp;
+#pragma unroll
+    for (int i = 0; i < St::GS; i++) {
+#pragma unroll
+        for (int j = 0; j < W; j++) S.GH[i].h[j] = z;
+        S.GV[i] = zp;
+    }
+    S.gprev = zp;
+#pragma unroll
+    for (int i = 0; i < St::PD; i++)
+        S.Lq[i] = fs_fetch<DEC, V, W>(L, min(t0 + i, h - 1), lp, xl, sh);
+    for (int tb = t0; tb <= tend; tb += UF) {
+        if (tb <= NS + 4 || tb + UF - 1 >= h)
+            fs_body<V, NS, true, XE, WRITE_G, DEC, WRITE_SM>(std::make_integer_sequence<int, UF>{}, S, tb, L, D, p, xl, x0, w, h, ybeg, yend, owns, fac, kk, ikc, lp, sh, O);
+        else
+            fs_body<V, NS, false, XE, WRITE_G, DEC, WRITE_SM>(std::make_integer_sequence<int, UF>{}, S, tb, L, D, p, xl, x0, w, h, ybeg, yend, owns, fac, kk, ikc, lp, sh, O);
+    }
+}
+
+constexpr int fs_hx(int ns) { return ns + 3 <= 8 ? 8 : (ns + 3 + 3) & ~3; }
+constexpr int fs_xv(int ns) { return 64 * fed_lane_px(ns) - 2 * fs_hx(ns); }
 
 template <typename V, int NS, bool WRITE_G, bool DEC, bool WRITE_SM>
 __global__ __launch_bounds__(256) void k_fed_sf(const V* __restrict__ src, V* __restrict__ smooth, V* __restrict__ flow,
@@ -231,6 +234,7 @@
                                                 FedFacs<V, NS> fac, SfTaps<V> kk, const HakImgState* __restrict__ state, int octave,
                                                 float fixed_ikc, int ry, int nbx, int nby, int nimg, int lp, int sh)
 {
+    constexpr int W = fed_lane_px(NS), HX = fs_hx(NS), XV = fs_xv(NS);
     int bx, by, img;
     if (!hak_xcd_decode(nbx, nby, nimg, bx, by, img)) return;
     const V* L = src + (long)img * stride;
@@ -240,12 +244,12 @@
     const float ikc = state ? state[img].ikc[octave] : fixed_ikc;
     const int lane = threadIdx.x & 63;
     const int wv = __builtin_amdgcn_readfirstlane(threadIdx.x >> 6);
-    const int x0 = bx * FS_XV - FS_HX + 4 * lane;
+    const int x0 = bx * XV - HX + W * lane;
     const int ybeg = (by * 4 + wv) * ry;
     if (ybeg >= h) return;
     const int yend = min(ybeg + ry, h);
-    const bool owns = 4 * lane >= FS_HX && 4 * lane < FS_HX + FS_XV && x0 < w && x0 >= 0;
-    if (bx == 0 || (bx + 1) * FS_XV + FS_HX >= w) fs_strip<V, NS, true, WRITE_G, DEC, WRITE_SM>(L, SMO, GO, D, w, h, p, fac, kk, ikc, x0, ybeg, yend, owns, lp, sh);
+    const bool owns = W * lane >= HX && W * lane < HX + XV && x0 < w && x0 >= 0;
+    if (bx == 0 || (bx + 1) * XV + HX >= w) fs_strip<V, NS, true, WRITE_G, DEC, WRITE_SM>(L, SMO, GO, D, w, h, p, fac, kk, ikc, x0, ybeg, yend, owns, lp, sh);
     else fs_strip<V, NS, false, WRITE_G, DEC, WRITE_SM>(L, SMO, GO, D, w, h, p, fac, kk, ikc, x0, ybeg, yend, owns, lp, sh);
 }
 
@@ -259,7 +263,8 @@
         if constexpr (std::is_same<V, float>::value) fac.f[k] = 0.5f * tau[k];
         else fac.f[k] = (int)(0.5f * tau[k] * 65536 + 0.5f);
     }
-    const int gx = (w + FS_XV - 1) / FS_XV;
+    constexpr int XV = fs_xv(NS);
+    const int gx = (w + XV - 1) / XV;
     const int ry = hak_stream_rows(h, (long)gx * nimg, 8);
     const int gy = (h + 4 * ry - 1) / (4 * ry);
     const unsigned grid = hak_xcd_grid(gx, gy, nimg);
@@ -282,14 +287,25 @@
                    SfTaps<V> kk, int diffusivity, const float* tau, int ns, const HakImgState* state, int octave, float fixed_ikc,
                    bool write_g, int sp = 0, int sh = 0)
 {
-    if (diffusivity != HAK_PM_G2 || (w & 3) || w < 16 || h < 8 || ns < 1 || ns > 4) return false;
+    constexpr int max_ns = std::is_same<V, float>::value ? HAK_FED_MAX_FUSE : HAK_FED_WIDE_STEPS;
+    if (diffusivity != HAK_PM_G2 || (w & 3) || w < 16 || h < 8 || ns < 1 || ns > max_ns) return false;
     if (!smooth && (sp > 0 || !std::is_same<V, float>::value)) return false;
     if ((write_g && smooth ? (flow < smooth ? smooth - flow : flow - smooth) : 0L) + (long)h * p >= (long)HAK_BUF_OOB / (long)sizeof(V)) return false;
     switch (ns) {
     case 1: launch_fs<V, 1>(st, src, smooth, flow, dst, stride, w, h, p, nimg, kk, tau, state, octave, fixed_ikc, write_g, sp, sh); break;
     case 2: launch_fs<V, 2>(st, src, smooth, flow, dst, stride, w, h, p, nimg, kk, tau, state, octave, fixed_ikc, write_g, sp, sh); break;
     case 3: launch_fs<V, 3>(st, src, smooth, flow, dst, stride, w, h, p, nimg, kk, tau, state, octave, fixed_ikc, write_g, sp, sh); break;
-    default: launch_fs<V, 4>(st, src, smooth, flow, dst, stride, w, h, p, nimg, kk, tau, state, octave, fixed_ikc, write_g, sp, sh); break;
+    case 4: launch_fs<V, 4>(st, src, smooth, flow, dst, stride, w, h, p, nimg, kk, tau, state, octave, fixed_ikc, write_g, sp, sh); break;
+    default:
+        if constexpr (std::is_same<V, float>::value) {
+            switch (ns) {
+            case 5: launch_fs<V, 5>(st, src, smooth, flow, dst, stride, w, h, p, nimg, kk, tau, state, octave, fixed_ikc, write_g, sp, sh); break;
+            case 6: launch_fs<V, 6>(st, src, smooth, flow, dst, stride, w, h, p, nimg, kk, tau, state, octave, fixed_ikc, write_g, sp, sh); break;
+            case 7: launch_fs<V, 7>(st, src, smooth, flow, dst, stride, w, h, p, nimg, kk, tau, state, octave, fixed_ikc, write_g, sp, sh); break;
+            default: launch_fs<V, 8>(st, src, smooth, flow, dst, stride, w, h, p, nimg, kk, tau, state, octave, fixed_ikc, write_g, sp, sh); break;
+            }
+        }
+        break;
     }
     return true;
 }
```

Result: faster. 6327 pairs/s, median of 6 (+2.6%).
